# ruolin/strawberry

Measured on NVIDIA B200. Metric: fragments*EM-iters/sec, higher is better.
Workload: dtype f64

## Files before the change

### strawberry_b200/csrc/sbq.cu

```cuda
#include <algorithm>
#include <chrono>
#include <cstdarg>
#include <cstdio>
#include <cstdlib>
#include <cstring>
#include <dlfcn.h>
#include <mutex>
#include <string>
#include <thread>
#include <vector>

#include <nccl.h>

#include "../../include/sbq.h"
#include "../../include/sbq_builder.h"
#include "sbq_kernels.cuh"
#include "sbq_grid.cuh"
#include "sbq_grid_tma.cuh"
#include "sbq_grid_dual.cuh"
#include "sbq_bias.cuh"
#include "sbq_weights.cuh"
#include "sbq_synth.cuh"
#include "sbq_rawbuild.cuh"

// ... 226 lines not shown
   if (cudaPointerGetAttributes(&a, p) != cudaSuccess) {
      cudaGetLastError();
      return false;
   }
   return a.type == cudaMemoryTypeHost;
}

int materialise(sbq_ctx* c) {
   if (!c->borrowed) return SBQ_SUCCESS;
   if (c->host_released) return fail(c, SBQ_ERR_STATE, "the borrowed batch was released by sbq_upload: sbq_clear and submit again");
   bool ok = true;
   c->h_loc_row_off.clear(); c->h_loc_iso_off.clear(); c->h_row_ptr.clear();
   c->h_col.clear(); c->h_count.clear(); c->h_iso_len.clear(); c->h_alpha.clear();
   ok &= c->h_loc_row_off.append(c->b_loc_row_off, c->n_loci + 1);
   ok &= c->h_loc_iso_off.append(c->b_loc_iso_off, c->n_loci + 1);
   ok &= c->h_row_ptr.append(c->b_row_ptr, c->n_row + 1);
   ok &= c->h_col.append(c->b_col, c->nnz);
   ok &= c->h_alpha.append(c->b_alpha, c->nnz);
   ok &= c->h_count.append(c->b_count, c->n_row);
   ok &= c->h_iso_len.append(c->b_iso_len, c->n_iso);
   c->borrowed = false;
   return ok ? SBQ_SUCCESS : fail(c, SBQ_ERR_NOMEM, "pinned staging allocation failed");
}

void reset_batch(sbq_ctx* c) {
   c->borrowed = false;
   c->host_released = false;
   c->meta.clear();
   c->h_loc_row_off.clear(); c->h_loc_iso_off.clear(); c->h_row_ptr.clear();
   c->h_col.clear(); c->h_count.clear(); c->h_iso_len.clear(); c->h_alpha.clear();
   c->n_loci = c->n_row = c->n_iso = c->nnz = 0;
   c->have_cov = false;
   c->h_cov.clear();
   c->deferred = 0;
   c->raw.clear();
   c->raw_mode = false;
   c->h_wseg.clear(); c->h_wn.clear(); c->h_wmask.clear(); c->h_wpool.clear(); c->h_wlen.clear(); c->h_wpool_off.clear();
   c->resident = c->solved = c->downloaded = false;
}

int ensure_origin(sbq_ctx* c) {
   if (c->h_loc_row_off.n == 0) {
      int64_t z = 0;
      if (!c->h_loc_row_off.append(&z, 1) || !c->h_loc_iso_off.append(&z, 1) || !c->h_row_ptr.append(&z, 1))
         return fail(c, SBQ_ERR_NOMEM, "pinned staging allocation failed");
   }
   return SBQ_SUCCESS;
}

constexpr int N_BUCKETS = 5;
const int BUCKET_NT[N_BUCKETS] = {64, 128, 512, 512, 512};
int smem_bucket(size_t bytes) { return bytes <= 12 * 1024 ? 0 : bytes <= 24 * 1024 ? 1 : bytes <= 56 * 1024 ? 2 : bytes <= 112 * 1024 ? 3 : 4; }

constexpr int64_t SGRID_MAX_NNZ = 1000 * 1000;
constexpr int SGRID_CTAS_DEFAULT = 32;
inline int sgrid_ctas() {
   static const int v = getenv("SBQ_SGRID_CTAS") ? std::max(1, atoi(getenv("SBQ_SGRID_CTAS"))) : SGRID_CTAS_DEFAULT;
   return v;
}
#define SGRID_CTAS sgrid_ctas()

int cluster_size_for(int64_t nnz) {
   static int64_t th[4] = {16 * 1024, 32 * 1024, 64 * 1024, 150 * 1024};
   static bool init = false;
   if (!init) {
      init = true;
      if (const char* e = std::getenv("SBQ_CS_THRESH")) {
         long long a, b, c2, d;
         if (std::sscanf(e, "%lld,%lld,%lld,%lld", &a, &b, &c2, &d) == 4) { th[0] = a * 1024; th[1] = b * 1024; th[2] = c2 * 1024; th[3] = d * 1024; }
      }
   }
   if (nnz <= th[0]) return 1;
   if (nnz <= th[1]) return 2;
   if (nnz <= th[2]) return 4;
   if (nnz <= th[3]) return 8;
   return 16;
}

void capture_meta_host(sbq_ctx* c) {
   const int64_t *lro = loc_row_off(c), *lio = loc_iso_off(c), *rp = row_ptr(c);
   c->meta.resize((size_t)c->n_loci);
   for (int64_t l = 0; l < c->n_loci; ++l)
      c->meta[l] = {rp[lro[l + 1]] - rp[lro[l]], 0, (int32_t)(lro[l + 1] - lro[l]), (int32_t)(lio[l + 1] - lio[l])};
}

int plan(sbq_ctx* c) {
   c->warp_list.clear();
   c->grid_list.clear();
   c->sgrid_list.clear();
   c->sgrid_max_iso = c->sgrid_max_iso_dual = 1;
   c->sgrid_tma_ok = true;
   c->classes.clear();
   c->warp_max_iso = 1;
   c->max_iso_all = 1;
   c->grid_max_iso = 1;
   c->grid_max_iso_dual = 1;
   c->grid_tma_ok = true;
   c->grid_dual_ok = !getenv("SBQ_GRID_NO_DUAL");
   const bool force_dual = getenv("SBQ_GRID_DUAL") != nullptr;
   static const bool sgrid_enabled = !getenv("SBQ_NO_SGRID");
   std::vector<char> dual_locus(c->n_loci, 0);
   std::vector<int64_t> nnz_of(c->n_loci);
   LaunchClass* slot[5][N_BUCKETS] = {};
   std::vector<LaunchClass> tmp;
   tmp.reserve(20);
   static const int64_t grid_min_nnz = getenv("SBQ_GRID_MIN_NNZ") ? atoll(getenv("SBQ_GRID_MIN_NNZ")) : 300 * 1000;
   for (int64_t l = 0; l < c->n_loci; ++l) {
      const int64_t R = c->meta[l].R, T = c->meta[l].T, nnz = c->meta[l].nnz;
      nnz_of[l] = nnz;
      c->max_iso_all = std::max(c->max_iso_all, (int)T);
      if (T > SBQ_MAX_ISO) return fail(c, SBQ_ERR_UNSUPPORTED, "locus %lld has %lld isoforms (> SBQ_MAX_ISO)", (long long)l, (long long)T);
      int tier;
      if (c->force_tier) tier = c->force_tier;
      else if (T <= WT_MAX_ISO && R <= WT_MAX_ROWS && nnz <= WT_MAX_NNZ) tier = 1;
      else if (nnz >= grid_min_nnz) tier = 3;
      else tier = 2;
      if (tier == 1 && T > WT_MAX_ISO) tier = 2;
      if (tier == 3 && !grid_tier_supports((int)T)) tier = 2;
      if (tier == 2 && cluster_stream_groups((int)T, SMEM_CAP, CL_NT, 1, 0) <= 0) {
         if (!grid_tier_supports((int)T)) return fail(c, SBQ_ERR_UNSUPPORTED, "locus %lld: %lld isoforms fit no tier", (long long)l, (long long)T);
         tier = 3;
      }
      if (tier == 1) {
         c->warp_list.push_back((int32_t)l);
         c->warp_max_iso = std::max(c->warp_max_iso, (int)T);
      } else if (tier == 3) {
         const bool small = !c->force_tier && sgrid_enabled && nnz < SGRID_MAX_NNZ;
         (small ? c->sgrid_list : c->grid_list).push_back((int32_t)l);
         const bool dual = c->grid_dual_ok && (grid_dual_supports_iso((int)T) || (force_dual && grid_dual_possible((int)T))) &&
                           nnz < (1LL << 32) && nnz <= 56 * R;
         dual_locus[l] = dual;
         int& mx_dual = small ? c->sgrid_max_iso_dual : c->grid_max_iso_dual;
         int& mx_rest = small ? c->sgrid_max_iso : c->grid_max_iso;
         bool& tma_ok = small ? c->sgrid_tma_ok : c->grid_tma_ok;
         if (dual) {
            mx_dual = std::max(mx_dual, (int)T);
         } else {
            mx_rest = std::max(mx_rest, (int)T);
            if (!grid_tma_supports((int)T, (long long)R, small ? SGRID_CTAS : c->prop.multiProcessorCount)) tma_ok = false;
         }
      } else {
         int cs = c->force_cluster ? c->force_cluster : cluster_size_for(nnz);
         int csi = cs == 1 ? 0 : cs == 2 ? 1 : cs == 4 ? 2 : cs == 8 ? 3 : 4;
         const size_t slice = cluster_slice_estimate(nnz, R, (int)T, cs);
         const int bucket = cs == 1 ? smem_bucket(cluster_fixed_doubles((int)T, 1, slice) * sizeof(double) + slice + 256) : N_BUCKETS - 1;
         if (!slot[csi][bucket]) {
            tmp.push_back(LaunchClass{cs, BUCKET_NT[bucket], {}, 0, 0, 0, 0});
            slot[csi][bucket] = &tmp.back();
         }
         LaunchClass* lc = slot[csi][bucket];
         lc->loci.push_back((int32_t)l);
         lc->max_iso = std::max(lc->max_iso, (int)T);
         lc->max_slice = std::max(lc->max_slice, slice);
         lc->smem = std::max(lc->smem, cluster_class_smem((int)T, slice, lc->lpr, cs));
      }
   }
   auto by_size = [&](int32_t a, int32_t b) { return nnz_of[a] != nnz_of[b] ? nnz_of[a] > nnz_of[b] : a < b; };
   {
      bool small_keys = true;
      for (int32_t l : c->warp_list) small_keys &= nnz_of[l] <= WT_MAX_NNZ;
      if (small_keys) {
         std::vector<int32_t> first(WT_MAX_NNZ + 2, 0), sorted(c->warp_list.size());
         for (int32_t l : c->warp_list) ++first[WT_MAX_NNZ - (int)nnz_of[l] + 1];
         for (int k = 1; k <= WT_MAX_NNZ + 1; ++k) first[k] += first[k - 1];
         for (int32_t l : c->warp_list) sorted[first[WT_MAX_NNZ - (int)nnz_of[l]]++] = l;
         c->warp_list.swap(sorted);
      } else {
         std::sort(c->warp_list.begin(), c->warp_list.end(), by_size);
      }
   }
   auto order_grid = [&](std::vector<int32_t>& list, size_t& n_dual, std::vector<int64_t>& rec_off) {
      std::sort(list.begin(), list.end(), [&](int32_t a, int32_t b) {
         if (dual_locus[a] != dual_locus[b]) return dual_locus[a] > dual_locus[b];
         if (dual_locus[a]) {
            const int na = grid_dual_nc(c->meta[a].T), nb_ = grid_dual_nc(c->meta[b].T);
            if (na != nb_) return na > nb_;
         }
         return by_size(a, b);
      });
      n_dual = 0;
      for (int32_t l : list) n_dual += dual_locus[l];
      rec_off.assign(n_dual + 1, 0);
      for (size_t i = 0; i < n_dual; ++i) rec_off[i + 1] = rec_off[i] + c->meta[list[i]].R + 1;
   };
   order_grid(c->grid_list, c->grid_n_dual, c->grid_rec_off);
   order_grid(c->sgrid_list, c->sgrid_n_dual, c->sgrid_rec_off);
   for (auto& lc : tmp) {
      std::sort(lc.loci.begin(), lc.loci.end(), by_size);
      if (cluster_stream_groups(lc.max_iso, SMEM_CAP, lc.lpr, 1, 0) <= 0)
         return fail(c, SBQ_ERR_UNSUPPORTED, "locus with %d isoforms does not fit the cluster tier", lc.max_iso);
      c->classes.push_back(std::move(lc));
   }
   std::sort(c->classes.begin(), c->classes.end(), [](const LaunchClass& a, const LaunchClass& b) { return a.cs != b.cs ? a.cs > b.cs : a.max_slice > b.max_slice; });

   c->h_lists.clear();
   c->warp_list_off = 0;
   if (!c->h_lists.append(c->warp_list.data(), c->warp_list.size())) return fail(c, SBQ_ERR_NOMEM, "list staging");
   c->grid_list_off = c->h_lists.n;
   if (!c->h_lists.append(c->grid_list.data(), c->grid_list.size())) return fail(c, SBQ_ERR_NOMEM, "list staging");
   c->sgrid_list_off = c->h_lists.n;
   if (!c->h_lists.append(c->sgrid_list.data(), c->sgrid_list.size())) return fail(c, SBQ_ERR_NOMEM, "list staging");
   for (auto& lc : c->classes) {
      lc.list_off = c->h_lists.n;
      if (!c->h_lists.append(lc.loci.data(), lc.loci.size())) return fail(c, SBQ_ERR_NOMEM, "list staging");
   }
   c->stats.loci_warp = (int64_t)c->warp_list.size();
   c->stats.loci_grid = (int64_t)(c->grid_list.size() + c->sgrid_list.size());
   c->stats.loci_cta = c->n_loci - c->stats.loci_warp - c->stats.loci_grid;
   return SBQ_SUCCESS;
}

size_t align_up(size_t x, size_t a = 256) { return (x + a - 1) / a * a; }

int alloc_device(sbq_ctx* c) {
   const size_t sz_lro = align_up((c->n_loci + 1) * sizeof(int64_t)), sz_rp = align_up((c->n_row + 1) * sizeof(int64_t) + 64);
   const size_t sz_col = align_up(c->nnz * sizeof(int32_t) + 64), sz_al = align_up(c->nnz * sizeof(double) + 64);
   const size_t sz_cnt = align_up(c->n_row * sizeof(int32_t) + 64), sz_il = align_up(c->n_iso * sizeof(int32_t));
   const size_t in_bytes = 2 * sz_lro + sz_rp + sz_col + sz_al + 2 * sz_cnt + sz_il;
   const size_t sz_iso_d = align_up(c->n_iso * sizeof(double)), sz_iso_i = align_up(c->n_iso * sizeof(int32_t));
   const size_t sz_loc_i = align_up(c->n_loci * sizeof(int32_t)), sz_loc_d = align_up(c->n_loci * sizeof(double));
   const size_t out_bytes = 4 * sz_iso_d + sz_iso_i + 2 * sz_loc_i + sz_loc_d + 256;
   if (!c->d_in.reserve(in_bytes) || !c->d_out.reserve(out_bytes) || !c->d_lists.reserve(align_up((size_t)c->n_loci * sizeof(int32_t)) + 256))
      return fail(c, SBQ_ERR_NOMEM, "device allocation failed (%zu MB)", (in_bytes + out_bytes) >> 20);

   char* p = (char*)c->d_in.p;
   DevParams& dp = c->dp;
   auto carve = [&](size_t bytes) { char* q = p; p += bytes; return q; };
   int64_t* d_lro = (int64_t*)carve(sz_lro);
   int64_t* d_lio = (int64_t*)carve(sz_lro);
   int64_t* d_rp = (int64_t*)carve(sz_rp);
   int32_t* d_col = (int32_t*)carve(sz_col);
   double* d_al = (double*)carve(sz_al);
   int32_t* d_cnt = (int32_t*)carve(sz_cnt);
   dp.neff = (int32_t*)carve(sz_cnt);
   int32_t* d_il = (int32_t*)carve(sz_il);
   dp.csc = nullptr;
   dp.loc_row_off = d_lro; dp.loc_iso_off = d_lio; dp.row_ptr = d_rp; dp.col = d_col; dp.alpha = d_al;
   dp.count = d_cnt; dp.iso_len = d_il;
   p = (char*)c->d_out.p;
   dp.theta = (double*)carve(sz_iso_d);
   dp.fpkm = (double*)carve(sz_iso_d);
   dp.frac = (double*)carve(sz_iso_d);
   c->d_tpm = (double*)carve(sz_iso_d);
   dp.keep = (int32_t*)carve(sz_iso_i);
   dp.iters = (int32_t*)carve(sz_loc_i);
   dp.status = (int32_t*)carve(sz_loc_i);
   dp.locus_fpkm = (double*)carve(sz_loc_d);
   c->d_fpkm_sum = (double*)carve(256);
   c->d_lists_p = (int32_t*)c->d_lists.p;
   return SBQ_SUCCESS;
}

template <typename K>
int set_kernel_attrs(sbq_ctx* c, K kernel, size_t smem, bool nonportable) {
   CU(cudaFuncSetAttribute(kernel, cudaFuncAttributeMaxDynamicSharedMemorySize, (int)smem));
   if (nonportable) CU(cudaFuncSetAttribute(kernel, cudaFuncAttributeNonPortableClusterSizeAllowed, 1));
   return SBQ_SUCCESS;
}

template <int NT, int NCACHE, int MINB>
int launch_cluster_class_nt(sbq_ctx* c, const LaunchClass& lc, cudaStream_t st) {
   auto kernel = em_cluster_kernel<NT, NCACHE, MINB>;
   int rc = set_kernel_attrs(c, kernel, lc.smem, lc.cs > 8);
   if (rc) return rc;
   cudaLaunchConfig_t cfg{};
   cfg.gridDim = dim3((unsigned)(lc.loci.size() * lc.cs));
   cfg.blockDim = dim3(NT);
   cfg.dynamicSmemBytes = lc.smem;
   cfg.stream = st;
   cudaLaunchAttribute attr[1];
   attr[0].id = cudaLaunchAttributeClusterDimension;
   attr[0].val.clusterDim.x = (unsigned)lc.cs;
   attr[0].val.clusterDim.y = 1;
   attr[0].val.clusterDim.z = 1;
   cfg.attrs = attr;
   cfg.numAttrs = 1;
   const int32_t* list = c->d_lists_p + lc.list_off;
   CU(cudaLaunchKernelEx(&cfg, kernel, c->dp, list, (int)lc.loci.size(), (unsigned)lc.smem));
   return SBQ_SUCCESS;
}

struct StagingMark {
   size_t lro, lio, rp, col, al, cnt, il, wseg, wn, wmask, wlen, wpool, wpoff;
   int64_t n_loci, n_row, n_iso, nnz;
   explicit StagingMark(const sbq_ctx* c)
       : lro(c->h_loc_row_off.n), lio(c->h_loc_iso_off.n), rp(c->h_row_ptr.n), col(c->h_col.n), al(c->h_alpha.n), cnt(c->h_count.n), il(c->h_iso_len.n),
         wseg(c->h_wseg.n), wn(c->h_wn.n), wmask(c->h_wmask.n), wlen(c->h_wlen.n), wpool(c->h_wpool.n), wpoff(c->h_wpool_off.n),
         n_loci(c->n_loci), n_row(c->n_row), n_iso(c->n_iso), nnz(c->nnz) {}
   void restore(sbq_ctx* c) const {
      c->h_loc_row_off.n = lro; c->h_loc_iso_off.n = lio; c->h_row_ptr.n = rp; c->h_col.n = col; c->h_alpha.n = al; c->h_count.n = cnt; c->h_iso_len.n = il;
      c->h_wseg.n = wseg; c->h_wn.n = wn; c->h_wmask.n = wmask; c->h_wlen.n = wlen; c->h_wpool.n = wpool; c->h_wpool_off.n = wpoff;
      c->n_loci = n_loci; c->n_row = n_row; c->n_iso = n_iso; c->nnz = nnz;
   }
};

int submit_locked(sbq_ctx* c, const sbq_locus* loci, int64_t n_loci) {
   if (c->host_released) return fail(c, SBQ_ERR_STATE, "the borrowed batch was released by sbq_upload: sbq_clear and submit again");
   for (int64_t l = 0; l < n_loci; ++l) {
      const sbq_locus& L = loci[l];
      if (L.n_iso < 1 || L.n_row < 0 || !L.row_ptr || !L.iso_len || (L.n_row > 0 && !L.count))
         return fail(c, SBQ_ERR_INVALID, "locus %lld: bad shape or null pointer", (long long)l);
      if (L.n_iso > SBQ_MAX_ISO) return fail(c, SBQ_ERR_UNSUPPORTED, "locus %lld: %d isoforms > SBQ_MAX_ISO", (long long)l, L.n_iso);
      for (int32_t i = 1; i <= L.n_row; ++i)
         if (L.row_ptr[i] < L.row_ptr[i - 1]) return fail(c, SBQ_ERR_INVALID, "locus %lld: row_ptr not monotone", (long long)l);
      if (L.row_ptr[L.n_row] > L.row_ptr[0] && (!L.col || !L.alpha)) return fail(c, SBQ_ERR_INVALID, "locus %lld: null col / alpha", (long long)l);
   }
   cudaSetDevice(c->device);
   int rc = materialise(c);
   if (rc) return rc;
   if ((rc = ensure_origin(c))) return rc;
   const StagingMark mark(c);
   for (int64_t l = 0; l < n_loci; ++l) {
      const sbq_locus& L = loci[l];
      const int64_t k0 = L.row_ptr[0], k1 = L.row_ptr[L.n_row];
      const int64_t base = c->nnz - k0;
      bool ok = c->h_row_ptr.reserve(c->h_row_ptr.n + L.n_row);
      if (ok) {
         for (int32_t i = 1; i <= L.n_row; ++i) c->h_row_ptr.p[c->h_row_ptr.n++] = L.row_ptr[i] + base;
         ok = c->h_col.append(L.col + k0, k1 - k0) && c->h_alpha.append(L.alpha + k0, k1 - k0) &&
              c->h_count.append(L.count, L.n_row) && c->h_iso_len.append(L.iso_len, L.n_iso);
      }
      c->nnz += k1 - k0;
      c->n_row += L.n_row;
      c->n_iso += L.n_iso;
      c->n_loci += 1;
      ok = ok && c->h_loc_row_off.append(&c->n_row, 1) && c->h_loc_iso_off.append(&c->n_iso, 1);
      if (!ok) {
         mark.restore(c);
         return fail(c, SBQ_ERR_NOMEM, "pinned staging");
      }
   }
   c->resident = c->solved = c->downloaded = false;
   return SBQ_SUCCESS;
}

}

#include "sbq_multi.cuh"

extern "C" {

int sbq_abi_version(void) { return SBQ_ABI_VERSION; }

const char* sbq_error_string(int err) {
   switch (err) {
      case SBQ_SUCCESS: return "success";
      case SBQ_ERR_INVALID: return "invalid argument";
      case SBQ_ERR_NO_DEVICE: return "no CUDA device (libsbq has no CPU path)";
      case SBQ_ERR_CUDA: return "CUDA runtime error";
      case SBQ_ERR_NOMEM: return "out of memory";
      case SBQ_ERR_STATE: return "invalid call sequence";
      case SBQ_ERR_UNSUPPORTED: return "shape outside supported limits";
      default: return "unknown error";
   }
}

const char* sbq_last_error(const sbq_ctx* c) { return c ? c->err.c_str() : ""; }

void sbq_config_default(sbq_config* cfg) {
   if (!cfg) return;
   memset(cfg, 0, sizeof *cfg);
   cfg->device = -1;
   cfg->max_iter = 1000;
   cfg->theta_tol = 1e-2;
   cfg->row_eps = 1e-5;
   cfg->min_iso_frac = 0.0;
   cfg->effective_len_norm = 0;
   cfg->insert_mean = 0.0;
   cfg->bias_mode = 0;
   cfg->max_out_it = 100;
   cfg->max_theta_it = 5000;
   cfg->max_bias_it = 10;
   cfg->bias_tol = 1e-2;
   cfg->n_gpus = 1;
}

int sbq_create(const sbq_config* cfg, sbq_ctx** out) {
   if (!cfg || !out) return SBQ_ERR_INVALID;
   *out = nullptr;
   if (cfg->max_iter < 1 || !(cfg->theta_tol >= 0) || cfg->bias_mode < 0 || cfg->bias_mode > 1) return SBQ_ERR_INVALID;
   if (cfg->bias_mode == 1 && (cfg->max_out_it < 1 || cfg->max_theta_it < 1 || cfg->max_bias_it < 1 || !(cfg->bias_tol >= 0))) return SBQ_ERR_INVALID;
   if (cfg->n_gpus < 0 || cfg->n_gpus > 64) return SBQ_ERR_INVALID;
   setenv("CUDA_DEVICE_MAX_CONNECTIONS", "32", 0);
   int ndev = 0;
   if (cudaGetDeviceCount(&ndev) != cudaSuccess || ndev == 0) {
      cudaGetLastError();
      return SBQ_ERR_NO_DEVICE;
   }
   int dev = cfg->device;
   if (dev < 0) {
      if (cfg->n_gpus > 1) dev = 0;
      else if (cudaGetDevice(&dev) != cudaSuccess) return SBQ_ERR_NO_DEVICE;
   }
   if (dev >= ndev) return SBQ_ERR_INVALID;
   if (cfg->n_gpus > 1 && dev + cfg->n_gpus > ndev) return SBQ_ERR_NO_DEVICE;
   sbq_ctx* c = new sbq_ctx();
   c->cfg = *cfg;
   c->device = dev;
   auto bail = [&](int code) { sbq_destroy(c); return code; };
   if (cudaSetDevice(dev) != cudaSuccess) return bail(SBQ_ERR_CUDA);
   if (cudaGetDeviceProperties(&c->prop, dev) != cudaSuccess) return bail(SBQ_ERR_CUDA);
   if (c->prop.major < 10) return bail(SBQ_ERR_NO_DEVICE);
   if (cudaStreamCreateWithFlags(&c->stream, cudaStreamNonBlocking) != cudaSuccess) return bail(SBQ_ERR_CUDA);
   if (cudaStreamCreateWithFlags(&c->copy_st, cudaStreamNonBlocking) != cudaSuccess) return bail(SBQ_ERR_CUDA);
   if (cudaEventCreateWithFlags(&c->ev_grid_ready, cudaEventDisableTiming) != cudaSuccess) return bail(SBQ_ERR_CUDA);
   for (auto& e : c->ev_class_ready)
      if (cudaEventCreateWithFlags(&e, cudaEventDisableTiming) != cudaSuccess) return bail(SBQ_ERR_CUDA);
   for (auto& s : c->side)
      if (cudaStreamCreateWithFlags(&s, cudaStreamNonBlocking) != cudaSuccess) return bail(SBQ_ERR_CUDA);
   for (auto& e : c->ev)
      if (cudaEventCreate(&e) != cudaSuccess) return bail(SBQ_ERR_CUDA);
   if (cudaEventCreateWithFlags(&c->ev_fork, cudaEventDisableTiming) != cudaSuccess) return bail(SBQ_ERR_CUDA);
   for (auto& e : c->ev_join)
      if (cudaEventCreateWithFlags(&e, cudaEventDisableTiming) != cudaSuccess) return bail(SBQ_ERR_CUDA);
   for (auto& t : c->lt)
// ... 89 lines not shown
   if (rows < 0 || isos < n_loci) return fail(c, SBQ_ERR_INVALID, "bad locus offsets");
   const int64_t k0 = rp[lro[0]], k1 = rp[lro[n_loci]];
   if (k1 < k0 || (k1 > k0 && (!col || !alpha)) || (rows > 0 && !count)) return fail(c, SBQ_ERR_INVALID, "bad CSR arrays");
   for (int64_t l = 0; l < n_loci; ++l) {
      const int64_t T = lio[l + 1] - lio[l];
      if (lro[l + 1] < lro[l] || T < 1) return fail(c, SBQ_ERR_INVALID, "locus %lld: bad shape", (long long)l);
      if (T > SBQ_MAX_ISO) return fail(c, SBQ_ERR_UNSUPPORTED, "locus %lld: %lld isoforms > SBQ_MAX_ISO", (long long)l, (long long)T);
   }
   if (c->n_loci == 0 && lro[0] == 0 && lio[0] == 0 && k0 == 0 && is_pinned(lro) && is_pinned(lio) && is_pinned(rp) &&
       is_pinned(iso_len) && (rows == 0 || is_pinned(count)) && (k1 == 0 || (is_pinned(col) && is_pinned(alpha)))) {
      c->borrowed = true;
      c->b_loc_row_off = lro; c->b_loc_iso_off = lio; c->b_row_ptr = rp;
      c->b_col = col; c->b_alpha = alpha; c->b_count = count; c->b_iso_len = iso_len;
      c->n_loci = n_loci; c->n_row = rows; c->n_iso = isos; c->nnz = k1;
      c->deferred = 2;
      c->resident = c->solved = c->downloaded = false;
      return SBQ_SUCCESS;
   }
   if (c->host_released) return fail(c, SBQ_ERR_STATE, "the borrowed batch was released by sbq_upload: sbq_clear and submit again");
   for (int64_t i = lro[0]; i < lro[n_loci]; ++i)
      if (rp[i + 1] < rp[i]) return fail(c, SBQ_ERR_INVALID, "row %lld: row_ptr not monotone", (long long)i);
   int rc = materialise(c);
   if (rc) return rc;
   if ((rc = ensure_origin(c))) return rc;
   const bool ok = c->h_loc_row_off.reserve(c->h_loc_row_off.n + n_loci) && c->h_loc_iso_off.reserve(c->h_loc_iso_off.n + n_loci) &&
                   c->h_row_ptr.reserve(c->h_row_ptr.n + rows) && c->h_col.reserve(c->h_col.n + (k1 - k0)) && c->h_alpha.reserve(c->h_alpha.n + (k1 - k0)) &&
                   c->h_count.reserve(c->h_count.n + rows) && c->h_iso_len.reserve(c->h_iso_len.n + isos);
   if (!ok) return fail(c, SBQ_ERR_NOMEM, "pinned staging");
   for (int64_t l = 1; l <= n_loci; ++l) {
      c->h_loc_row_off.p[c->h_loc_row_off.n++] = c->n_row + (lro[l] - lro[0]);
      c->h_loc_iso_off.p[c->h_loc_iso_off.n++] = c->n_iso + (lio[l] - lio[0]);
   }
   const int64_t base = c->nnz - k0;
   for (int64_t i = 1; i <= rows; ++i) c->h_row_ptr.p[c->h_row_ptr.n++] = rp[lro[0] + i] + base;
   c->h_col.append(col + k0, k1 - k0);
   c->h_alpha.append(alpha + k0, k1 - k0);
   c->h_count.append(count + lro[0], rows);
   c->h_iso_len.append(iso_len + lio[0], isos);
   c->n_loci += n_loci; c->n_row += rows; c->n_iso += isos; c->nnz += k1 - k0;
   c->deferred = 2;
   c->resident = c->solved = c->downloaded = false;
   return SBQ_SUCCESS;
}

int sbq_validate(sbq_ctx* c) {
   if (!c) return SBQ_ERR_INVALID;
   std::lock_guard<std::mutex> lk(c->mu);
   if (c->host_released) return fail(c, SBQ_ERR_STATE, "the borrowed batch was released by sbq_upload");
   const int64_t *lro = loc_row_off(c), *lio = loc_iso_off(c), *rp = row_ptr(c);
   const int32_t* col = colp(c);
   for (int64_t l = 0; l < c->n_loci; ++l) {
      const int64_t T = lio[l + 1] - lio[l];
      for (int64_t i = lro[l]; i < lro[l + 1]; ++i) {
         if (rp[i + 1] < rp[i]) return fail(c, SBQ_ERR_INVALID, "locus %lld row %lld: row_ptr not monotone", (long long)l, (long long)(i - lro[l]));
         for (int64_t k = rp[i]; k < rp[i + 1]; ++k) {
            if (col[k] < 0 || col[k] >= T) return fail(c, SBQ_ERR_INVALID, "locus %lld: column %d out of range", (long long)l, col[k]);
            if (k > rp[i] && col[k] <= col[k - 1]) return fail(c, SBQ_ERR_INVALID, "locus %lld row %lld: columns not strictly ascending", (long long)l, (long long)(i - lro[l]));
         }
      }
   }
   return SBQ_SUCCESS;
}

}

static int raw_upload(sbq_ctx* c);

static int upload_begin(sbq_ctx* c) {
   CU(cudaSetDevice(c->device));
   if (c->upload_pending) {
      CU(cudaStreamSynchronize(c->copy_st));
      c->upload_pending = false;
   }
   if (c->n_loci == 0) return fail(c, SBQ_ERR_STATE, "nothing submitted");
   if (c->host_released) return fail(c, SBQ_ERR_STATE, "the borrowed batch was released by the previous sbq_upload: sbq_clear and submit again");
   {
      const int rc = alloc_device(c);
      if (rc) return rc;
   }
   DevParams& dp = c->dp;
   int64_t *d_lro = const_cast<int64_t*>(dp.loc_row_off), *d_lio = const_cast<int64_t*>(dp.loc_iso_off), *d_rp = const_cast<int64_t*>(dp.row_ptr);
   int32_t *d_col = const_cast<int32_t*>(dp.col), *d_cnt = const_cast<int32_t*>(dp.count), *d_il = const_cast<int32_t*>(dp.iso_len);
   double* d_al = const_cast<double*>(dp.alpha);

   cudaStream_t st = c->copy_st;
   c->upload_pending = true;
   c->resident = c->solved = c->downloaded = false;
   CU(cudaEventRecord(c->ev[0], st));
   CU(cudaMemcpyAsync(d_lro, loc_row_off(c), (c->n_loci + 1) * sizeof(int64_t), cudaMemcpyHostToDevice, st));
   CU(cudaMemcpyAsync(d_lio, loc_iso_off(c), (c->n_loci + 1) * sizeof(int64_t), cudaMemcpyHostToDevice, st));
   CU(cudaMemcpyAsync(d_rp, row_ptr(c), (c->n_row + 1) * sizeof(int64_t), cudaMemcpyHostToDevice, st));
   if (c->n_row) CU(cudaMemcpyAsync(d_cnt, countp(c), c->n_row * sizeof(int32_t), cudaMemcpyHostToDevice, st));
   CU(cudaMemcpyAsync(d_il, iso_lenp(c), c->n_iso * sizeof(int32_t), cudaMemcpyHostToDevice, st));
   if (!c->r_frags.reserve((size_t)c->n_loci) || !c->d_frags.reserve(align_up((size_t)c->n_loci * 8))) return fail(c, SBQ_ERR_NOMEM, "fragment-total buffers");
   locus_frags_kernel<<<std::max(1, std::min<int>((int)((c->n_loci + 7) / 8), c->prop.multiProcessorCount * 8)), 256, 0, st>>>(d_lro, d_cnt, c->n_loci, (long long*)c->d_frags.p);
   CU(cudaGetLastError());
   CU(cudaMemcpyAsync(c->r_frags.p, c->d_frags.p, (size_t)c->n_loci * 8, cudaMemcpyDeviceToHost, st));
   if (c->nnz) CU(cudaMemcpyAsync(d_col, colp(c), c->nnz * sizeof(int32_t), cudaMemcpyHostToDevice, st));
   const bool timing = getenv("SBQ_TIMING") != nullptr;
   const auto t_plan0 = std::chrono::steady_clock::now();
   {
      capture_meta_host(c);
      const int rc = plan(c);
      if (rc) {
         cudaStreamSynchronize(st);
         c->upload_pending = false;
         return rc;
      }
   }
   if (timing) fprintf(stderr, "SBQ_TIMING plan_ms %.3f\n", std::chrono::duration<double, std::milli>(std::chrono::steady_clock::now() - t_plan0).count());
   if (c->h_lists.n) CU(cudaMemcpyAsync(c->d_lists_p, c->h_lists.p, c->h_lists.n * sizeof(int32_t), cudaMemcpyHostToDevice, st));
   const int64_t* lro = loc_row_off(c);
   const int64_t* rp = row_ptr(c);
   const double* al = alphap(c);
   std::vector<std::pair<int64_t, int64_t>> done;
   auto copy_loci = [&](const std::vector<int32_t>& loci) -> int {
      for (int32_t l : loci) {
         const int64_t k0 = rp[lro[l]], k1 = rp[lro[l + 1]];
         if (k1 > k0) {
            CU(cudaMemcpyAsync(d_al + k0, al + k0, (size_t)(k1 - k0) * sizeof(double), cudaMemcpyHostToDevice, st));
            done.emplace_back(k0, k1);
         }
      }
      return SBQ_SUCCESS;
   };
   for (auto& r : c->class_ready) r = false;
   c->grid_ready = false;
   if (!(c->grid_list.empty() && c->sgrid_list.empty()) && c->grid_list.size() + c->sgrid_list.size() <= 16) {
      int rc = copy_loci(c->grid_list);
      if (rc) return rc;
      rc = copy_loci(c->sgrid_list);
      if (rc) return rc;
      CU(cudaEventRecord(c->ev_grid_ready, st));
      c->grid_ready = true;
   }
   size_t n_prio = 0;
   for (size_t i = 0; i < c->classes.size() && i < (size_t)N_SIDE_STREAMS; ++i) {
      if (c->classes[i].cs < 8 || n_prio + c->classes[i].loci.size() > 48) continue;
      n_prio += c->classes[i].loci.size();
      const int rc = copy_loci(c->classes[i].loci);
      if (rc) return rc;
      CU(cudaEventRecord(c->ev_class_ready[i], st));
      c->class_ready[i] = true;
   }
   std::sort(done.begin(), done.end());
   int64_t pos = 0;
   for (size_t i = 0; i <= done.size(); ++i) {
      const int64_t end = i < done.size() ? done[i].first : c->nnz;
      if (end > pos) CU(cudaMemcpyAsync(d_al + pos, al + pos, (size_t)(end - pos) * sizeof(double), cudaMemcpyHostToDevice, st));
      if (i < done.size()) pos = std::max(pos, done[i].second);
   }
   CU(cudaEventRecord(c->ev[1], st));
   if (!c->classes.empty()) {
      if (!c->d_csc.reserve(align_up(c->nnz * 4 + 16))) return fail(c, SBQ_ERR_NOMEM, "device allocation failed (transposed-index scratch)");
      dp.csc = (unsigned*)c->d_csc.p;
   }
   c->stats.h2d_bytes = 2 * (c->n_loci + 1) * 8 + (c->n_row + 1) * 8 + c->nnz * 12 + c->n_row * 4 + c->n_iso * 4 + (int64_t)c->h_lists.n * 4;
   c->stats.n_loci = c->n_loci; c->stats.n_row = c->n_row; c->stats.n_iso = c->n_iso; c->stats.nnz = c->nnz;
   c->stats.weights_ms = 0.0;
   c->col16_ready = false;
   c->resident = true;
   return SBQ_SUCCESS;
}

static int upload_wait(sbq_ctx* c) {
   if (!c->upload_pending) return SBQ_SUCCESS;
   CU(cudaSetDevice(c->device));
   CU(cudaStreamSynchronize(c->copy_st));
   c->upload_pending = false;
   if (c->borrowed) c->host_released = true;
   for (size_t l = 0; l < c->meta.size(); ++l) c->meta[l].frags = c->r_frags.p[l];
   float ms = 0;
   CU(cudaEventElapsedTime(&ms, c->ev[0], c->ev[1]));
   c->stats.upload_ms = ms;
   return SBQ_SUCCESS;
}

extern "C" {

int sbq_upload_begin(sbq_ctx* c) {
   if (!c) return SBQ_ERR_INVALID;
   if (c->multi || c->deferred == 1 || c->raw_mode || c->cfg.bias_mode == 1) return sbq_upload(c);
   std::lock_guard<std::mutex> lk(c->mu);
   return upload_begin(c);
}

int sbq_upload(sbq_ctx* c) {
   if (!c) return SBQ_ERR_INVALID;
   if (c->multi) return multi_upload(c);
   std::lock_guard<std::mutex> lk(c->mu);
   if (c->raw_mode) {
      if (c->n_loci == 0) return fail(c, SBQ_ERR_STATE, "nothing submitted");
      return raw_upload(c);
   }
   {
      int rc = upload_begin(c);
      if (!rc) rc = upload_wait(c);
      if (rc) return rc;
   }
   if (c->deferred == 1) {
      if (!c->have_model) return fail(c, SBQ_ERR_STATE, "deferred weights need sbq_set_insert_model()");
      if ((int64_t)c->h_wseg.n != c->nnz) return fail(c, SBQ_ERR_STATE, "deferred-weight descriptors do not cover the batch");
      const size_t b_seg = align_up(c->nnz * 8 + 8), b_n = align_up(c->nnz + 8), b_m = align_up(c->nnz * 4 + 8), b_l = align_up(c->nnz * 4 + 8);
      const size_t b_pool = align_up(c->h_wpool.n * 4 + 8), b_emp = align_up(c->model_emp.size() * 8 + 8);
      if (!c->d_weights.reserve(b_seg + b_n + b_m + b_l + b_pool + b_emp)) return fail(c, SBQ_ERR_NOMEM, "device allocation failed (weight descriptors)");
      char* q = (char*)c->d_weights.p;
      int64_t* d_seg = (int64_t*)q; q += b_seg;
      uint8_t* d_n = (uint8_t*)q; q += b_n;
      uint32_t* d_m = (uint32_t*)q; q += b_m;
      int32_t* d_l = (int32_t*)q; q += b_l;
      uint32_t* d_pool = (uint32_t*)q; q += b_pool;
      double* d_emp = (double*)q;
      cudaStream_t st = c->stream;
      CU(cudaEventRecord(c->ev[5], st));
      CU(cudaMemcpyAsync(d_seg, c->h_wseg.p, c->nnz * 8, cudaMemcpyHostToDevice, st));
      CU(cudaMemcpyAsync(d_n, c->h_wn.p, c->nnz, cudaMemcpyHostToDevice, st));
      CU(cudaMemcpyAsync(d_m, c->h_wmask.p, c->nnz * 4, cudaMemcpyHostToDevice, st));
      CU(cudaMemcpyAsync(d_l, c->h_wlen.p, c->nnz * 4, cudaMemcpyHostToDevice, st));
      if (c->h_wpool.n) CU(cudaMemcpyAsync(d_pool, c->h_wpool.p, c->h_wpool.n * 4, cudaMemcpyHostToDevice, st));
      if (!c->model_emp.empty()) CU(cudaMemcpyAsync(d_emp, c->model_emp.data(), c->model_emp.size() * 8, cudaMemcpyHostToDevice, st));
      WeightModel wm{c->model.use_emp, c->model.start_offset, c->model.end_offset, c->model.total_reads, d_emp, c->model.mean, c->model.sd, c->model_read_len};
      const int blocks = std::max(1, std::min<int>((int)((c->nnz + 7) / 8), c->prop.multiProcessorCount * 16));
      weights_kernel<<<blocks, 256, 0, st>>>(c->nnz, d_seg, d_n, d_m, d_l, d_pool, wm, const_cast<double*>(c->dp.alpha));
      CU(cudaGetLastError());
      CU(cudaEventRecord(c->ev[6], st));
      CU(cudaStreamSynchronize(st));
      float wms = 0;
      CU(cudaEventElapsedTime(&wms, c->ev[5], c->ev[6]));
      c->weights_ms = wms;
      c->stats.weights_ms = wms;
      c->stats.h2d_bytes += (int64_t)(c->nnz * 17 + c->h_wpool.n * 4 + c->model_emp.size() * 8);
   }
   if (c->cfg.bias_mode == 1) {
      if (!c->have_cov) return fail(c, SBQ_ERR_STATE, "bias_mode = 1 needs sbq_set_covariates() after the last submit");
      const size_t K = (size_t)c->n_cov;
      const size_t bx = align_up(c->n_row * K * 8 + 8), bw = align_up(c->n_row * 8 + 8), bb = align_up(c->n_loci * K * 8 + 8), bo = align_up(c->n_loci * 4 + 8);
      if (!c->d_bias.reserve(bx + 2 * bw + bb + 2 * bo + 64)) return fail(c, SBQ_ERR_NOMEM, "device allocation failed (bias scratch)");
      char* q = (char*)c->d_bias.p;
      c->bpar.x = (const double*)q; q += bx;
      c->bpar.w = (double*)q; q += bw;
      c->bpar.d = (double*)q; q += bw;
      c->bpar.beta = (double*)q; q += bb;
      c->bpar.outer = (int32_t*)q; q += bo;
      c->d_bias_list = (int32_t*)q; q += bo;
      c->d_bias_queue = (int*)q;
      c->bpar.n_cov = c->n_cov;
      {
         c->bias_list.clear();
         std::vector<int32_t> cls[6];
         for (int k = 0; k < 6; ++k) c->bias_cls[k] = BiasClass{};
         for (int64_t l = 0; l < c->n_loci; ++l) {
            const int cs = bias_cluster_size(c->meta[l].nnz);
            const int k = bias_warp_tier(c->meta[l].nnz, c->meta[l].R, c->meta[l].T) ? 5 : cs == 16 ? 0 : cs == 8 ? 1 : cs == 4 ? 2 : cs == 2 ? 3 : 4;
            cls[k].push_back((int32_t)l);
            c->bias_cls[k].cs = cs;
            c->bias_cls[k].max_iso = std::max(c->bias_cls[k].max_iso, (int)c->meta[l].T);
         }
         for (int k = 0; k < 6; ++k) {
            std::sort(cls[k].begin(), cls[k].end(), [&](int32_t a, int32_t b) { return c->meta[a].nnz != c->meta[b].nnz ? c->meta[a].nnz > c->meta[b].nnz : a < b; });
            c->bias_cls[k].off = c->bias_list.size();
            c->bias_cls[k].n = cls[k].size();
            c->bias_list.insert(c->bias_list.end(), cls[k].begin(), cls[k].end());
         }
         if (c->n_loci) CU(cudaMemcpyAsync(c->d_bias_list, c->bias_list.data(), c->n_loci * 4, cudaMemcpyHostToDevice, c->stream));
      }
      if (K) CU(cudaMemcpyAsync((void*)c->bpar.x, c->h_cov.p, c->n_row * K * 8, cudaMemcpyHostToDevice, c->stream));
      CU(cudaStreamSynchronize(c->stream));
      c->stats.h2d_bytes += (int64_t)(c->n_row * K * 8);
   }
   c->resident = true;
   c->col16_ready = false;
   c->solved = c->downloaded = false;
   return SBQ_SUCCESS;
}

int sbq_solve(sbq_ctx* c, int64_t total_mapped_reads) {
   if (!c) return SBQ_ERR_INVALID;
   if (c->multi) return multi_solve(c, total_mapped_reads);
   std::lock_guard<std::mutex> lk(c->mu);
   CU(cudaSetDevice(c->device));
   if (!c->resident) return fail(c, SBQ_ERR_STATE, "sbq_solve before sbq_upload");

   DevParams& dp = c->dp;
   dp.max_iter = c->cfg.max_iter;
   dp.tol = c->cfg.theta_tol;
   dp.row_eps = c->cfg.row_eps;
   dp.min_frac = c->cfg.min_iso_frac;
   dp.eff_len_norm = c->cfg.effective_len_norm;
   dp.insert_mean = c->cfg.insert_mean;
   dp.rpm = 1e6 / (double)(int)total_mapped_reads;

   cudaStream_t st = c->stream;
   int64_t launches = 0;
   if (c->cfg.bias_mode == 1) {
      const size_t smem = bias_smem_bytes(c->max_iso_all);
      if (smem > SMEM_CAP) return fail(c, SBQ_ERR_UNSUPPORTED, "bias mode supports up to %d isoforms per locus", (int)((SMEM_CAP / 8 - 8) / (5 + BI_W)));
      c->bpar.max_out_it = c->cfg.max_out_it;
      c->bpar.max_theta_it = c->cfg.max_theta_it;
      c->bpar.max_bias_it = c->cfg.max_bias_it;
      c->bpar.bias_tol = c->cfg.bias_tol;
      int rc_attr = set_kernel_attrs(c, em_bias_kernel, smem, c->bias_cls[0].n > 0);
      if (rc_attr) return rc_attr;
      CU(cudaEventRecord(c->ev[2], st));
      CU(cudaEventRecord(c->ev_fork, st));
      int n_side = 0;
      if (c->bias_cls[5].n) {
         const BiasClass& bc = c->bias_cls[5];
         cudaStream_t ss = c->side[n_side];
         CU(cudaStreamWaitEvent(ss, c->ev_fork, 0));
         ++n_side;
         const size_t wsmem = bias_warp_smem_bytes();
         CU(cudaFuncSetAttribute(em_bias_warp_kernel, cudaFuncAttributeMaxDynamicSharedMemorySize, (int)wsmem));
         int occ = 1;
         CU(cudaOccupancyMaxActiveBlocksPerMultiprocessor(&occ, em_bias_warp_kernel, BW_WARPS * 32, wsmem));
         const long long want = ((long long)bc.n + BW_WARPS - 1) / BW_WARPS;
         const unsigned grid = (unsigned)std::max(1LL, std::min(want, (long long)c->prop.multiProcessorCount * std::max(1, occ)));
         CU(cudaMemsetAsync(c->d_bias_queue, 0, sizeof(int), ss));
         em_bias_warp_kernel<<<grid, BW_WARPS * 32, wsmem, ss>>>(c->dp, c->bpar, (const int32_t*)(c->d_bias_list + bc.off), (int)bc.n, c->d_bias_queue);
         CU(cudaGetLastError());
         ++launches;
      }
      for (int k = 0; k < 5; ++k) {
         const BiasClass& bc = c->bias_cls[k];
         if (!bc.n) continue;
         cudaStream_t ss = c->side[n_side % N_SIDE_STREAMS];
         if (n_side < N_SIDE_STREAMS) CU(cudaStreamWaitEvent(ss, c->ev_fork, 0));
         ++n_side;
         cudaLaunchConfig_t cfg{};
         cfg.gridDim = dim3((unsigned)(bc.n * bc.cs));
         cfg.blockDim = dim3(BI_NT);
         cfg.dynamicSmemBytes = bias_smem_bytes(bc.max_iso);
         cfg.stream = ss;
         cudaLaunchAttribute attr[1];
         attr[0].id = cudaLaunchAttributeClusterDimension;
         attr[0].val.clusterDim.x = (unsigned)bc.cs;
         attr[0].val.clusterDim.y = 1;
         attr[0].val.clusterDim.z = 1;
         cfg.attrs = attr;
         cfg.numAttrs = 1;
         CU(cudaLaunchKernelEx(&cfg, em_bias_kernel, c->dp, c->bpar, (const int32_t*)(c->d_bias_list + bc.off), (int)bc.n));
         ++launches;
      }
      for (int i = 0; i < std::min(n_side, N_SIDE_STREAMS); ++i) {
         CU(cudaEventRecord(c->ev_join[i], c->side[i]));
         CU(cudaStreamWaitEvent(st, c->ev_join[i], 0));
      }
      CU(cudaEventRecord(c->ev[3], st));
      fpkm_sum_kernel<<<1, 1024, 0, st>>>(dp.locus_fpkm, c->n_loci, c->d_fpkm_sum);
      CU(cudaGetLastError());
      CU(cudaEventRecord(c->ev[4], st));
      CU(cudaStreamSynchronize(st));
      float ms_ = 0;
      CU(cudaEventElapsedTime(&ms_, c->ev[2], c->ev[4]));
      c->stats.solve_ms = ms_;
      CU(cudaEventElapsedTime(&ms_, c->ev[2], c->ev[3]));
      c->stats.em_ms = ms_;
      c->stats.grid_em_ms = 0;
      c->stats.kernel_launches = launches + 1;
      c->launch_stats.clear();
      c->locus_launch.assign(c->n_loci, -1);
      c->solved = true;
      c->downloaded = false;
      return SBQ_SUCCESS;
   }
   CU(cudaEventRecord(c->ev[2], st));
   CU(cudaEventRecord(c->ev_fork, st));
   int used_side = 0;
   c->stats.grid_em_ms = 0;
   for (auto& t : c->lt) t.used = false;
   const bool pending = c->upload_pending;
   auto launch_grid_part = [&](const std::vector<int32_t>& list, size_t list_off, size_t n_dual_, const std::vector<int64_t>& rec_off, int max_iso_rest,
                               bool tma_ok, const cudaDeviceProp& prop_, DevBuf& scratch, DevBuf& rowrec, DevBuf& pkbuf, cudaStream_t gs_, int& variant,
                               int& n_launch) -> int {
      int rc = 0;
      variant = 0;
      const int32_t* d_grid = c->d_lists_p + list_off;
      const int n_dual = (int)n_dual_, n_rest = (int)list.size() - n_dual;
      if (n_dual) {
         GridDualBufs bf{&scratch.p, &scratch.cap, &c->d_col16.p, &c->d_col16.cap, &rowrec.p, &rowrec.cap, &pkbuf.p, &pkbuf.cap};
         int nl = 0;
         std::vector<int> h_iso((size_t)n_dual);
         for (int i = 0; i < n_dual; ++i) h_iso[i] = c->meta[list[i]].T;
         rc = grid_dual_launch(c->dp, c->nnz, d_grid, n_dual, h_iso.data(), rec_off.data(), prop_, bf, c->col16_ready, gs_, &nl);
         n_launch += nl;
         variant = 3;
      }
      if (rc == 0 && n_rest) {
         int nl = 0;
         if (tma_ok && !getenv("SBQ_GRID_NO_TMA")) {
            if (!variant) variant = 2;
            rc = grid_tma_launch(c->dp, c->nnz, d_grid + n_dual, n_rest, max_iso_rest, prop_, &scratch.p, &scratch.cap,
                                 &c->d_col16.p, &c->d_col16.cap, c->col16_ready, gs_, &nl);
         } else {
            if (!variant) variant = 1;
            rc = grid_tier_launch(c->dp, d_grid + n_dual, n_rest, prop_, &scratch.p, &scratch.cap, gs_, &nl);
         }
         n_launch += nl;
      }
      return rc;
   };
   auto grid_failed = [&](int rc) -> int {
      c->resident = false;
      c->col16_ready = false;
      return fail(c, rc < -6 ? SBQ_ERR_CUDA : rc, "grid tier launch failed: %s", cudaGetErrorString(cudaGetLastError()));
   };
   if (!(c->grid_list.empty() && c->sgrid_list.empty())) {
      const size_t need16 = (size_t)c->nnz * 2 + 256;
      if (need16 > c->d_col16.cap) {
         if (!c->d_col16.reserve(need16)) return fail(c, SBQ_ERR_NOMEM, "device allocation failed (16-bit slots)");
         c->col16_ready = false;
      }
   }
   if (!c->grid_list.empty()) {
      if (pending) CU(cudaStreamWaitEvent(st, c->grid_ready ? c->ev_grid_ready : c->ev[1], 0));
      CU(cudaEventRecord(c->ev[6], st));
      int n_launch = 0;
      const int rc = launch_grid_part(c->grid_list, c->grid_list_off, c->grid_n_dual, c->grid_rec_off, c->grid_max_iso, c->grid_tma_ok, c->prop,
                                      c->d_grid_scratch, c->d_rowrec, c->d_pk, st, c->grid_variant, n_launch);
      if (rc != 0) return grid_failed(rc);
      launches += n_launch;
      CU(cudaEventRecord(c->ev[7], st));
   }
   c->lt_sgrid.used = false;
   if (!c->sgrid_list.empty()) {
      cudaDeviceProp prop_sg = c->prop;
      prop_sg.multiProcessorCount = std::min(SGRID_CTAS, c->prop.multiProcessorCount);
      cudaStream_t gs_ = c->sgrid_st;
      CU(cudaStreamWaitEvent(gs_, c->ev_fork, 0));
      if (pending) CU(cudaStreamWaitEvent(gs_, c->grid_ready ? c->ev_grid_ready : c->ev[1], 0));
      if (!c->grid_list.empty()) {
         CU(cudaStreamWaitEvent(gs_, c->ev[7], 0));
      }
      CU(cudaEventRecord(c->lt_sgrid.e0, gs_));
      int n_launch = 0;
      const int rc = launch_grid_part(c->sgrid_list, c->sgrid_list_off, c->sgrid_n_dual, c->sgrid_rec_off, c->sgrid_max_iso, c->sgrid_tma_ok, prop_sg,
                                      c->d_sgrid_scratch, c->d_srowrec, c->d_spk, gs_, c->sgrid_variant, n_launch);
      if (rc != 0) return grid_failed(rc);
      launches += n_launch;
      CU(cudaEventRecord(c->lt_sgrid.e1, gs_));
      CU(cudaEventRecord(c->ev_sgrid_join, gs_));
      c->lt_sgrid.used = true;
   }
   if (!(c->grid_list.empty() && c->sgrid_list.empty())) c->col16_ready = true;
   const bool serialize = getenv("SBQ_SERIALIZE") != nullptr;
   static const int order_mode = getenv("SBQ_ORDER") ? atoi(getenv("SBQ_ORDER")) : SBQ_DEFAULT_ORDER;
   const int ncls = (int)c->classes.size();
   std::vector<int> ord;
   int warp_pos = ncls;
   {
      std::vector<int> big, small, rest;
      for (int i = 0; i < ncls; ++i) {
         const LaunchClass& lc = c->classes[i];
         if (lc.lpr < CL_NT) small.push_back(i);
         else if (lc.cs >= (order_mode == 3 ? 16 : 8)) big.push_back(i);
         else rest.push_back(i);
      }
      if (order_mode == 1) { ord = small; ord.insert(ord.end(), big.begin(), big.end()); ord.insert(ord.end(), rest.begin(), rest.end()); warp_pos = 0; }
      else if (order_mode == 2 || order_mode == 3) { ord = big; warp_pos = (int)ord.size(); ord.insert(ord.end(), small.begin(), small.end()); ord.insert(ord.end(), rest.begin(), rest.end()); }
      else { for (int i = 0; i < ncls; ++i) ord.push_back(i); }
   }
   auto launch_warp = [&]() -> int {
      if (c->warp_list.empty()) return SBQ_SUCCESS;
      const size_t smem = warp_tier_smem_bytes(c->warp_max_iso);
      CU(cudaFuncSetAttribute(em_warp_kernel, cudaFuncAttributeMaxDynamicSharedMemorySize, (int)smem));
      const int n = (int)c->warp_list.size();
      int per_sm = 1;
      CU(cudaOccupancyMaxActiveBlocksPerMultiprocessor(&per_sm, em_warp_kernel, WT_WARPS * 32, smem));
      int grid = std::max(1, std::min((n + WT_WARPS - 1) / WT_WARPS, per_sm * c->prop.multiProcessorCount));
      static const int warp_cta_cap = getenv("SBQ_WARP_CTAS") ? atoi(getenv("SBQ_WARP_CTAS")) : SBQ_DEFAULT_WARP_CTAS;
      if (warp_cta_cap > 0) grid = std::min(grid, warp_cta_cap);
      int* queue = (int*)((char*)c->d_fpkm_sum + 64);
      if (pending) CU(cudaStreamWaitEvent(st, c->ev[1], 0));
      CU(cudaMemsetAsync(queue, 0, sizeof(int), st));
      CU(cudaEventRecord(c->lt[0].e0, st));
      em_warp_kernel<<<grid, WT_WARPS * 32, smem, st>>>(c->dp, c->d_lists_p + c->warp_list_off, n, c->warp_max_iso, queue);
      CU(cudaGetLastError());
      CU(cudaEventRecord(c->lt[0].e1, st));
      c->lt[0].used = true;
      ++launches;
      return SBQ_SUCCESS;
   };
   for (int pos = 0; pos <= ncls; ++pos) {
      if (pos == warp_pos) {
         const int rcw = launch_warp();
         if (rcw) return rcw;
      }
      if (pos == ncls) break;
      const int i = ord[pos];
      const LaunchClass& lc = c->classes[i];
      cudaStream_t ss = serialize ? st : c->side[i % N_SIDE_STREAMS];
      if (!serialize && i < N_SIDE_STREAMS) CU(cudaStreamWaitEvent(ss, c->ev_fork, 0));
      if (pending) CU(cudaStreamWaitEvent(ss, (i < N_SIDE_STREAMS && c->class_ready[i]) ? c->ev_class_ready[i] : c->ev[1], 0));
      LaunchTimer& t = c->lt[2 + i % N_SIDE_STREAMS];
      CU(cudaEventRecord(t.e0, ss));
      int rc = lc.lpr == 64 ? launch_cluster_class_nt<64, 0, 8>(c, lc, ss) : lc.lpr == 128 ? launch_cluster_class_nt<128, 0, 4>(c, lc, ss) :
               lc.lpr == 256 ? launch_cluster_class_nt<256, 0, 2>(c, lc, ss) : launch_cluster_class_nt<CL_NT, 0, 1>(c, lc, ss);
      if (rc) return rc;
      CU(cudaEventRecord(t.e1, ss));
      t.used = true;
      ++launches;
   }
   used_side = ncls;
   for (int i = 0; i < std::min(used_side, N_SIDE_STREAMS) && !serialize; ++i) {
      CU(cudaEventRecord(c->ev_join[i], c->side[i]));
      CU(cudaStreamWaitEvent(st, c->ev_join[i], 0));
   }
   if (c->lt_sgrid.used) CU(cudaStreamWaitEvent(st, c->ev_sgrid_join, 0));
   CU(cudaEventRecord(c->ev[3], st));
   fpkm_sum_kernel<<<1, 1024, 0, st>>>(dp.locus_fpkm, c->n_loci, c->d_fpkm_sum);
   CU(cudaGetLastError());
   ++launches;
   CU(cudaEventRecord(c->ev[4], st));
   CU(cudaStreamSynchronize(st));
   if (pending) {
      const int rcw = upload_wait(c);
      if (rcw) return rcw;
   }
   float ms = 0;
   CU(cudaEventElapsedTime(&ms, c->ev[2], c->ev[4]));
   c->stats.solve_ms = ms;
   CU(cudaEventElapsedTime(&ms, c->ev[2], c->ev[3]));
   c->stats.em_ms = ms;
   if (!c->grid_list.empty()) {
      CU(cudaEventElapsedTime(&ms, c->ev[6], c->ev[7]));
      c->stats.grid_em_ms = ms;
   }
   c->launch_stats.clear();
   c->locus_launch.assign(c->n_loci, -1);
   auto add_stat = [&](int kind, int cs, int lpr, const std::vector<int32_t>& loci, double ms_, cudaEvent_t e0 = nullptr) {
      sbq_launch_stat ls{};
      ls.kind = kind; ls.cluster_size = cs; ls.lanes_per_row = lpr; ls.n_loci = (int64_t)loci.size(); ls.ms = ms_;
      float st_ms = 0;
      if (e0 && cudaEventElapsedTime(&st_ms, c->ev[2], e0) == cudaSuccess) ls.start_ms = st_ms;
      for (int32_t l : loci) c->locus_launch[l] = (int32_t)c->launch_stats.size();
      c->launch_stats.push_back(ls);
   };
   if (c->lt[0].used) { CU(cudaEventElapsedTime(&ms, c->lt[0].e0, c->lt[0].e1)); add_stat(1, 1, 1, c->warp_list, ms, c->lt[0].e0); }
   if (!c->grid_list.empty()) { add_stat(3, 0, 32, c->grid_list, c->stats.grid_em_ms, c->ev[6]); c->launch_stats.back().variant = c->grid_variant; }
   if (c->lt_sgrid.used) {
      CU(cudaEventElapsedTime(&ms, c->lt_sgrid.e0, c->lt_sgrid.e1));
      add_stat(3, std::min(SGRID_CTAS, c->prop.multiProcessorCount), 32, c->sgrid_list, ms, c->lt_sgrid.e0);
      c->launch_stats.back().variant = c->sgrid_variant;
   }
   for (size_t i = 0; i < c->classes.size(); ++i) {
      LaunchTimer& t = c->lt[2 + i % N_SIDE_STREAMS];
      CU(cudaEventElapsedTime(&ms, t.e0, t.e1));
      add_stat(2, c->classes[i].cs, c->classes[i].lpr, c->classes[i].loci, ms, t.e0);
   }
   c->stats.kernel_launches = launches;
   c->solved = true;
   c->downloaded = false;
   return SBQ_SUCCESS;
}

int sbq_fpkm_sum(sbq_ctx* c, double* local_sum) {
   if (!c || !local_sum) return SBQ_ERR_INVALID;
   if (c->multi) {
      std::lock_guard<std::mutex> lk(c->mu);
      if (!c->solved) return fail(c, SBQ_ERR_STATE, "sbq_fpkm_sum before sbq_solve");
      const int rc = multi_allreduce_locked(c);
      if (!rc) *local_sum = c->multi->global_sum;
      return rc;
   }
   std::lock_guard<std::mutex> lk(c->mu);
   CU(cudaSetDevice(c->device));
   if (!c->solved) return fail(c, SBQ_ERR_STATE, "sbq_fpkm_sum before sbq_solve");
   CU(cudaMemcpyAsync(local_sum, c->d_fpkm_sum, sizeof(double), cudaMemcpyDeviceToHost, c->stream));
   CU(cudaStreamSynchronize(c->stream));
   return SBQ_SUCCESS;
}

int sbq_fpkm_sum_to_device(sbq_ctx* c, void* dev_double) {
   if (!c || !dev_double) return SBQ_ERR_INVALID;
   if (c->multi) {
      std::lock_guard<std::mutex> lk(c->mu);
      if (!c->solved) return fail(c, SBQ_ERR_STATE, "sbq_fpkm_sum_to_device before sbq_solve");
      const int rc = multi_allreduce_locked(c);
      if (rc) return rc;
      CU(cudaMemcpy(dev_double, c->multi->d_sum[0] + 1, sizeof(double), cudaMemcpyDefault));
      return SBQ_SUCCESS;
   }
   std::lock_guard<std::mutex> lk(c->mu);
   CU(cudaSetDevice(c->device));
   if (!c->solved) return fail(c, SBQ_ERR_STATE, "sbq_fpkm_sum_to_device before sbq_solve");
   CU(cudaMemcpyAsync(dev_double, c->d_fpkm_sum, sizeof(double), cudaMemcpyDeviceToDevice, c->stream));
   CU(cudaStreamSynchronize(c->stream));
   return SBQ_SUCCESS;
}

int sbq_finalize_tpm(sbq_ctx* c, double global_fpkm_sum) {
   if (!c) return SBQ_ERR_INVALID;
   if (c->multi) return multi_finalize_tpm(c, global_fpkm_sum);
   std::lock_guard<std::mutex> lk(c->mu);
   CU(cudaSetDevice(c->device));
   if (!c->solved) return fail(c, SBQ_ERR_STATE, "sbq_finalize_tpm before sbq_solve");
   const int64_t n = c->n_iso;
   tpm_kernel<<<(unsigned)((n + 255) / 256), 256, 0, c->stream>>>(c->dp.fpkm, c->d_tpm, n, global_fpkm_sum);
   CU(cudaGetLastError());
   c->stats.kernel_launches += 1;
   c->downloaded = false;
   return SBQ_SUCCESS;
}

int sbq_download(sbq_ctx* c) {
   if (!c) return SBQ_ERR_INVALID;
   if (c->multi) return multi_download(c);
   std::lock_guard<std::mutex> lk(c->mu);
   CU(cudaSetDevice(c->device));
   if (!c->solved) return fail(c, SBQ_ERR_STATE, "sbq_download before sbq_solve");
   const size_t ni = c->n_iso, nl = c->n_loci;
   bool ok = c->r_theta.reserve(ni) && c->r_fpkm.reserve(ni) && c->r_frac.reserve(ni) && c->r_tpm.reserve(ni) &&
             c->r_keep.reserve(ni) && c->r_iters.reserve(nl) && c->r_status.reserve(nl) && c->r_locus_fpkm.reserve(nl);
   if (!ok) return fail(c, SBQ_ERR_NOMEM, "pinned result buffers");
   cudaStream_t st = c->stream;
   CU(cudaEventRecord(c->ev[8], st));
   CU(cudaMemcpyAsync(c->r_theta.p, c->dp.theta, ni * 8, cudaMemcpyDeviceToHost, st));
   CU(cudaMemcpyAsync(c->r_fpkm.p, c->dp.fpkm, ni * 8, cudaMemcpyDeviceToHost, st));
   CU(cudaMemcpyAsync(c->r_frac.p, c->dp.frac, ni * 8, cudaMemcpyDeviceToHost, st));
   CU(cudaMemcpyAsync(c->r_tpm.p, c->d_tpm, ni * 8, cudaMemcpyDeviceToHost, st));
   CU(cudaMemcpyAsync(c->r_keep.p, c->dp.keep, ni * 4, cudaMemcpyDeviceToHost, st));
   CU(cudaMemcpyAsync(c->r_iters.p, c->dp.iters, nl * 4, cudaMemcpyDeviceToHost, st));
   CU(cudaMemcpyAsync(c->r_status.p, c->dp.status, nl * 4, cudaMemcpyDeviceToHost, st));
   CU(cudaMemcpyAsync(&c->r_fpkm_sum, c->d_fpkm_sum, 8, cudaMemcpyDeviceToHost, st));
   CU(cudaEventRecord(c->ev[9], st));
   CU(cudaStreamSynchronize(st));
   float ms = 0;
   CU(cudaEventElapsedTime(&ms, c->ev[8], c->ev[9]));
   c->stats.download_ms = ms;
   c->stats.d2h_bytes = (int64_t)ni * 36 + (int64_t)nl * 8 + 8;

   c->stats_stale = true;
   c->downloaded = true;
   return SBQ_SUCCESS;
}

int sbq_run(sbq_ctx* c, int64_t total_mapped_reads) {
   int rc = sbq_upload_begin(c);
   if (rc) return rc;
   if ((rc = sbq_solve(c, total_mapped_reads))) return rc;
   if (c->multi) {
      if ((rc = multi_tpm(c))) return rc;
      return sbq_download(c);
   }
   double s = 0.0;
   if ((rc = sbq_fpkm_sum(c, &s))) return rc;
   if ((rc = sbq_finalize_tpm(c, s))) return rc;
   return sbq_download(c);
}

// ... 201 lines not shown
      while (cap < 2 * Hl) cap <<= 1;
      tab_off[l + 1] = tab_off[l] + cap;
   }
   const int64_t CM = cm_off[L], TAB = tab_off[L];
   const int n_scan = (int)((std::max<int64_t>(H, 1) + RB_SCAN_BLOCK - 1) / RB_SCAN_BLOCK);
   size_t need = 0;
   auto sz = [&](size_t bytes) { const size_t o = need; need += align_up(bytes + 16); return o; };
   const size_t o_hl = sz(H * 4), o_hfp = sz((H + 1) * 8), o_hfo = sz(r.hf_off.size() * 4), o_hfl = sz(r.hf_len.size() * 4), o_hfc = sz(r.hf_code.size());
   const size_t o_hm = sz(H * 4), o_hr = sz(H * 4), o_lho = sz((L + 1) * 8), o_lio = sz((L + 1) * 8), o_lso = sz((L + 1) * 8);
   const size_t o_ifp = sz((T + 1) * 8), o_ifo = sz(r.if_off.size() * 4), o_ifl = sz(r.if_len.size() * 4), o_ifc = sz(r.if_code.size());
   const size_t o_sl = sz(S * 4), o_sr = sz(S * 4), o_isp = sz((T + 1) * 8), o_isg = sz(r.iso_seg.size() * 4), o_il = sz(T * 4);
   const size_t o_co = sz(H * RB_MAXC * 2), o_nc = sz(H), o_va = sz(H), o_ch = sz(H * 8), o_fh = sz(H * 8), o_cmo = sz((L + 1) * 8), o_cm = sz(CM * 4);
   const size_t o_to = sz((L + 1) * 8), o_k1 = sz(TAB * 8), o_m1 = sz(TAB * 4), o_s1 = sz(H * 4), o_k2 = sz(TAB * 8), o_m2 = sz(TAB * 4), o_s2 = sz(H * 4);
   const size_t o_ir = sz(H * 4), o_cp = sz((H + 1) * 8), o_hc = sz(H * 4), o_fl = sz(64), o_bs = sz((size_t)n_scan * 8 + 8), o_g = sz((L + 1) * 8);
   if (!c->d_raw.reserve(need)) return fail(c, SBQ_ERR_NOMEM, "device allocation failed (raw batch, %zu MB)", need >> 20);
   char* base = (char*)c->d_raw.p;
   cudaStream_t st = c->stream;
   CU(cudaEventRecord(c->ev[0], st));
   auto up = [&](size_t off, const void* src, size_t bytes) -> int {
      if (bytes) CU(cudaMemcpyAsync(base + off, src, bytes, cudaMemcpyHostToDevice, st));
      return 0;
   };
   int rc = 0;
   rc |= up(o_hl, r.hit_locus.data(), H * 4); rc |= up(o_hfp, r.hit_feat_ptr.data(), (H + 1) * 8); rc |= up(o_hfo, r.hf_off.data(), r.hf_off.size() * 4);
   rc |= up(o_hfl, r.hf_len.data(), r.hf_len.size() * 4); rc |= up(o_hfc, r.hf_code.data(), r.hf_code.size()); rc |= up(o_hm, r.hit_mass.data(), H * 4);
   rc |= up(o_hr, r.hit_ref.data(), H * 4); rc |= up(o_lho, r.loc_hit_off.data(), (L + 1) * 8); rc |= up(o_lio, lio, (L + 1) * 8);
   rc |= up(o_lso, r.loc_seg_off.data(), (L + 1) * 8); rc |= up(o_ifp, r.iso_feat_ptr.data(), (T + 1) * 8); rc |= up(o_ifo, r.if_off.data(), r.if_off.size() * 4);
   rc |= up(o_ifl, r.if_len.data(), r.if_len.size() * 4); rc |= up(o_ifc, r.if_code.data(), r.if_code.size()); rc |= up(o_sl, r.seg_left.data(), S * 4);
   rc |= up(o_sr, r.seg_right.data(), S * 4); rc |= up(o_isp, r.iso_seg_ptr.data(), (T + 1) * 8); rc |= up(o_isg, r.iso_seg.data(), r.iso_seg.size() * 4);
   rc |= up(o_il, c->h_iso_len.p, T * 4); rc |= up(o_cmo, cm_off.data(), (L + 1) * 8); rc |= up(o_to, tab_off.data(), (L + 1) * 8);
   if (rc) return SBQ_ERR_CUDA;
   RawBatch& b = c->rb;
   b = RawBatch{};
   b.n_hit = H; b.n_loci = (int32_t)L; b.long_read = r.long_read;
   b.hit_locus = (const int32_t*)(base + o_hl); b.hit_feat_ptr = (const int64_t*)(base + o_hfp); b.hf_off = (const uint32_t*)(base + o_hfo);
   b.hf_len = (const uint32_t*)(base + o_hfl); b.hf_code = (const uint8_t*)(base + o_hfc); b.hit_mass = (const float*)(base + o_hm);
   b.hit_ref = (const int32_t*)(base + o_hr); b.loc_hit_off = (const int64_t*)(base + o_lho); b.loc_iso_off = (const int64_t*)(base + o_lio);
   b.loc_seg_off = (const int64_t*)(base + o_lso); b.iso_feat_ptr = (const int64_t*)(base + o_ifp); b.if_off = (const uint32_t*)(base + o_ifo);
   b.if_len = (const uint32_t*)(base + o_ifl); b.if_code = (const uint8_t*)(base + o_ifc); b.seg_left = (const uint32_t*)(base + o_sl);
   b.seg_right = (const uint32_t*)(base + o_sr); b.iso_seg_ptr = (const int64_t*)(base + o_isp); b.iso_seg = (const int32_t*)(base + o_isg);
   b.iso_len = (const int32_t*)(base + o_il);
   b.coords = (uint16_t*)(base + o_co); b.ncoord = (uint8_t*)(base + o_nc); b.valid = (uint8_t*)(base + o_va); b.chash = (unsigned long long*)(base + o_ch);
   b.fhash = (unsigned long long*)(base + o_fh); b.loc_cm_off = (const int64_t*)(base + o_cmo); b.cm = (uint32_t*)(base + o_cm);
   b.loc_tab_off = (const int64_t*)(base + o_to); b.keys1 = (unsigned long long*)(base + o_k1); b.min1 = (uint32_t*)(base + o_m1); b.slot1 = (uint32_t*)(base + o_s1);
   b.keys2 = (unsigned long long*)(base + o_k2); b.min2 = (uint32_t*)(base + o_m2); b.slot2 = (uint32_t*)(base + o_s2);
   b.is_rep = (int32_t*)(base + o_ir); b.cls_prefix = (int64_t*)(base + o_cp); b.hit_class = (int32_t*)(base + o_hc); b.flags = (int*)(base + o_fl);
   long long* d_bs = (long long*)(base + o_bs);
   int64_t* d_gather = (int64_t*)(base + o_g);
   CU(cudaMemsetAsync(base + o_k1, 0xff, TAB * 8, st));
   CU(cudaMemsetAsync(base + o_m1, 0xff, TAB * 4, st));
   CU(cudaMemsetAsync(base + o_k2, 0xff, TAB * 8, st));
   CU(cudaMemsetAsync(base + o_m2, 0xff, TAB * 4, st));
   CU(cudaMemsetAsync(b.flags, 0, 64, st));
   const int nbk = std::max(1, std::min<int>((int)((H + 127) / 128), c->prop.multiProcessorCount * 16));
   auto check_flags = [&](const char* where) -> int {
      int f = 0;
      CU(cudaMemcpyAsync(&f, b.flags, sizeof f, cudaMemcpyDeviceToHost, st));
      CU(cudaStreamSynchronize(st));
      if (f) return fail(c, SBQ_ERR_UNSUPPORTED, "device class assignment refused the batch (%s):%s%s%s%s - use the host builder (sbq_build_locus) for it", where,
                         f & RB_FLAG_COORDS ? " a hit touches more than 16 exon segments;" : "", f & RB_FLAG_COLLISION ? " 64-bit hash collision;" : "",
                         f & RB_FLAG_MASS ? " fragment masses are not multiples of 1/2 (or a class holds >= 2^23): the float sum would depend on the set order;" : "",
                         f & RB_FLAG_NSEG ? " a class spans more than 32 segments of an isoform;" : "");
      return 0;
   };
   if (H) {
      raw_hit_kernel<<<nbk, 128, 0, st>>>(b);
      raw_class_insert_kernel<<<nbk, 256, 0, st>>>(b);
      raw_class_rep_kernel<<<nbk, 256, 0, st>>>(b);
      CU(cudaGetLastError());
   }
   if (rb_scan(st, b.is_rep, H, d_bs, b.cls_prefix)) return fail(c, SBQ_ERR_CUDA, "scan failed");
   rb_gather_kernel<<<(unsigned)((L + 1 + 255) / 256), 256, 0, st>>>(b.cls_prefix, b.loc_hit_off, L + 1, d_gather);
   std::vector<int64_t> cls_off(L + 1);
   CU(cudaMemcpyAsync(cls_off.data(), d_gather, (L + 1) * 8, cudaMemcpyDeviceToHost, st));
   if ((rc = check_flags("hits"))) return rc;
   const int64_t R = cls_off[L];
   std::vector<int64_t> cmask_off(L + 1, 0);
   std::vector<int32_t> class_locus((size_t)R);
   for (int64_t l = 0; l < L; ++l) {
      const int64_t W = (lio[l + 1] - lio[l] + 31) / 32;
      cmask_off[l + 1] = cmask_off[l] + (cls_off[l + 1] - cls_off[l]) * W;
      for (int64_t x = cls_off[l]; x < cls_off[l + 1]; ++x) class_locus[x] = (int32_t)l;
   }
   size_t need2 = 0;
   auto sz2 = [&](size_t bytes) { const size_t o = need2; need2 += align_up(bytes + 16); return o; };
   const int n_scan2 = (int)((std::max<int64_t>(R, 1) + RB_SCAN_BLOCK - 1) / RB_SCAN_BLOCK);
   const size_t p_co = sz2((L + 1) * 8), p_mo = sz2((L + 1) * 8), p_cl = sz2(R * 4), p_rep = sz2(R * 8), p_ms = sz2(R * 4), p_nf = sz2(R * 4), p_cmk = sz2(cmask_off[L] * 4),
                p_nz = sz2(R * 4), p_rp = sz2((R + 1) * 8), p_bs = sz2((size_t)n_scan2 * 8 + 8), p_g = sz2((L + 1) * 8);
   if (!c->d_raw2.reserve(need2)) return fail(c, SBQ_ERR_NOMEM, "device allocation failed (class arrays)");
   char* base2 = (char*)c->d_raw2.p;
   CU(cudaMemcpyAsync(base2 + p_co, cls_off.data(), (L + 1) * 8, cudaMemcpyHostToDevice, st));
   CU(cudaMemcpyAsync(base2 + p_mo, cmask_off.data(), (L + 1) * 8, cudaMemcpyHostToDevice, st));
   if (R) CU(cudaMemcpyAsync(base2 + p_cl, class_locus.data(), R * 4, cudaMemcpyHostToDevice, st));
   CU(cudaMemsetAsync(base2 + p_ms, 0, align_up(R * 4 + 16), st));
   CU(cudaMemsetAsync(base2 + p_nf, 0, align_up(R * 4 + 16), st));
   CU(cudaMemsetAsync(base2 + p_cmk, 0, align_up(cmask_off[L] * 4 + 16), st));
   b.loc_cls_off = (const int64_t*)(base2 + p_co); b.loc_cmask_off = (const int64_t*)(base2 + p_mo); b.class_rep = (int64_t*)(base2 + p_rep);
   b.class_mass = (float*)(base2 + p_ms); b.class_nfrag = (int32_t*)(base2 + p_nf); b.cmask = (uint32_t*)(base2 + p_cmk); b.class_nnz = (int32_t*)(base2 + p_nz);
   const int32_t* d_class_locus = (const int32_t*)(base2 + p_cl);
   int64_t* d_rp_tmp = (int64_t*)(base2 + p_rp);
   const int nbc = std::max(1, std::min<int>((int)((R + 127) / 128), c->prop.multiProcessorCount * 16));
   if (H) {
      raw_member_kernel<<<nbk, 256, 0, st>>>(b);
      raw_mass_kernel<<<nbk, 256, 0, st>>>(b);
   }
   if (R) raw_nnz_kernel<<<nbc, 256, 0, st>>>(b, R, d_class_locus);
   CU(cudaGetLastError());
   if (rb_scan(st, b.class_nnz, R, (long long*)(base2 + p_bs), d_rp_tmp)) return fail(c, SBQ_ERR_CUDA, "scan failed");
   rb_gather_kernel<<<(unsigned)((L + 1 + 255) / 256), 256, 0, st>>>(d_rp_tmp, b.loc_cls_off, L + 1, (int64_t*)(base2 + p_g));
   std::vector<int64_t> nz_off(L + 1);
   CU(cudaMemcpyAsync(nz_off.data(), base2 + p_g, (L + 1) * 8, cudaMemcpyDeviceToHost, st));
   if ((rc = check_flags("classes"))) return rc;
   c->n_row = R;
   c->nnz = nz_off[L];
   if ((rc = alloc_device(c))) return rc;
   DevParams& dp = c->dp;
   CU(cudaMemcpyAsync(const_cast<int64_t*>(dp.loc_row_off), cls_off.data(), (L + 1) * 8, cudaMemcpyHostToDevice, st));
   CU(cudaMemcpyAsync(const_cast<int64_t*>(dp.loc_iso_off), lio, (L + 1) * 8, cudaMemcpyHostToDevice, st));
   CU(cudaMemcpyAsync(const_cast<int64_t*>(dp.row_ptr), d_rp_tmp, (R + 1) * 8, cudaMemcpyDeviceToDevice, st));
   CU(cudaMemcpyAsync(const_cast<int32_t*>(dp.iso_len), c->h_iso_len.p, T * 4, cudaMemcpyHostToDevice, st));
   const int64_t nnz = c->nnz;
   const size_t b_seg = align_up(nnz * 8 + 8), b_n = align_up(nnz + 8), b_m = align_up(nnz * 4 + 8), b_l = align_up(nnz * 4 + 8), b_pool = align_up((size_t)nnz * RB_POOL * 4 + 8),
                b_emp = align_up(c->model_emp.size() * 8 + 8);
   if (!c->d_weights.reserve(b_seg + b_n + b_m + b_l + b_pool + b_emp)) return fail(c, SBQ_ERR_NOMEM, "device allocation failed (weight descriptors)");
   char* q = (char*)c->d_weights.p;
   int64_t* d_seg = (int64_t*)q; q += b_seg;
   uint8_t* d_n = (uint8_t*)q; q += b_n;
   uint32_t* d_m = (uint32_t*)q; q += b_m;
   int32_t* d_l = (int32_t*)q; q += b_l;
   uint32_t* d_pool = (uint32_t*)q; q += b_pool;
   double* d_emp = (double*)q;
   if (R) raw_fill_kernel<<<nbc, 128, 0, st>>>(b, R, d_class_locus, dp.row_ptr, const_cast<int32_t*>(dp.col), const_cast<double*>(dp.alpha), const_cast<int32_t*>(dp.count),
                                               d_seg, d_n, d_m, d_l, d_pool);
   CU(cudaGetLastError());
   if ((rc = check_flags("weights"))) return rc;
   CU(cudaEventRecord(c->ev[5], st));
   if (!r.long_read && nnz) {
      if (!c->model_emp.empty()) CU(cudaMemcpyAsync(d_emp, c->model_emp.data(), c->model_emp.size() * 8, cudaMemcpyHostToDevice, st));
      WeightModel wm{c->model.use_emp, c->model.start_offset, c->model.end_offset, c->model.total_reads, d_emp, c->model.mean, c->model.sd, c->model_read_len};
      const int blocks = std::max(1, std::min<int>((int)((nnz + 7) / 8), c->prop.multiProcessorCount * 16));
      weights_kernel<<<blocks, 256, 0, st>>>(nnz, d_seg, d_n, d_m, d_l, d_pool, wm, const_cast<double*>(dp.alpha));
      CU(cudaGetLastError());
   }
   CU(cudaEventRecord(c->ev[6], st));
   if (!c->r_frags.reserve((size_t)L) || !c->d_frags.reserve(align_up((size_t)L * 8))) return fail(c, SBQ_ERR_NOMEM, "fragment-total buffers");
   locus_frags_kernel<<<std::max(1, std::min<int>((int)((L + 7) / 8), c->prop.multiProcessorCount * 8)), 256, 0, st>>>(dp.loc_row_off, dp.count, L, (long long*)c->d_frags.p);
   CU(cudaMemcpyAsync(c->r_frags.p, c->d_frags.p, (size_t)L * 8, cudaMemcpyDeviceToHost, st));
   CU(cudaStreamSynchronize(st));
   c->meta.resize((size_t)L);
   for (int64_t l = 0; l < L; ++l) c->meta[l] = {nz_off[l + 1] - nz_off[l], c->r_frags.p[l], (int32_t)(cls_off[l + 1] - cls_off[l]), (int32_t)(lio[l + 1] - lio[l])};
   if ((rc = plan(c))) return rc;
   if (c->h_lists.n) CU(cudaMemcpyAsync(c->d_lists_p, c->h_lists.p, c->h_lists.n * sizeof(int32_t), cudaMemcpyHostToDevice, st));
   if (!c->classes.empty()) {
      if (!c->d_csc.reserve(align_up(c->nnz * 4 + 16))) return fail(c, SBQ_ERR_NOMEM, "device allocation failed (transposed-index scratch)");
      dp.csc = (unsigned*)c->d_csc.p;
   }
   CU(cudaEventRecord(c->ev[1], st));
   CU(cudaStreamSynchronize(st));
   float ms = 0;
   CU(cudaEventElapsedTime(&ms, c->ev[0], c->ev[1]));
   c->stats.upload_ms = ms;
   CU(cudaEventElapsedTime(&ms, c->ev[5], c->ev[6]));
   c->stats.weights_ms = ms;
   c->weights_ms = ms;
   c->stats.h2d_bytes = (int64_t)(H * 20 + r.hf_off.size() * 9 + r.if_off.size() * 9 + S * 8 + r.iso_seg.size() * 4 + T * 20 + L * 40);
   c->stats.n_loci = c->n_loci; c->stats.n_row = c->n_row; c->stats.n_iso = c->n_iso; c->stats.nnz = c->nnz;
   c->resident = true;
   c->col16_ready = false;
   c->solved = c->downloaded = false;
   return SBQ_SUCCESS;
}

extern "C" {

int sbq_fetch_raw_classes(sbq_ctx* c, int32_t* hit_class, uint8_t* hit_ncoord, uint16_t* hit_coords, int64_t* class_rep, float* class_mass, int32_t* class_nfrag) {
   if (!c) return SBQ_ERR_INVALID;
   std::lock_guard<std::mutex> lk(c->mu);
   if (c->multi) return fail(c, SBQ_ERR_UNSUPPORTED, "sbq_fetch_raw_classes is single-device (a test aid)");
   CU(cudaSetDevice(c->device));
   if (!c->resident || !c->raw_mode) return fail(c, SBQ_ERR_STATE, "sbq_fetch_raw_classes needs an uploaded raw batch");
   const RawBatch& b = c->rb;
   cudaStream_t st = c->stream;
   if (hit_class && b.n_hit) CU(cudaMemcpyAsync(hit_class, b.hit_class, b.n_hit * 4, cudaMemcpyDeviceToHost, st));
   if (hit_ncoord && b.n_hit) CU(cudaMemcpyAsync(hit_ncoord, b.ncoord, b.n_hit, cudaMemcpyDeviceToHost, st));
   if (hit_coords && b.n_hit) CU(cudaMemcpyAsync(hit_coords, b.coords, b.n_hit * RB_MAXC * 2, cudaMemcpyDeviceToHost, st));
   if (class_rep && c->n_row) CU(cudaMemcpyAsync(class_rep, b.class_rep, c->n_row * 8, cudaMemcpyDeviceToHost, st));
   if (class_mass && c->n_row) CU(cudaMemcpyAsync(class_mass, b.class_mass, c->n_row * 4, cudaMemcpyDeviceToHost, st));
   if (class_nfrag && c->n_row) CU(cudaMemcpyAsync(class_nfrag, b.class_nfrag, c->n_row * 4, cudaMemcpyDeviceToHost, st));
   CU(cudaStreamSynchronize(st));
   return SBQ_SUCCESS;
}

int sbq_synth_giant(sbq_ctx* c, const sbq_synth_giant_spec* sp) {
   if (!c || !sp || sp->n_loci < 1 || sp->rows_per_locus < 1 || sp->iso_lo < 1 || sp->iso_hi < sp->iso_lo || sp->iso_hi > SBQ_MAX_ISO ||
       !(sp->mean_extra >= 0) || sp->mean_extra > 200.0)
      return SBQ_ERR_INVALID;
   if (c->multi) return fail(c, SBQ_ERR_UNSUPPORTED, "sbq_synth_giant is per device: give every device of a partition its own locus ids");
   if (c->cfg.bias_mode) return fail(c, SBQ_ERR_UNSUPPORTED, "sbq_synth_giant generates no covariates");
   std::lock_guard<std::mutex> lk(c->mu);
   CU(cudaSetDevice(c->device));
   reset_batch(c);
   const int L = sp->n_loci;
   const int64_t rows = sp->rows_per_locus, n_row = (int64_t)L * rows;
   std::vector<SynthLocus> hl((size_t)L);
   std::vector<int64_t> h_lro((size_t)L + 1), h_lio((size_t)L + 1, 0);
   for (int l = 0; l < L; ++l) {
      const uint64_t id = sp->locus_ids ? (uint64_t)(uint32_t)sp->locus_ids[l] : (uint64_t)l;
      hl[l].key_deg = synth_key(sp->seed, id, 1);
      hl[l].key_ent = synth_key(sp->seed, id, 2);
      hl[l].key_len = synth_key(sp->seed, id, 3);
      hl[l].T = sp->iso_lo + (int32_t)(sm64(synth_key(sp->seed, id, 0)) % (uint64_t)(sp->iso_hi - sp->iso_lo + 1));
      hl[l].pad = 0;
      h_lro[l] = (int64_t)l * rows;
      h_lio[l + 1] = h_lio[l] + hl[l].T;
   }
   h_lro[L] = n_row;
   double cdf[SYN_CDF];
   {
      double pk = std::exp(-sp->mean_extra);
      cdf[0] = pk;
      for (int k = 1; k < SYN_CDF; ++k) {
         pk = pk * (sp->mean_extra / (double)k);
         cdf[k] = cdf[k - 1] + pk;
      }
   }
   const int n_scan = (int)((n_row + SYN_SCAN_BLOCK - 1) / SYN_SCAN_BLOCK);
   const size_t b_loci = align_up(L * sizeof(SynthLocus)), b_cdf = align_up(sizeof cdf), b_deg = align_up((size_t)n_row), b_sum = align_up((size_t)n_scan * 8 + 8);
   if (!c->d_synth.reserve(b_loci + b_cdf + b_deg + b_sum + 256)) return fail(c, SBQ_ERR_NOMEM, "device allocation failed (generator scratch)");
   char* q = (char*)c->d_synth.p;
   SynthLocus* d_loci = (SynthLocus*)q; q += b_loci;
   double* d_cdf = (double*)q; q += b_cdf;
   unsigned char* d_deg = (unsigned char*)q; q += b_deg;
   long long* d_bsum = (long long*)q; q += b_sum;
   unsigned long long* d_total = (unsigned long long*)q;
   cudaStream_t st = c->stream;
   CU(cudaEventRecord(c->ev[0], st));
   CU(cudaMemcpyAsync(d_loci, hl.data(), L * sizeof(SynthLocus), cudaMemcpyHostToDevice, st));
   CU(cudaMemcpyAsync(d_cdf, cdf, sizeof cdf, cudaMemcpyHostToDevice, st));
   CU(cudaMemsetAsync(d_total, 0, 8, st));
   const int nb = c->prop.multiProcessorCount * 8;
   synth_degree_kernel<<<nb, 256, 0, st>>>(d_loci, L, rows, d_cdf, d_deg, d_total);
   CU(cudaGetLastError());
   unsigned long long total = 0;
   CU(cudaMemcpyAsync(&total, d_total, 8, cudaMemcpyDeviceToHost, st));
   CU(cudaStreamSynchronize(st));
   c->n_loci = L; c->n_row = n_row; c->n_iso = h_lio[L]; c->nnz = (int64_t)total;
   {
      const int rc = alloc_device(c);
      if (rc) { reset_batch(c); return rc; }
   }
   DevParams& dp = c->dp;
   CU(cudaMemcpyAsync(const_cast<int64_t*>(dp.loc_row_off), h_lro.data(), (L + 1) * 8, cudaMemcpyHostToDevice, st));
   CU(cudaMemcpyAsync(const_cast<int64_t*>(dp.loc_iso_off), h_lio.data(), (L + 1) * 8, cudaMemcpyHostToDevice, st));
   synth_scan_sums_kernel<<<n_scan, 1024, 0, st>>>(d_deg, n_row, d_bsum);
   synth_scan_blocks_kernel<<<1, 1024, 0, st>>>(d_bsum, n_scan);
   synth_scan_fill_kernel<<<n_scan, 1024, 0, st>>>(d_deg, n_row, d_bsum, const_cast<int64_t*>(dp.row_ptr), const_cast<int32_t*>(dp.count));
   synth_fill_kernel<<<nb, 256, 0, st>>>(d_loci, L, rows, dp.row_ptr, const_cast<int32_t*>(dp.col), const_cast<double*>(dp.alpha));
   synth_len_kernel<<<std::min(L, 1024), 256, 0, st>>>(d_loci, L, dp.loc_iso_off, const_cast<int32_t*>(dp.iso_len));
   CU(cudaGetLastError());
   std::vector<int64_t> bound((size_t)L + 1);
   CU(cudaMemcpy2DAsync(bound.data(), 8, dp.row_ptr, (size_t)rows * 8, 8, (size_t)L + 1, cudaMemcpyDeviceToHost, st));
   CU(cudaStreamSynchronize(st));
   c->meta.resize((size_t)L);
   for (int l = 0; l < L; ++l) c->meta[l] = {bound[l + 1] - bound[l], rows, (int32_t)rows, hl[l].T};
   if (rows > INT32_MAX) return fail(c, SBQ_ERR_INVALID, "rows_per_locus too large");
   {
      const int rc = plan(c);
      if (rc) { reset_batch(c); return rc; }
   }
   if (c->h_lists.n) CU(cudaMemcpyAsync(c->d_lists_p, c->h_lists.p, c->h_lists.n * sizeof(int32_t), cudaMemcpyHostToDevice, st));
   if (!c->classes.empty()) {
      if (!c->d_csc.reserve(align_up(c->nnz * 4 + 16))) return fail(c, SBQ_ERR_NOMEM, "device allocation failed (transposed-index scratch)");
      dp.csc = (unsigned*)c->d_csc.p;
   }
   CU(cudaEventRecord(c->ev[1], st));
   CU(cudaStreamSynchronize(st));
   float ms = 0;
   CU(cudaEventElapsedTime(&ms, c->ev[0], c->ev[1]));
   c->stats.upload_ms = ms;
   c->stats.h2d_bytes = 0;
   c->stats.n_loci = c->n_loci; c->stats.n_row = c->n_row; c->stats.n_iso = c->n_iso; c->stats.nnz = c->nnz;
   c->stats.weights_ms = 0.0;
   c->deferred = 2;
   c->host_released = true;
   c->resident = true;
   c->col16_ready = false;
   c->solved = c->downloaded = false;
   return SBQ_SUCCESS;
}

int sbq_fetch_batch(sbq_ctx* c, int64_t* loc_row_off_, int64_t* loc_iso_off_, int64_t* row_ptr_, int32_t* col, double* alpha, int32_t* count, int32_t* iso_len) {
   if (!c) return SBQ_ERR_INVALID;
   if (c->multi) return fail(c, SBQ_ERR_UNSUPPORTED, "sbq_fetch_batch is single-device");
   std::lock_guard<std::mutex> lk(c->mu);
   CU(cudaSetDevice(c->device));
   if (!c->resident) return fail(c, SBQ_ERR_STATE, "sbq_fetch_batch before sbq_upload / sbq_synth_giant");
   { const int rcw = upload_wait(c); if (rcw) return rcw; }
   cudaStream_t st = c->stream;
   if (loc_row_off_) CU(cudaMemcpyAsync(loc_row_off_, c->dp.loc_row_off, (c->n_loci + 1) * 8, cudaMemcpyDeviceToHost, st));
   if (loc_iso_off_) CU(cudaMemcpyAsync(loc_iso_off_, c->dp.loc_iso_off, (c->n_loci + 1) * 8, cudaMemcpyDeviceToHost, st));
   if (row_ptr_) CU(cudaMemcpyAsync(row_ptr_, c->dp.row_ptr, (c->n_row + 1) * 8, cudaMemcpyDeviceToHost, st));
   if (col) CU(cudaMemcpyAsync(col, c->dp.col, c->nnz * 4, cudaMemcpyDeviceToHost, st));
   if (alpha) CU(cudaMemcpyAsync(alpha, c->dp.alpha, c->nnz * 8, cudaMemcpyDeviceToHost, st));
   if (count) CU(cudaMemcpyAsync(count, c->dp.count, c->n_row * 4, cudaMemcpyDeviceToHost, st));
   if (iso_len) CU(cudaMemcpyAsync(iso_len, c->dp.iso_len, c->n_iso * 4, cudaMemcpyDeviceToHost, st));
   CU(cudaStreamSynchronize(st));
   return SBQ_SUCCESS;
}

int sbq_fetch_alpha(sbq_ctx* c, double* alpha) {
   if (!c || !alpha) return SBQ_ERR_INVALID;
   if (c->multi) return fail(c, SBQ_ERR_UNSUPPORTED, "sbq_fetch_alpha is single-device");
   std::lock_guard<std::mutex> lk(c->mu);
   CU(cudaSetDevice(c->device));
   if (!c->resident) return fail(c, SBQ_ERR_STATE, "sbq_fetch_alpha before sbq_upload");
   { const int rcw = upload_wait(c); if (rcw) return rcw; }
   CU(cudaMemcpyAsync(alpha, c->dp.alpha, c->nnz * 8, cudaMemcpyDeviceToHost, c->stream));
   CU(cudaStreamSynchronize(c->stream));
   return SBQ_SUCCESS;
}

int sbq_set_covariates(sbq_ctx* c, const double* x, int64_t n_row, int32_t n_cov) {
   if (!c || n_cov < 0 || n_cov > BI_MAX_COV || (n_cov > 0 && !x)) return SBQ_ERR_INVALID;
   std::lock_guard<std::mutex> lk(c->mu);
   if (n_row != c->n_row) return fail(c, SBQ_ERR_INVALID, "covariates for %lld rows, %lld rows queued", (long long)n_row, (long long)c->n_row);
   cudaSetDevice(c->device);
   c->h_cov.clear();
   if (!c->h_cov.append(x, (size_t)n_row * n_cov)) return fail(c, SBQ_ERR_NOMEM, "pinned staging");
   c->n_cov = n_cov;
   c->have_cov = true;
   c->resident = c->solved = c->downloaded = false;
   return SBQ_SUCCESS;
}

int sbq_bias_results(sbq_ctx* c, double* beta, int32_t* outer_iters) {
   if (!c) return SBQ_ERR_INVALID;
   std::lock_guard<std::mutex> lk(c->mu);
   CU(cudaSetDevice(c->device));
   if (c->cfg.bias_mode != 1 || !c->solved) return fail(c, SBQ_ERR_STATE, "sbq_bias_results needs a solved bias-mode batch");
   if (c->multi) {
      MultiState& m = *c->multi;
      const size_t K = (size_t)c->n_cov;
      for (size_t i = 0; i < m.child.size(); ++i) {
         const size_t n = m.loci_of[i].size();
         if (!n) continue;
         std::vector<double> b(n * K + 1);
         std::vector<int32_t> o(n);
         const int rc = sbq_bias_results(m.child[i], b.data(), o.data());
         if (rc) return fail(c, rc, "device %d: %s", m.devices[i], m.child[i]->err.c_str());
         for (size_t x = 0; x < n; ++x) {
            const int32_t l = m.loci_of[i][x];
            if (beta && K) memcpy(beta + (size_t)l * K, b.data() + x * K, K * 8);
            if (outer_iters) outer_iters[l] = o[x];
         }
      }
      return SBQ_SUCCESS;
   }
   const size_t K = (size_t)c->n_cov, nl = (size_t)c->n_loci;
   if (!c->r_beta.reserve(nl * K + 1) || !c->r_outer.reserve(nl)) return fail(c, SBQ_ERR_NOMEM, "pinned result buffers");
   if (K) CU(cudaMemcpyAsync(c->r_beta.p, c->bpar.beta, nl * K * 8, cudaMemcpyDeviceToHost, c->stream));
   CU(cudaMemcpyAsync(c->r_outer.p, c->bpar.outer, nl * 4, cudaMemcpyDeviceToHost, c->stream));
   CU(cudaStreamSynchronize(c->stream));
   if (beta && K) memcpy(beta, c->r_beta.p, nl * K * 8);
   if (outer_iters) memcpy(outer_iters, c->r_outer.p, nl * 4);
   return SBQ_SUCCESS;
}

int sbq_get_launch_stats(const sbq_ctx* cc, sbq_launch_stat* out, int cap) {
   if (!cc || (!out && cap > 0)) return SBQ_ERR_INVALID;
   sbq_ctx* c = const_cast<sbq_ctx*>(cc);
   std::lock_guard<std::mutex> lk(c->mu);
   if (c->multi) {
      int n = 0;
      for (sbq_ctx* ch : c->multi->child) {
         const int k = sbq_get_launch_stats(ch, out && n < cap ? out + n : nullptr, n < cap ? cap - n : 0);
         if (k > 0) n += k;
      }
      return n;
   }
   account(c);
   const int n = (int)c->launch_stats.size();
   for (int i = 0; i < n && i < cap; ++i) out[i] = c->launch_stats[i];
   return n;
}

int sbq_partition_lpt(const int64_t* cost, int64_t n, int32_t n_parts, int32_t* owner) {
   if (n < 0 || n_parts < 1 || (n > 0 && (!cost || !owner))) return SBQ_ERR_INVALID;
   std::vector<int64_t> order((size_t)n);
   for (int64_t i = 0; i < n; ++i) order[i] = i;
   std::sort(order.begin(), order.end(), [&](int64_t a, int64_t b) { return cost[a] != cost[b] ? cost[a] > cost[b] : a < b; });
   std::vector<int64_t> load((size_t)n_parts, 0);
   for (int64_t l : order) {
      int32_t best = 0;
      for (int32_t q = 1; q < n_parts; ++q)
         if (load[q] < load[best]) best = q;
      owner[l] = best;
      load[best] += cost[l];
   }
   return SBQ_SUCCESS;
}

int sbq_locus_devices(sbq_ctx* c, int32_t* device_of_locus) {
   if (!c || !device_of_locus) return SBQ_ERR_INVALID;
   std::lock_guard<std::mutex> lk(c->mu);
   if (!c->resident) return fail(c, SBQ_ERR_STATE, "sbq_locus_devices before sbq_upload");
   for (int64_t l = 0; l < c->n_loci; ++l) device_of_locus[l] = c->multi ? c->multi->devices[c->multi->owner[l]] : c->device;
   return SBQ_SUCCESS;
}

int sbq_em_solve(sbq_ctx* c, const sbq_locus* locus, double* theta, int32_t* iters) {
   if (!c || !locus || !theta) return SBQ_ERR_INVALID;
   int rc = sbq_clear(c);
   if (rc) return rc;
   if ((rc = sbq_submit(c, locus, 1))) return rc;
   if ((rc = sbq_run(c, 1000000))) return rc;
   int32_t it = 0, st = 0;
   if ((rc = sbq_results(c, theta, nullptr, nullptr, nullptr, nullptr, &it, &st))) return rc;
   if (iters) *iters = it;
   return st;
}

#ifdef SBQ_TRACE
int sbq_debug_trace(unsigned long long* out, int cap) {
   unsigned n = 0;
   cudaDeviceSynchronize();
// ... 24 lines not shown
```

### strawberry_b200/csrc/sbq_kernels.cuh

```cuda
#pragma once
#include <cooperative_groups.h>
#include <cuda_runtime.h>
#include <stdint.h>

namespace sbq {
namespace cg = cooperative_groups;

enum : int { LOCUS_OK = 0, LOCUS_ITER_CAP = 1, LOCUS_ZERO_DENOM = 2, LOCUS_NO_ROWS = 3 };

struct DevParams {
   const int64_t* loc_row_off;
   const int64_t* loc_iso_off;
   const int64_t* row_ptr;
   const int32_t* col;
   const double* alpha;
   const int32_t* count;
   const int32_t* iso_len;
   int32_t* neff;
   unsigned* csc;
   double* theta;
   double* fpkm;
   double* frac;
   int32_t* keep;
   int32_t* iters;
   int32_t* status;
   double* locus_fpkm;
   int max_iter;
   double tol;
   double row_eps;
   double min_frac;
   int eff_len_norm;
   double insert_mean;
   double rpm;
};

__device__ __forceinline__ double warp_sum(double v) {
#pragma unroll
   for (int o = 16; o > 0; o >>= 1) v += __shfl_xor_sync(0xffffffffu, v, o);
   return v;
}
__device__ __forceinline__ long long warp_sum_ll(long long v) {
#pragma unroll
   for (int o = 16; o > 0; o >>= 1) v += __shfl_xor_sync(0xffffffffu, v, o);
   return v;
}
template <int W>
__device__ __forceinline__ double group_sum(double v) {
#pragma unroll
   for (int o = W / 2; o > 0; o >>= 1) v += __shfl_xor_sync(0xffffffffu, v, o);
   return v;
}

__device__ __forceinline__ double iso_fpkm(const DevParams& p, double theta, int len, bool& na) {
   double kb;
   na = false;
   if (p.eff_len_norm) {
      kb = (double)len - p.insert_mean;
      if (kb < 0) { na = true; return 0.0; }
      kb = 1e3 / kb;
   } else {
      kb = 1e3 / (double)len;
   }
   return theta * p.rpm * kb;
}

#ifdef SBQ_TRACE
constexpr unsigned TRACE_CAP = 1u << 18;
__device__ unsigned long long g_trace[TRACE_CAP * 4];
__device__ unsigned g_trace_n;
__device__ __forceinline__ unsigned long long trace_now() { unsigned long long t; asm volatile("mov.u64 %0, %%globaltimer;" : "=l"(t)); return t; }
__device__ __forceinline__ unsigned trace_smid() { unsigned s; asm volatile("mov.u32 %0, %%smid;" : "=r"(s)); return s; }
__device__ __forceinline__ void trace_emit(unsigned cs, unsigned nt, int locus, unsigned rank, unsigned long long t0, int iters) {
   const unsigned i = atomicAdd(&g_trace_n, 1u);
   if (i < TRACE_CAP) {
      g_trace[4 * i] = ((unsigned long long)cs << 48) | ((unsigned long long)nt << 32) | (unsigned)locus;
      g_trace[4 * i + 1] = ((unsigned long long)rank << 48) | ((unsigned long long)trace_smid() << 32) | (unsigned)iters;
      g_trace[4 * i + 2] = t0;
      g_trace[4 * i + 3] = trace_now();
   }
}
#endif
constexpr int WT_WARPS = 8;
constexpr int WT_MAX_ISO = 32;
constexpr int WT_MAX_ROWS = 64;
constexpr int WT_MAX_NNZ = 256;
constexpr int WT_STRIDE = 33;

__host__ __device__ inline size_t warp_tier_smem_bytes(int max_iso) {
   return (size_t)WT_WARPS * ((size_t)max_iso * WT_STRIDE + WT_MAX_ISO) * sizeof(double);
}

constexpr int WT_REG = 4;

__global__ void __launch_bounds__(WT_WARPS * 32)
em_warp_kernel(DevParams p, const int32_t* __restrict__ list, int n_list, int max_iso, int* queue) {
   extern __shared__ double smem[];
   const int warp = threadIdx.x >> 5, lane = threadIdx.x & 31;
   double* acc = smem + (size_t)warp * ((size_t)max_iso * WT_STRIDE + WT_MAX_ISO);
   double* th = acc + (size_t)max_iso * WT_STRIDE;
   const int32_t* __restrict__ col = p.col;
   const double* __restrict__ al = p.alpha;
   const double tol2 = p.tol * p.tol;
#ifdef SBQ_TRACE
   const unsigned long long trace_t0 = trace_now();
#endif

   for (;;) {
      int w = 0;
      if (lane == 0) w = atomicAdd(queue, 1);
      w = __shfl_sync(0xffffffffu, w, 0);
      if (w >= n_list) {
#ifdef SBQ_TRACE
         if (threadIdx.x == 0) trace_emit(0, WT_WARPS * 32, -1, 0, trace_t0, 0);
#endif
         break;
      }
      const int l = list[w];
      const int64_t r0 = p.loc_row_off[l];
      const int R = (int)(p.loc_row_off[l + 1] - r0);
      const int64_t t0 = p.loc_iso_off[l];
      const int T = (int)(p.loc_iso_off[l + 1] - t0);
      const int64_t* __restrict__ rp = p.row_ptr + r0;
      int32_t* neff = p.neff + r0;

      for (int x = lane; x < T * WT_STRIDE; x += 32) acc[x] = 0.0;
      __syncwarp();

      long long tot = 0;
      int kept = 0;
      int64_t my_k0 = 0;
      int my_cnt = 0, my_ne = -1;
      for (int i = lane; i < R; i += 32) {
         const int64_t k0 = rp[i], k1 = rp[i + 1];
         const int n = p.count[r0 + i];
         tot += n;
         bool keep = false;
         for (int64_t k = k0; k < k1; ++k) keep |= al[k] > p.row_eps;
         neff[i] = keep ? n : -1;
         if (keep) {
            ++kept;
            for (int64_t k = k0; k < k1; ++k) acc[col[k] * WT_STRIDE + lane] += al[k];
         }
         if (i == lane) { my_k0 = k0; my_cnt = (int)(k1 - k0); my_ne = keep ? n : -1; }
      }
      tot = warp_sum_ll(tot);
      kept = (int)warp_sum_ll(kept);
      __syncwarp();
      const int nl = R < 32 ? R : 32;
      double s = 0.0;
      if (lane < T) {
         for (int x = 0; x < nl; ++x) { s += acc[lane * WT_STRIDE + x]; acc[lane * WT_STRIDE + x] = 0.0; }
      }
      const bool fast = R <= 32 && __all_sync(0xffffffffu, my_cnt <= WT_REG);
      double ra[WT_REG];
      int rc[WT_REG];
#pragma unroll
      for (int e = 0; e < WT_REG; ++e) {
         const bool v = fast && my_ne >= 0 && e < my_cnt;
         ra[e] = v ? al[my_k0 + e] : 0.0;
         rc[e] = v ? col[my_k0 + e] : 0;
      }
      const double theta0 = (double)tot / (double)T;
      double cur = theta0;
      int status = LOCUS_ITER_CAP, iters = 0;
      if (kept == 0) {
         status = LOCUS_NO_ROWS;
      } else {
         if (lane < T) th[lane] = cur;
         __syncwarp();
         for (int it = 0; it < p.max_iter; ++it) {
            iters = it + 1;
            bool zero = false;
            if (fast) {
               double t[WT_REG], d = 0.0;
#pragma unroll
               for (int e = 0; e < WT_REG; ++e) { t[e] = th[rc[e]]; d += ra[e] * t[e]; }
               if (my_ne >= 0) {
                  if (d == 0) {
                     zero = true;
                  } else {
                     const double r = (double)my_ne / d;
#pragma unroll
                     for (int e = 0; e < WT_REG; ++e)
                        if (ra[e] != 0.0) acc[rc[e] * WT_STRIDE + lane] += ra[e] * t[e] * r;
                  }
               }
            } else {
               for (int i = lane; i < R; i += 32) {
                  const int ne = neff[i];
                  if (ne < 0) continue;
                  const int64_t k0 = rp[i], k1 = rp[i + 1];
                  double d = 0.0;
                  for (int64_t k = k0; k < k1; ++k) d += al[k] * th[col[k]];
                  if (d == 0) {
                     zero = true;
                  } else {
                     const double r = (double)ne / d;
                     for (int64_t k = k0; k < k1; ++k) {
                        const int c = col[k];
                        acc[c * WT_STRIDE + lane] += al[k] * th[c] * r;
                     }
                  }
               }
            }
            if (__any_sync(0xffffffffu, zero)) { status = LOCUS_ZERO_DENOM; break; }
            __syncwarp();
            double nw = 0.0;
            if (lane < T) {
               double n0 = 0.0, n1 = 0.0;
               int x = 0;
               for (; x + 1 < nl; x += 2) {
                  n0 += acc[lane * WT_STRIDE + x];
                  n1 += acc[lane * WT_STRIDE + x + 1];
                  acc[lane * WT_STRIDE + x] = 0.0;
                  acc[lane * WT_STRIDE + x + 1] = 0.0;
               }
               if (x < nl) { n0 += acc[lane * WT_STRIDE + x]; acc[lane * WT_STRIDE + x] = 0.0; }
               nw = n0 + n1;
            }
            const double diff = lane < T ? nw - cur : 0.0;
            const double d2 = warp_sum(diff * diff);
            if (d2 < tol2) { status = LOCUS_OK; break; }
            cur = nw;
            __syncwarp();
            if (lane < T) th[lane] = (s != 0) ? cur / s : 0.0;
            __syncwarp();
         }
      }

      const double theta_out = (status == LOCUS_ZERO_DENOM || status == LOCUS_NO_ROWS) ? theta0 : cur;
      bool na = false;
      double f = 0.0;
      if (lane < T && status != LOCUS_NO_ROWS) f = iso_fpkm(p, theta_out, p.iso_len[t0 + lane], na);
      const double sum = warp_sum(f);
      double fr = 0.0;
      int kp = 0;
      if (lane < T && status != LOCUS_NO_ROWS) {
         if (!na) fr = f / sum;
         kp = !(fr < p.min_frac) ? (na ? -1 : 1) : 0;
      }
      const double kept_sum = warp_sum(kp != 0 ? f : 0.0);
      if (lane < T) {
         p.theta[t0 + lane] = theta_out;
         p.fpkm[t0 + lane] = f;
         p.frac[t0 + lane] = fr;
         p.keep[t0 + lane] = kp;
      }
      if (lane == 0) {
         p.iters[l] = iters;
         p.status[l] = status;
         p.locus_fpkm[l] = kept_sum;
      }
      __syncwarp();
   }
}

constexpr int CL_NT = 512;
constexpr int CL_NT_SMALL = 128;
constexpr int CL_LPR_STREAM = 32;

constexpr int CL_A2A_MAX = 4096;
constexpr size_t CL_SMEM_CAP = 220 * 1024;
__host__ __device__ inline int cluster_a2a_stride(int T) { return (T + 1) & ~1; }
__host__ __device__ inline bool cluster_a2a(int T, int cs, size_t slice_bytes) {
   if (cs <= 1 || (long long)cs * cluster_a2a_stride(T) > CL_A2A_MAX) return false;
   return ((size_t)4 * T + (size_t)cs * cluster_a2a_stride(T) + 64) * sizeof(double) + slice_bytes + 256 <= CL_SMEM_CAP;
}
__host__ __device__ inline size_t cluster_fixed_doubles(int T, int cs, size_t slice_bytes) {
   return (size_t)4 * T + (cluster_a2a(T, cs, slice_bytes) ? (size_t)cs * cluster_a2a_stride(T) + 64 : (size_t)2 * T + 64);
}

__host__ __device__ inline int cluster_stream_groups(int T, size_t smem_bytes, int nt, int cs, size_t slice_bytes) {
   const long long budget = (long long)(smem_bytes / sizeof(double)) - (long long)cluster_fixed_doubles(T, cs, slice_bytes);
   long long G = budget / (T > 0 ? T : 1);
   if (G > nt / CL_LPR_STREAM) G = nt / CL_LPR_STREAM;
   return (int)G;
}
__host__ __device__ inline int cluster_diag_slots(int T) { return (T + 7) & ~3; }
__host__ __device__ inline size_t cluster_resident_csr_bytes(size_t nnz_c, size_t nrows, int T) {
   const size_t npos = nnz_c + (size_t)T;
   return (npos + 1) * 8 + (nrows + 2) * 8 + (size_t)cluster_diag_slots(T) * 4 + nrows * 4 + ((size_t)T + 1) * 4 + nrows * 2 + npos * 2 + 64;
}
__host__ __device__ inline size_t cluster_resident_bytes(size_t nnz_c, size_t nrows, int T) {
   return cluster_resident_csr_bytes(nnz_c, nrows, T) + nnz_c * 4 + 4;
}

__host__ __device__ inline size_t cluster_class_smem(int max_iso, size_t slice_bytes, int nt, int cs) {
   const size_t fixed = cluster_fixed_doubles(max_iso, cs, slice_bytes) * sizeof(double);
   const size_t stream = (size_t)(nt / CL_LPR_STREAM) * max_iso * sizeof(double);
   const size_t want = fixed + (slice_bytes > stream ? slice_bytes : stream) + 256;
   return want < CL_SMEM_CAP ? want : CL_SMEM_CAP;
}
__host__ __device__ inline size_t cluster_slice_estimate(long long nnz, long long R, int T, int cs) {
   return (size_t)(1.12 * (double)cluster_resident_bytes((size_t)(nnz / cs + 1), (size_t)(R / cs + 1), T)) + 512;
}

template <int NT>
__device__ __forceinline__ double block_sum(double v, double* red) {
   v = warp_sum(v);
   if ((threadIdx.x & 31) == 0) red[threadIdx.x >> 5] = v;
   __syncthreads();
   double t = 0.0;
#pragma unroll
   for (int w = 0; w < NT / 32; ++w) t += red[w];
   __syncthreads();
   return t;
}

struct GlobalRows {
   const int64_t* rp;
   const double* al;
   const int32_t* col;
   int32_t* ne;
   int64_t k_a;
   __device__ __forceinline__ unsigned start(int i) const { return (unsigned)(rp[i] - k_a); }
   __device__ __forceinline__ double a(unsigned k) const { return al[k]; }
   __device__ __forceinline__ int c(unsigned k) const { return col[k]; }
   __device__ __forceinline__ int get_ne(int i) const { return ne[i]; }
   __device__ __forceinline__ void set_ne(int i, int v) const { ne[i] = v; }
};

template <int LPR, typename Rows>
__device__ __forceinline__ void cluster_setup_pass(const Rows& rows, const int32_t* __restrict__ cnt, int nrows, int G, int g, int lg,
                                                   double row_eps, double* my_acc, long long& tot, int& kept) {
   for (int base = 0; base < nrows; base += G) {
      const int i = base + g;
      const bool valid = i < nrows;
      unsigned k0 = 0, k1 = 0;
      int n = 0;
      if (valid) { k0 = rows.start(i); k1 = rows.start(i + 1); n = cnt[i]; }
      bool keep = false;
      for (unsigned k = k0 + lg; k < k1; k += LPR) keep |= rows.a(k) > row_eps;
#pragma unroll
      for (int o = LPR / 2; o > 0; o >>= 1) keep |= (bool)__shfl_xor_sync(0xffffffffu, (int)keep, o);
      if (valid && lg == 0) { rows.set_ne(i, keep ? n : -1); tot += n; kept += keep; }
      if (keep)
         for (unsigned k = k0 + lg; k < k1; k += LPR) my_acc[rows.c(k)] += rows.a(k);
      __syncwarp();
   }
}

template <int LPR, typename Rows>
__device__ __forceinline__ void cluster_em_pass(const Rows& rows, int nrows, int G, int g, int lg, const double* th, double* my_acc, int& zero) {
   for (int base = 0; base < nrows; base += 2 * G) {
      const int i0 = base + g, i1 = base + G + g;
      int ne0 = -1, ne1 = -1;
      unsigned a0 = 0, b0 = 0, a1 = 0, b1 = 0;
      if (i0 < nrows) { ne0 = rows.get_ne(i0); if (ne0 >= 0) { a0 = rows.start(i0); b0 = rows.start(i0 + 1); } }
      if (i1 < nrows) { ne1 = rows.get_ne(i1); if (ne1 >= 0) { a1 = rows.start(i1); b1 = rows.start(i1 + 1); } }
      double d0 = 0.0, d1 = 0.0;
      for (unsigned k = a0 + lg; k < b0; k += LPR) d0 += rows.a(k) * th[rows.c(k)];
      for (unsigned k = a1 + lg; k < b1; k += LPR) d1 += rows.a(k) * th[rows.c(k)];
#pragma unroll
      for (int o = LPR / 2; o > 0; o >>= 1) {
         d0 += __shfl_xor_sync(0xffffffffu, d0, o);
         d1 += __shfl_xor_sync(0xffffffffu, d1, o);
      }
      if (ne0 >= 0) {
         if (d0 == 0) zero = 1;
         else {
            const double r = (double)ne0 / d0;
            for (unsigned k = a0 + lg; k < b0; k += LPR) { const int c = rows.c(k); my_acc[c] += rows.a(k) * th[c] * r; }
         }
      }
      __syncwarp();
      if (ne1 >= 0) {
         if (d1 == 0) zero = 1;
         else {
            const double r = (double)ne1 / d1;
            for (unsigned k = a1 + lg; k < b1; k += LPR) { const int c = rows.c(k); my_acc[c] += rows.a(k) * th[c] * r; }
         }
      }
      __syncwarp();
   }
}

struct ResidentSlice {
   double* al;
   double* r;
   unsigned* jd;
   int* ne;
   unsigned* cp;
   unsigned short* rlen;
   unsigned short* col;
   unsigned* ent;
   unsigned* ent_g;
   unsigned n_ent_s;
   __device__ __forceinline__ unsigned get_ent(unsigned x) const { return x < n_ent_s ? ent[x] : ent_g[x]; }
   __device__ __forceinline__ void put_ent(unsigned x, unsigned v) const { if (x < n_ent_s) ent[x] = v; else ent_g[x] = v; }
   int nrows, T;
   unsigned nnz, npos;
};

#ifndef SBQ_MIN_LANES
#define SBQ_MIN_LANES 1
#endif
__device__ __forceinline__ int lanes_for(int items, int nt) {
   int l = 32;
   while (l > SBQ_MIN_LANES && (long long)items * l > nt) l >>= 1;
   return l;
}

template <int NT>
__device__ __forceinline__ void resident_e_pass_rows4(const ResidentSlice& S, const double* th, int& zero) {
   const int tid = threadIdx.x;
   for (int base = 0; base < S.nrows; base += 4 * NT) {
      int sv[4], ne[4], len[4];
      double d[4];
#pragma unroll
      for (int u = 0; u < 4; ++u) {
         sv[u] = base + u * NT + tid;
         ne[u] = -1; len[u] = 0; d[u] = 0.0;
         if (sv[u] < S.nrows) {
            ne[u] = S.ne[sv[u]];
            if (ne[u] >= 0) len[u] = S.rlen[sv[u]];
         }
      }
      const int maxlen = max(max(len[0], len[1]), max(len[2], len[3]));
      for (int k = 0; k < maxlen; k += 4) {
         const uint4 o = *reinterpret_cast<const uint4*>(S.jd + k);
         const unsigned ov[4] = {o.x, o.y, o.z, o.w};
         double a[4][4];
         int c[4][4];
#pragma unroll
         for (int u = 0; u < 4; ++u)
#pragma unroll
            for (int e = 0; e < 4; ++e) {
               const unsigned pos = k + e < len[u] ? ov[e] + (unsigned)sv[u] : S.npos;
               a[u][e] = S.al[pos];
               c[u][e] = (int)S.col[pos];
            }
#pragma unroll
         for (int u = 0; u < 4; ++u)
#pragma unroll
            for (int e = 0; e < 4; ++e) {
               const double t = a[u][e] * th[c[u][e]];
               d[u] += k + e < len[u] ? t : 0.0;
            }
      }
#pragma unroll
      for (int u = 0; u < 4; ++u) {
         if (sv[u] < S.nrows) {
            double r = 0.0;
            if (ne[u] >= 0) {
               if (d[u] == 0) zero = 1; else r = (double)ne[u] / d[u];
            }
            S.r[sv[u]] = r;
         }
      }
   }
}

template <int NT>
__device__ __forceinline__ void resident_e_pass(const ResidentSlice& S, const double* th, int lpr, int& zero) {
   const int tid = threadIdx.x, g = tid / lpr, lg = tid % lpr, par = NT / lpr;
   for (int base = 0; base < S.nrows; base += par) {
      const int s = base + g;
      int ne = -1, len = 0;
      if (s < S.nrows) {
         ne = S.ne[s];
         if (ne >= 0) len = S.rlen[s];
      }
      double d0 = 0.0, d1 = 0.0;
      int k = 4 * lg;
      for (; k + 4 * lpr + 4 <= len; k += 8 * lpr) {
         const uint4 o = *reinterpret_cast<const uint4*>(S.jd + k);
         const uint4 q = *reinterpret_cast<const uint4*>(S.jd + k + 4 * lpr);
         const unsigned p0 = o.x + s, p1 = o.y + s, p2 = o.z + s, p3 = o.w + s;
         const unsigned p4 = q.x + s, p5 = q.y + s, p6 = q.z + s, p7 = q.w + s;
         const int c0 = S.col[p0], c1 = S.col[p1], c2 = S.col[p2], c3 = S.col[p3];
         const int c4 = S.col[p4], c5 = S.col[p5], c6 = S.col[p6], c7 = S.col[p7];
         const double a0 = S.al[p0], a1 = S.al[p1], a2 = S.al[p2], a3 = S.al[p3];
         const double a4 = S.al[p4], a5 = S.al[p5], a6 = S.al[p6], a7 = S.al[p7];
         const double t0 = th[c0], t1 = th[c1], t2 = th[c2], t3 = th[c3];
         const double t4 = th[c4], t5 = th[c5], t6 = th[c6], t7 = th[c7];
         d0 += a0 * t0;
         d1 += a1 * t1;
         d0 += a2 * t2;
         d1 += a3 * t3;
         d0 += a4 * t4;
         d1 += a5 * t5;
         d0 += a6 * t6;
         d1 += a7 * t7;
      }
      for (; k < len; k += 4 * lpr) {
         const uint4 o = *reinterpret_cast<const uint4*>(S.jd + k);
         const bool v1 = k + 1 < len, v2 = k + 2 < len, v3 = k + 3 < len;
         const unsigned p0 = o.x + s, p1 = v1 ? o.y + s : S.npos, p2 = v2 ? o.z + s : S.npos, p3 = v3 ? o.w + s : S.npos;
         const double a0 = S.al[p0], a1 = S.al[p1], a2 = S.al[p2], a3 = S.al[p3];
         const int c0 = S.col[p0], c1 = S.col[p1], c2 = S.col[p2], c3 = S.col[p3];
         const double t0 = a0 * th[c0], t1 = a1 * th[c1], t2 = a2 * th[c2], t3 = a3 * th[c3];
         d0 += t0;
         d1 += v1 ? t1 : 0.0;
         d0 += v2 ? t2 : 0.0;
         d1 += v3 ? t3 : 0.0;
      }
      double d = d0 + d1;
      for (int o = lpr >> 1; o > 0; o >>= 1) d += __shfl_xor_sync(0xffffffffu, d, o);
      if (s < S.nrows && lg == 0) {
         double r = 0.0;
         if (ne >= 0) {
            if (d == 0) zero = 1; else r = (double)ne / d;
         }
         S.r[s] = r;
      }
   }
}

template <int NT, typename Emit>
__device__ __forceinline__ void resident_col_pass(const ResidentSlice& S, const double* scale, const Emit& emit, int lpc) {
   const int tid = threadIdx.x, g = tid / lpc, lg = tid % lpc, par = NT / lpc;
   const unsigned pad = ((unsigned)S.nrows << 16) | S.npos;
   for (int base = 0; base < S.T; base += par) {
      const int j = base + g;
      double sum = 0.0;
      if (j < S.T) {
         const unsigned x1 = S.cp[j + 1];
         for (unsigned x = S.cp[j] + lg; x < x1; x += 8 * lpc) {
            unsigned e[8];
#pragma unroll
            for (int u = 0; u < 8; ++u) e[u] = (x + u * lpc < x1) ? S.get_ent(x + u * lpc) : pad;
#pragma unroll
            for (int u = 0; u < 8; ++u) sum += S.al[e[u] & 0xffffu] * S.r[e[u] >> 16];
         }
      }
      for (int o = lpc >> 1; o > 0; o >>= 1) sum += __shfl_xor_sync(0xffffffffu, sum, o);
      if (j < S.T && lg == 0) *emit.ptr(j) = scale ? scale[j] * sum : sum;
   }
}

template <int NCACHE>
struct ColSlot {
   int j;
   int q, lanes, wl;
   unsigned x_tail, x1;
   int ncache;
   double* out;
   unsigned e[NCACHE > 0 ? NCACHE : 1];
};
struct RowSlot {
   int s;
   int q, lanes, n;
   int len;
   int ne;
};

template <int NT>
__device__ __forceinline__ unsigned assign_slots(int n_items, int my_len, unsigned total_work, unsigned* s_slot, int* s_lanes, int* s_total) {
   const int tid = threadIdx.x;
   const int budget = max(NT / 4, NT - n_items / 2 - 16);
   int E = max(8, (int)((total_work + budget - 1) / budget));
   for (;;) {
      if (tid < n_items) s_lanes[tid] = min(32, max(1, (my_len + E - 1) / E));
      __syncthreads();
      if (tid == 0) {
         int off = 0;
         for (int i0 = 0; i0 < n_items; i0 += 8) {
            int L[8];
#pragma unroll
            for (int u = 0; u < 8; ++u) L[u] = i0 + u < n_items ? s_lanes[i0 + u] : 0;
#pragma unroll
            for (int u = 0; u < 8; ++u) {
               if ((off & 31) + L[u] > 32) off = (off + 31) & ~31;
               const int o = off;
               off += L[u];
               L[u] = o | (L[u] << 16);
            }
#pragma unroll
            for (int u = 0; u < 8; ++u)
               if (i0 + u < n_items) s_lanes[i0 + u] = L[u];
         }
         *s_total = off;
      }
      __syncthreads();
      const int total = *s_total;
      if (total <= NT) break;
      __syncthreads();
      E += max(1, E >> 3);
   }
   s_slot[tid] = 0xffffffffu;
   __syncthreads();
   if (tid < n_items) {
      const int off = s_lanes[tid] & 0xffff, L = s_lanes[tid] >> 16;
      for (int q = 0; q < L; ++q) s_slot[off + q] = (unsigned)tid | ((unsigned)q << 16) | ((unsigned)L << 24);
   }
   __syncthreads();
   const unsigned sl = s_slot[tid];
   __syncthreads();
   return sl;
}

template <int NT>
__device__ __forceinline__ unsigned assign_row_slots(const unsigned short* rlen, int nrows, unsigned total_work, unsigned* s_winfo) {
   const int tid = threadIdx.x;
   if (tid < 32) {
      const int E0 = max(8, (int)((total_work + NT - 1) / NT));
      const int longest = nrows > 0 ? (int)rlen[0] : 1;
      int E = E0 + (E0 * tid + 7) / 8;
      if (tid == 31) E = max(E, longest);
      int first = 0;
      for (int w = 0; w < NT / 32 && first < nrows; ++w) first += 32 / min(32, max(1, ((int)rlen[first] + E - 1) / E));
      const unsigned fits = __ballot_sync(0xffffffffu, first >= nrows);
      if (tid == __ffs(fits) - 1) {
         int f = 0, w = 0;
         for (; w < NT / 32 && f < nrows; ++w) {
            const int L = min(32, max(1, ((int)rlen[f] + E - 1) / E));
            const int n = 32 / L;
            s_winfo[w] = (unsigned)f | ((unsigned)n << 16) | ((unsigned)L << 24);
            f += n;
         }
         for (; w < NT / 32; ++w) s_winfo[w] = 0xffffffffu;
      }
   }
   __syncthreads();
   const unsigned info = s_winfo[tid >> 5];
   __syncthreads();
   return info;
}

__device__ __forceinline__ double row_sum(double v, int q, int lanes, int n) {
   for (int o = 1; o < lanes; o <<= 1) {
      const double u = __shfl_down_sync(0xffffffffu, v, o * n);
      if (q + o < lanes) v += u;
   }
   return v;
}

__device__ __forceinline__ double group_sum(double v, int q, int lanes, int wl) {
   for (int o = 1; o < wl; o <<= 1) {
      const double u = __shfl_down_sync(0xffffffffu, v, o);
      if (q + o < lanes) v += u;
   }
   return v;
}

__device__ __forceinline__ void slot_e_pass(const ResidentSlice& S, const RowSlot& rs, const double* th, int& zero) {
   const unsigned s = (unsigned)max(rs.s, 0);
   const int len = rs.len, step = 4 * rs.lanes;
   double d0 = 0.0, d1 = 0.0;
   int k = 4 * rs.q;
   for (; k + step + 4 <= len; k += 2 * step) {
      const uint4 o = *reinterpret_cast<const uint4*>(S.jd + k);
      const uint4 q = *reinterpret_cast<const uint4*>(S.jd + k + step);
      const unsigned p0 = o.x + s, p1 = o.y + s, p2 = o.z + s, p3 = o.w + s;
      const unsigned p4 = q.x + s, p5 = q.y + s, p6 = q.z + s, p7 = q.w + s;
      const int c0 = S.col[p0], c1 = S.col[p1], c2 = S.col[p2], c3 = S.col[p3];
      const int c4 = S.col[p4], c5 = S.col[p5], c6 = S.col[p6], c7 = S.col[p7];
      const double a0 = S.al[p0], a1 = S.al[p1], a2 = S.al[p2], a3 = S.al[p3];
      const double a4 = S.al[p4], a5 = S.al[p5], a6 = S.al[p6], a7 = S.al[p7];
      const double t0 = th[c0], t1 = th[c1], t2 = th[c2], t3 = th[c3];
      const double t4 = th[c4], t5 = th[c5], t6 = th[c6], t7 = th[c7];
      d0 += a0 * t0;
      d1 += a1 * t1;
      d0 += a2 * t2;
      d1 += a3 * t3;
      d0 += a4 * t4;
      d1 += a5 * t5;
      d0 += a6 * t6;
      d1 += a7 * t7;
   }
   for (; k < len; k += step) {
      const uint4 o = *reinterpret_cast<const uint4*>(S.jd + k);
      const bool v1 = k + 1 < len, v2 = k + 2 < len, v3 = k + 3 < len;
      const unsigned p0 = o.x + s, p1 = v1 ? o.y + s : S.npos, p2 = v2 ? o.z + s : S.npos, p3 = v3 ? o.w + s : S.npos;
      const double a0 = S.al[p0], a1 = S.al[p1], a2 = S.al[p2], a3 = S.al[p3];
      const int c0 = S.col[p0], c1 = S.col[p1], c2 = S.col[p2], c3 = S.col[p3];
      const double t0 = a0 * th[c0], t1 = a1 * th[c1], t2 = a2 * th[c2], t3 = a3 * th[c3];
      d0 += t0;
      d1 += v1 ? t1 : 0.0;
      d0 += v2 ? t2 : 0.0;
      d1 += v3 ? t3 : 0.0;
   }
   const double d = row_sum(d0 + d1, rs.q, rs.lanes, rs.n);
   if (rs.s >= 0 && rs.q == 0) {
      double r = 0.0;
      if (rs.ne >= 0) {
         if (d == 0) zero = 1; else r = (double)rs.ne / d;
      }
      S.r[s] = r;
   }
}

template <int NCACHE>
__device__ __forceinline__ void slot_col_pass(const ResidentSlice& S, const ColSlot<NCACHE>& cs, const double* scale) {
   double s0 = 0.0, s1 = 0.0;
   if (NCACHE > 0) {
#pragma unroll
      for (int u0 = 0; u0 < NCACHE; u0 += 8) {
         if (u0 < cs.ncache) {
#pragma unroll
            for (int u = u0; u < u0 + 8; u += 2) {
               s0 += S.al[cs.e[u] & 0xffffu] * S.r[cs.e[u] >> 16];
               s1 += S.al[cs.e[u + 1] & 0xffffu] * S.r[cs.e[u + 1] >> 16];
            }
         }
      }
   }
   if (cs.x_tail < cs.x1) {
      const unsigned pad = ((unsigned)S.nrows << 16) | S.npos;
      for (unsigned x = cs.x_tail; x < cs.x1; x += 8 * cs.lanes) {
         unsigned e[8];
#pragma unroll
         for (int u = 0; u < 8; ++u) e[u] = (x + u * cs.lanes < cs.x1) ? S.get_ent(x + u * cs.lanes) : pad;
         double a[8], r[8];
#pragma unroll
         for (int u = 0; u < 8; ++u) { a[u] = S.al[e[u] & 0xffffu]; r[u] = S.r[e[u] >> 16]; }
#pragma unroll
         for (int u = 0; u < 8; u += 2) {
            s0 += a[u] * r[u];
            s1 += a[u + 1] * r[u + 1];
         }
      }
   }
   const double sum = group_sum(s0 + s1, cs.q, cs.lanes, cs.wl);
   if (cs.j >= 0 && cs.q == 0) *cs.out = scale ? scale[cs.j] * sum : sum;
}

__device__ __forceinline__ void cluster_arrive_release() { asm volatile("barrier.cluster.arrive.release.aligned;" ::: "memory"); }
__device__ __forceinline__ void cluster_arrive_relaxed() { asm volatile("barrier.cluster.arrive.relaxed.aligned;" ::: "memory"); }
__device__ __forceinline__ void cluster_wait() { asm volatile("barrier.cluster.wait.acquire.aligned;" ::: "memory"); }

struct OwnerMap {
   cg::cluster_group* cluster;
   double* stage;
   int B;
   unsigned rank, CS;
   __device__ __forceinline__ double* ptr(int j) const {
      const int o = j / B;
      double* base = CS > 1 ? cluster->map_shared_rank(stage, (unsigned)o) : stage;
      return base + (size_t)rank * B + (j - o * B);
   }
};
struct LocalOut {
   double* out;
   __device__ __forceinline__ double* ptr(int j) const { return out + j; }
};

template <int NT, int NCACHE, int MINB>
__global__ void __launch_bounds__(NT, MINB)
em_cluster_kernel(DevParams p, const int32_t* __restrict__ list, int n_list, unsigned smem_launch) {
   cg::cluster_group cluster = cg::this_cluster();
   const unsigned CS = cluster.num_blocks();
   const unsigned rank = cluster.block_rank();
   const int item = blockIdx.x / CS;
   const int l = list[item];
   const int tid = threadIdx.x, lane = tid & 31;
#ifdef SBQ_TRACE
   const unsigned long long trace_t0 = trace_now();
#endif

   const int64_t r0 = p.loc_row_off[l];
   const int R = (int)(p.loc_row_off[l + 1] - r0);
   const int64_t t0 = p.loc_iso_off[l];
   const int T = (int)(p.loc_iso_off[l + 1] - t0);

   extern __shared__ double smem[];
   double* th = smem;
   double* bufA = th + T;
   double* bufB = bufA + T;
   double* sdiv = bufB + T;
   double* part = sdiv + T;
   const int64_t* __restrict__ rp = p.row_ptr + r0;
   const size_t slice_est = cluster_slice_estimate((long long)(rp[R] - rp[0]), R, T, (int)CS);
   double* dyn = smem + cluster_fixed_doubles(T, (int)CS, slice_est);
   __shared__ double red[NT / 32];
   __shared__ int s_rows[2];
   double* cur = bufA;
   double* nxt = bufB;

   const unsigned smem_bytes = min(smem_launch, (unsigned)cluster_class_smem(T, slice_est, NT, (int)CS));

   if (tid < 2) {
      const int64_t base = rp[0], nnz = rp[R] - base;
      const int64_t target = base + (nnz * (int64_t)(rank + tid)) / CS;
      int lo = 0, hi = R;
      if (rank + tid >= CS) lo = R;
      else if (rank + tid == 0) hi = 0;
      while (lo < hi) {
         const int mid = (lo + hi) >> 1;
         if (rp[mid] < target) lo = mid + 1; else hi = mid;
      }
      s_rows[tid] = lo;
   }
   __syncthreads();
   const int ra = s_rows[0], rb = s_rows[1], nrows = rb - ra;
   const int64_t k_a = rp[ra];
   const unsigned nnz_c = (unsigned)(rp[rb] - k_a);

   const size_t used = (size_t)((char*)dyn - (char*)smem);
   const int lpr = lanes_for(nrows, NT), lpc = lanes_for(T, NT);
   int too_long = 0;
   for (int i = tid; i < nrows; i += NT) too_long |= (rp[ra + i + 1] - rp[ra + i]) > (int64_t)T;
   too_long = __syncthreads_or(too_long);
   const bool small_idx = (uint64_t)nnz_c + (uint64_t)T <= 65535u && nrows <= 65535 && !too_long;
   const unsigned npos = nnz_c + (unsigned)T;
   const bool csc_in_smem = small_idx && used + cluster_resident_bytes(nnz_c, (size_t)nrows, T) <= smem_bytes;
   const bool resident = small_idx && used + cluster_resident_csr_bytes(nnz_c, (size_t)nrows, T) <= smem_bytes;
   const int jdn = cluster_diag_slots(T);
   ResidentSlice S;
   S.al = dyn;
   S.r = S.al + npos + 1;
   S.jd = (unsigned*)(S.r + nrows + 1 + ((npos + nrows) & 1u));
   S.ne = (int*)(S.jd + jdn);
   S.cp = (unsigned*)(S.ne + nrows);
   S.rlen = (unsigned short*)(S.cp + T + 1);
   S.col = S.rlen + nrows;
   S.ent = (unsigned*)(S.col + npos + 1 + ((npos + 1 + nrows) & 1u));
   S.ent_g = p.csc + (size_t)k_a;
   S.n_ent_s = 0;
   if (csc_in_smem) S.n_ent_s = nnz_c;
   else if (resident) S.n_ent_s = (unsigned)min((size_t)nnz_c, (smem_bytes - used - cluster_resident_csr_bytes(nnz_c, (size_t)nrows, T)) / 4);
   S.nrows = nrows; S.T = T; S.nnz = nnz_c; S.npos = npos;
   GlobalRows grows{rp + ra, p.alpha + k_a, p.col + k_a, p.neff + r0 + ra, k_a};
   const int G = resident ? 0 : cluster_stream_groups(T, smem_bytes, NT, (int)CS, slice_est);
   double* acc = dyn;
   const int g32 = tid / CL_LPR_STREAM, lg32 = tid % CL_LPR_STREAM;
   double* my_acc = acc + (size_t)(g32 < G ? g32 : 0) * T;
   const bool use_slots = resident && T <= NT;
   const bool use_row_slots = resident && nrows <= NT;
   ColSlot<NCACHE> slot;
   slot.j = -1; slot.q = 0; slot.lanes = 1; slot.wl = 1; slot.x_tail = slot.x1 = 0; slot.ncache = 0; slot.out = part;
   RowSlot rslot;
   rslot.s = -1; rslot.q = 0; rslot.lanes = 1; rslot.n = 1; rslot.len = 0; rslot.ne = -1;

#ifdef SBQ_PHASE_TIMING
   long long ph[8] = {0, 0, 0, 0, 0, 0, 0, 0};
#define SBQ_TICK(k) { const long long t_ = clock64(); ph[k] += t_ - t_prev; t_prev = t_; }
#define SBQ_STICK(k) { const long long t_ = clock64(); st[k] += t_ - t_prev; t_prev = t_; }
   long long st[8] = {0, 0, 0, 0, 0, 0, 0, 0};
   long long t_prev = clock64();
   const long long t_start = t_prev;
#else
#define SBQ_TICK(k)
#define SBQ_STICK(k)
#endif
   long long tot = 0;
   int kept = 0;
   if (resident) {
      unsigned* keys = (unsigned*)S.al;
      int P = 1;
      while (P < nrows) P <<= 1;
      for (int i = tid; i < P; i += NT)
         keys[i] = i < nrows ? ((65535u - (unsigned)(rp[ra + i + 1] - rp[ra + i])) << 16) | (unsigned)i : 0xffffffffu;
      __syncthreads();
      for (int kk = 2; kk <= P; kk <<= 1) {
         for (int jj = kk >> 1; jj > 0; jj >>= 1) {
            for (int i = tid; i < P; i += NT) {
               const int x = i ^ jj;
               if (x > i) {
                  const unsigned a = keys[i], b = keys[x];
                  if (((i & kk) == 0) ? (a > b) : (a < b)) { keys[i] = b; keys[x] = a; }
               }
            }
            __syncthreads();
         }
      }
      SBQ_STICK(0)
      for (int i = tid; i < nrows; i += NT) {
         const unsigned key = keys[i];
         S.rlen[i] = (unsigned short)(65535u - (key >> 16));
         S.ne[i] = (int)(key & 0xffffu);
      }
      for (int j = tid; j <= T; j += NT) S.cp[j] = 0;
      __syncthreads();
      for (int k = tid; k < jdn; k += NT) {
         unsigned v = 0;
         if (k > 0) {
            int lo = 0, hi = nrows;
            while (lo < hi) {
               const int mid = (lo + hi) >> 1;
               if ((int)S.rlen[mid] > k - 1) lo = mid + 1; else hi = mid;
            }
            v = (unsigned)lo | (lo > 0 ? 1u : 0u);
         }
         S.jd[k] = v;
      }
      __syncthreads();
      if (tid < 32) {
         const int chunk = (jdn + 31) / 32, k0 = lane * chunk, k1 = min(jdn, k0 + chunk);
         unsigned sum = 0;
         for (int k = k0; k < k1; ++k) sum += S.jd[k];
         unsigned incl = sum;
         for (int o = 1; o < 32; o <<= 1) {
            const unsigned v = __shfl_up_sync(0xffffffffu, incl, o);
            if (lane >= o) incl += v;
         }
         unsigned run = incl - sum;
         for (int k = k0; k < k1; ++k) { run += S.jd[k]; S.jd[k] = run; }
      }
      __syncthreads();
      SBQ_STICK(1)
      {
         const int32_t* __restrict__ cnt = p.count + r0 + ra;
         int lf = 1;
         while (lf < 32 && (long long)lf * nrows < (long long)nnz_c) lf <<= 1;
         const int g = tid / lf, lg = tid % lf, par = NT / lf;
         for (int base = 0; base < nrows; base += 2 * par) {
            int sv[2], iv[2], lenv[2], keepv[2];
            unsigned g0v[2];
            double a[2][4];
            int c[2][4];
#pragma unroll
            for (int r = 0; r < 2; ++r) {
               sv[r] = base + r * par + g;
               iv[r] = 0; lenv[r] = 0; g0v[r] = 0; keepv[r] = 0;
               if (sv[r] < nrows) {
                  iv[r] = S.ne[sv[r]];
                  lenv[r] = S.rlen[sv[r]];
               }
            }
#pragma unroll
            for (int r = 0; r < 2; ++r)
               if (sv[r] < nrows) g0v[r] = (unsigned)(rp[ra + iv[r]] - k_a);
#pragma unroll
            for (int r = 0; r < 2; ++r)
#pragma unroll
               for (int u = 0; u < 4; ++u) {
                  const int k = lg + u * lf;
                  a[r][u] = 0.0; c[r][u] = 0;
                  if (k < lenv[r]) { a[r][u] = grows.al[g0v[r] + k]; c[r][u] = grows.col[g0v[r] + k]; }
               }
#pragma unroll
            for (int r = 0; r < 2; ++r) {
#pragma unroll
               for (int u = 0; u < 4; ++u) {
                  const int k = lg + u * lf;
                  if (k < lenv[r]) {
                     const unsigned pos = S.jd[k] + sv[r];
                     S.al[pos] = a[r][u];
                     S.col[pos] = (unsigned short)c[r][u];
                     keepv[r] |= a[r][u] > p.row_eps;
                     atomicAdd(&S.cp[c[r][u] + 1], 1u);
                  }
               }
               for (int k = lg + 4 * lf; k < lenv[r]; k += lf) {
                  const double av = grows.al[g0v[r] + k];
                  const int cv = grows.col[g0v[r] + k];
                  const unsigned pos = S.jd[k] + sv[r];
                  S.al[pos] = av;
                  S.col[pos] = (unsigned short)cv;
                  keepv[r] |= av > p.row_eps;
                  atomicAdd(&S.cp[cv + 1], 1u);
               }
            }
            __syncwarp();
#pragma unroll
            for (int r = 0; r < 2; ++r) {
               int keep = keepv[r];
               for (int o = lf >> 1; o > 0; o >>= 1) keep |= __shfl_xor_sync(0xffffffffu, keep, o);
               if (sv[r] < nrows && lg == 0) {
                  const int n = cnt[iv[r]];
                  S.ne[sv[r]] = keep ? n : -1;
                  S.r[sv[r]] = keep ? 1.0 : 0.0;
                  tot += n;
                  kept += keep;
               }
            }
         }
         if (tid == 0) { S.al[npos] = 0.0; S.col[npos] = 0; S.r[nrows] = 0.0; }
      }
      __syncthreads();
      if (tid < 32) {
         const int chunk = (T + 31) / 32, j0 = lane * chunk, j1 = min(T, j0 + chunk);
         unsigned sum = 0;
         for (int j = j0; j < j1; ++j) sum += S.cp[j + 1];
         unsigned incl = sum;
         for (int o = 1; o < 32; o <<= 1) {
            const unsigned v = __shfl_up_sync(0xffffffffu, incl, o);
            if (lane >= o) incl += v;
         }
         unsigned run = incl - sum;
         for (int j = j0; j < j1; ++j) { const unsigned c = S.cp[j + 1]; S.cp[j + 1] = run + c; run += c; }
      }
      __syncthreads();
      SBQ_STICK(2)
      {
         const int nw = NT / 32, w = tid >> 5;
         const int C = min(32, (T + nw - 1) / nw);
         const int nchunks = (T + C - 1) / C;
         const unsigned lt = (1u << lane) - 1u;
         for (int ch = w; ch < nchunks; ch += nw) {
            const int jlo = ch * C, jn = min(C, T - jlo);
            unsigned wp = lane < jn ? S.cp[jlo + lane] : 0u;
            for (int base = 0; base < nrows; base += 32) {
               const int s = base + lane;
               int len = 0, cur = 0;
               if (s < nrows) {
                  len = S.rlen[s];
                  int lo = 0, hi = len;
                  while (lo < hi) {
                     const int mid = (lo + hi) >> 1;
                     if ((int)S.col[S.jd[mid] + s] < jlo) lo = mid + 1; else hi = mid;
                  }
                  cur = lo;
               }
               unsigned pos = 0;
               int nextc = -1;
               if (cur < len) { pos = S.jd[cur] + s; nextc = S.col[pos]; }
               if (__ballot_sync(0xffffffffu, nextc >= 0 && nextc < jlo + jn) == 0u) continue;
               for (int jj = 0; jj < jn; ++jj) {
                  const bool hit = nextc == jlo + jj;
                  const unsigned m = __ballot_sync(0xffffffffu, hit);
                  const unsigned basep = __shfl_sync(0xffffffffu, wp, jj);
                  if (hit) {
                     S.put_ent(basep + __popc(m & lt), pos | ((unsigned)s << 16));
                     ++cur;
                     nextc = -1;
                     if (cur < len) { pos = S.jd[cur] + s; nextc = S.col[pos]; }
                  }
                  if (lane == jj) wp += __popc(m);
               }
            }
         }
      }
      __syncthreads();
      SBQ_STICK(3)
      __shared__ unsigned s_slot[NT];
      __shared__ int s_lanes[NT];
      __shared__ int s_total;
      if (use_row_slots) {
         const unsigned info = assign_row_slots<NT>(S.rlen, nrows, nnz_c, s_slot);
         if (info != 0xffffffffu) {
            const int first = (int)(info & 0xffffu), n = (int)((info >> 16) & 0xffu), L = (int)(info >> 24);
            rslot.lanes = L;
            rslot.n = n;
            rslot.q = lane / n;
            const int row = first + lane % n;
            if (rslot.q < L && row < nrows) {
               rslot.s = row;
               rslot.ne = S.ne[row];
               rslot.len = rslot.ne >= 0 ? (int)S.rlen[row] : 0;
            } else {
               rslot.q = L;
            }
         }
      }
      SBQ_STICK(4)
      if (use_slots) {
         const int len_j = tid < T ? (int)(S.cp[tid + 1] - S.cp[tid]) : 0;
         const unsigned sl = assign_slots<NT>(T, len_j, nnz_c, s_slot, s_lanes, &s_total);
         const unsigned pad = ((unsigned)nrows << 16) | npos;
         if (sl != 0xffffffffu) {
            slot.j = (int)(sl & 0xffffu);
            slot.lanes = (int)(sl >> 24);
            slot.q = (int)((sl >> 16) & 0xffu);
            const unsigned x0 = S.cp[slot.j] + (unsigned)slot.q;
            slot.x1 = S.cp[slot.j + 1];
            slot.x_tail = x0 + (unsigned)NCACHE * slot.lanes;
            if (NCACHE > 0) {
#pragma unroll
               for (int u = 0; u < NCACHE; ++u) {
                  const unsigned x = x0 + (unsigned)u * slot.lanes;
                  const bool v = x < slot.x1;
                  slot.e[u] = v ? S.get_ent(x) : pad;
                  slot.ncache += v;
               }
            }
            slot.out = part + slot.j;
         } else if (NCACHE > 0) {
#pragma unroll
            for (int u = 0; u < NCACHE; ++u) slot.e[u] = pad;
         }
         slot.wl = __reduce_max_sync(0xffffffffu, slot.lanes);
         SBQ_STICK(5)
         slot_col_pass(S, slot, nullptr);
      } else {
         resident_col_pass<NT>(S, nullptr, LocalOut{part}, lpc);
      }
   } else {
      for (int x = tid; x < G * T; x += NT) acc[x] = 0.0;
      __syncthreads();
      if (g32 < G) cluster_setup_pass<CL_LPR_STREAM>(grows, p.count + r0 + ra, nrows, G, g32, lg32, p.row_eps, my_acc, tot, kept);
      __syncthreads();
      for (int j = tid; j < T; j += NT) {
         double sj = 0.0;
         for (int gg = 0; gg < G; ++gg) { sj += acc[(size_t)gg * T + j]; acc[(size_t)gg * T + j] = 0.0; }
         part[j] = sj;
      }
   }
   {
      const double tot_b = block_sum<NT>((double)tot, red);
      const double kept_b = block_sum<NT>((double)kept, red);
      if (tid == 0) { part[T + 1] = tot_b; part[T + 2] = kept_b; }
   }
   cluster.sync();
   double total = 0.0, kept_all = 0.0;
   for (unsigned r = 0; r < CS; ++r) {
      const double* rp_part = CS > 1 ? cluster.map_shared_rank(part, r) : part;
      total += rp_part[T + 1];
      kept_all += rp_part[T + 2];
   }
   for (int j = tid; j < T; j += NT) {
      double sj = 0.0;
      for (unsigned r = 0; r < CS; ++r) {
         const double* rp_part = CS > 1 ? cluster.map_shared_rank(part, r) : part;
         sj += rp_part[j];
      }
      sdiv[j] = sj;
   }
   const double theta0 = total / (double)T;
   for (int j = tid; j < T; j += NT) { cur[j] = theta0; th[j] = theta0; }
   cluster.sync();

   const double tol2 = p.tol * p.tol;
   int status = LOCUS_ITER_CAP, iters = 0;
#ifdef SBQ_PHASE_TIMING
   const long long t_setup = clock64() - t_start;
   t_prev = clock64();
#endif
   const bool a2a = cluster_a2a(T, (int)CS, slice_est);
   const int Tp = cluster_a2a_stride(T);
   const int B = a2a ? Tp : (T + (int)CS - 1) / (int)CS;
   double* stage = part;
   double* dsq = a2a ? part + (size_t)CS * Tp : part + T + 16;
   double* flags = a2a ? dsq + 16 : part + 2 * T + 32;
   double* d2p = flags + 16;
   const OwnerMap own{&cluster, a2a ? stage + (size_t)rank * Tp : stage, a2a ? T : B, a2a ? 0u : rank, a2a ? 1u : CS};
   if (slot.j >= 0) slot.out = own.ptr(slot.j);
   const int nb = max(0, min(B, T - (int)rank * B));
   bool pend_b = false;
   if (kept_all == 0) {
      status = LOCUS_NO_ROWS;
   } else {
      for (int it = 0; it < p.max_iter; ++it) {
         iters = it + 1;
         int zero = 0;
         if (resident) {
            if (use_row_slots) slot_e_pass(S, rslot, th, zero);
            else if (lpr == 1) resident_e_pass_rows4<NT>(S, th, zero);
            else resident_e_pass<NT>(S, th, lpr, zero);
            SBQ_TICK(0)
            zero = __syncthreads_or(zero);
            SBQ_TICK(1)
            if (use_slots) slot_col_pass(S, slot, th);
            else resident_col_pass<NT>(S, th, own, lpc);
            SBQ_TICK(2)
         } else {
            if (g32 < G) cluster_em_pass<CL_LPR_STREAM>(grows, nrows, G, g32, lg32, th, my_acc, zero);
            zero = __syncthreads_or(zero);
            for (int j = tid; j < T; j += NT) {
               double sj = 0.0;
               for (int gg = 0; gg < G; ++gg) { sj += acc[(size_t)gg * T + j]; acc[(size_t)gg * T + j] = 0.0; }
               *own.ptr(j) = sj;
            }
         }
         double d2 = 0.0;
         if (CS == 1) {
            __syncthreads();
            SBQ_TICK(3)
            if (zero) { status = LOCUS_ZERO_DENOM; break; }
            double dd = 0.0;
            for (int j = tid; j < T; j += NT) {
               const double v = stage[j], sj = sdiv[j];
               nxt[j] = v;
               th[j] = (sj != 0) ? v / sj : 0.0;
               const double diff = v - cur[j];
               dd += diff * diff;
            }
            if ((tid & ~31) < T) dd = warp_sum(dd);
            if (lane == 0) dsq[tid >> 5] = dd;
            SBQ_TICK(4)
            __syncthreads();
            SBQ_TICK(6)
#pragma unroll
            for (int w = 0; w < NT / 32; ++w) d2 += dsq[w];
         } else if (a2a) {
            __syncthreads();
            if (pend_b) { cluster_wait(); pend_b = false; }
            {
               const int half = Tp >> 1, items = ((int)CS - 1) * half;
               const double2* mine = reinterpret_cast<const double2*>(stage + (size_t)rank * Tp);
               for (int x = tid; x < items; x += NT) {
                  const int pr = x / half, jj = x - pr * half;
                  const unsigned peer = (rank + 1u + (unsigned)pr) & (CS - 1u);
                  reinterpret_cast<double2*>(cluster.map_shared_rank(stage, peer) + (size_t)rank * Tp)[jj] = mine[jj];
               }
               if (tid < (int)CS) cluster.map_shared_rank(flags, (unsigned)tid)[rank] = (double)zero;
            }
            SBQ_TICK(3)
            cluster_arrive_release();
            cluster_wait();
            SBQ_TICK(4)
            double zf = 0.0;
            for (unsigned r = 0; r < CS; ++r) zf += flags[r];
            if (zf != 0.0) { status = LOCUS_ZERO_DENOM; break; }
            double dd = 0.0;
            for (int j = tid; j < T; j += NT) {
               double a[16];
#pragma unroll
               for (int r = 0; r < 16; ++r) a[r] = r < (int)CS ? stage[(size_t)r * Tp + j] : 0.0;
#pragma unroll
               for (int o = 8; o > 0; o >>= 1)
#pragma unroll
                  for (int r = 0; r < o; ++r) a[r] += a[r + o];
               const double v = a[0], sj = sdiv[j];
               nxt[j] = v;
               th[j] = (sj != 0) ? v / sj : 0.0;
               const double diff = v - cur[j];
               dd += diff * diff;
            }
            if ((tid & ~31) < T) dd = warp_sum(dd);
            if (lane == 0) dsq[tid >> 5] = dd;
            SBQ_TICK(5)
            __syncthreads();
            cluster_arrive_relaxed();
            pend_b = true;
            SBQ_TICK(6)
#pragma unroll
            for (int w = 0; w < NT / 32; ++w) d2 += dsq[w];
         } else {
            if (tid < (int)CS) cluster.map_shared_rank(flags, (unsigned)tid)[rank] = (double)zero;
            cluster.sync();
            SBQ_TICK(3)
            double zf = 0.0;
            for (unsigned r = 0; r < CS; ++r) zf += flags[r];
            if (zf != 0.0) { status = LOCUS_ZERO_DENOM; break; }
            {
               const int items = nb * (int)CS;
               const unsigned r = (unsigned)tid % CS;
               double* peer_nxt = cluster.map_shared_rank(nxt, r);
               double* peer_th = cluster.map_shared_rank(th, r);
               for (int base = 0; base < items; base += NT) {
                  const int x = base + tid, jj = x / (int)CS;
                  double v = x < items ? stage[(size_t)r * B + jj] : 0.0;
                  for (unsigned o = CS >> 1; o > 0; o >>= 1) v += __shfl_xor_sync(0xffffffffu, v, o);
                  if (x < items) {
                     const int j = (int)rank * B + jj;
                     const double sj = sdiv[j];
                     peer_nxt[j] = v;
                     peer_th[j] = (sj != 0) ? v / sj : 0.0;
                     if (r == 0) { const double diff = v - cur[j]; dsq[jj] = diff * diff; }
                  }
               }
            }
            SBQ_TICK(4)
            __syncthreads();
            if (tid < 32) {
               double d = 0.0;
               for (int jj = lane; jj < nb; jj += 32) d += dsq[jj];
               d = warp_sum(d);
               if (lane < (int)CS) cluster.map_shared_rank(d2p, (unsigned)lane)[rank] = d;
            }
            SBQ_TICK(5)
            cluster.sync();
            SBQ_TICK(6)
            for (unsigned r = 0; r < CS; ++r) d2 += d2p[r];
         }
         if (d2 < tol2) { status = LOCUS_OK; break; }
         { double* t_ = cur; cur = nxt; nxt = t_; }
         SBQ_TICK(7)
      }
   }
#ifdef SBQ_PHASE_TIMING
   if (rank == 0 && (tid == 0 || tid == NT - 32))
      printf("setup: sort %lld jd %lld fill %lld csc %lld rowslots %lld colslots %lld\n", st[0], st[1], st[2], st[3], st[4], st[5]);
   if (rank == 0 && (tid == 0 || tid == NT - 32))
      printf("locus %d tid %d iters %d resident %d csc_smem %d slots %d/%d lanes %d/%d ncache %d lpr %d lpc %d nrows %d nnz %u setup %lld | E %lld or %lld col %lld csync1 %lld own %lld d2 %lld csync2 %lld chk %lld (cycles/iter)\n", l, tid, iters,
             (int)resident, (int)csc_in_smem, (int)use_row_slots, (int)use_slots, rslot.lanes, slot.lanes, slot.ncache, lpr, lpc, nrows, nnz_c, t_setup, ph[0] / iters, ph[1] / iters, ph[2] / iters, ph[3] / iters, ph[4] / iters, ph[5] / iters, ph[6] / iters, ph[7] / iters);
#endif
   if (pend_b) cluster_wait();
   cluster.sync();
#ifdef SBQ_TRACE
   if (tid == 0) trace_emit(CS, NT, l, rank, trace_t0, iters);
#endif

   if (rank != 0) return;
   const bool uniform = status == LOCUS_ZERO_DENOM || status == LOCUS_NO_ROWS;
   double fsum = 0.0;
   for (int j = tid; j < T; j += NT) {
      const double tj = uniform ? theta0 : cur[j];
      bool na = false;
      double f = 0.0;
      if (status != LOCUS_NO_ROWS) f = iso_fpkm(p, tj, p.iso_len[t0 + j], na);
      p.theta[t0 + j] = tj;
      p.fpkm[t0 + j] = f;
      th[j] = na ? -1.0 : 0.0;
      fsum += f;
   }
   fsum = block_sum<NT>(fsum, red);
   double ksum = 0.0;
   for (int j = tid; j < T; j += NT) {
      const bool na = th[j] < 0;
      const double f = p.fpkm[t0 + j];
      double fr = 0.0;
      int kp = 0;
      if (status != LOCUS_NO_ROWS) {
         if (!na) fr = f / fsum;
         kp = !(fr < p.min_frac) ? (na ? -1 : 1) : 0;
      }
      p.frac[t0 + j] = fr;
      p.keep[t0 + j] = kp;
      if (kp != 0) ksum += f;
   }
   ksum = block_sum<NT>(ksum, red);
   if (tid == 0) {
      p.iters[l] = iters;
      p.status[l] = status;
      p.locus_fpkm[l] = ksum;
   }
}

__global__ void __launch_bounds__(1024) fpkm_sum_kernel(const double* __restrict__ locus_fpkm, int64_t n, double* out) {
   __shared__ double red[32];
   double v = 0.0;
   for (int64_t i = threadIdx.x; i < n; i += 1024) v += locus_fpkm[i];
   v = block_sum<1024>(v, red);
   if (threadIdx.x == 0) *out = v;
}

__global__ void tpm_kernel(const double* __restrict__ fpkm, double* __restrict__ tpm, int64_t n, double total) {
   const int64_t i = (int64_t)blockIdx.x * blockDim.x + threadIdx.x;
   if (i < n) tpm[i] = 1e6 * fpkm[i] / total;
}

__global__ void __launch_bounds__(256) locus_frags_kernel(const int64_t* __restrict__ loc_row_off, const int32_t* __restrict__ count, int64_t n_loci, long long* __restrict__ out) {
   const int lane = threadIdx.x & 31;
   const int64_t nw = ((int64_t)gridDim.x * blockDim.x) >> 5;
   for (int64_t l = ((int64_t)blockIdx.x * blockDim.x + threadIdx.x) >> 5; l < n_loci; l += nw) {
      long long v = 0;
      for (int64_t i = loc_row_off[l] + lane; i < loc_row_off[l + 1]; i += 32) v += count[i];
      v = warp_sum_ll(v);
      if (lane == 0) out[l] = v;
   }
}

__global__ void tpm_dev_kernel(const double* __restrict__ fpkm, double* __restrict__ tpm, int64_t n, const double* __restrict__ total) {
   const int64_t i = (int64_t)blockIdx.x * blockDim.x + threadIdx.x;
   const double tot = *total;
   if (i < n) tpm[i] = 1e6 * fpkm[i] / tot;
}

}
```

Baseline: 51.10 billion.

## Pack resident sparse slice into vectorized blocked layout with shared/global CSC blocks

Reorganizes the resident per-cluster sparse slice so row entries are stored in padded groups loaded as double2/uint2 with packed 16-bit column pairs, and the transposed (column) index is stored in uint4 blocks split between shared memory and a global overflow region. The column pass now walks these blocks per column instead of scalar entries with per-lane caching, removing the NCACHE template parameter and slot caching. This cuts the number of scalar shared loads in both E and column passes but adds padding overhead (extra smem allowance, larger scratch) and more complex setup.

```diff
diff --git a/strawberry_b200/csrc/sbq.cu b/strawberry_b200/csrc/sbq.cu
--- a/strawberry_b200/csrc/sbq.cu
+++ b/strawberry_b200/csrc/sbq.cu
@@ -402,7 +402,7 @@
          lc->loci.push_back((int32_t)l);
          lc->max_iso = std::max(lc->max_iso, (int)T);
          lc->max_slice = std::max(lc->max_slice, slice);
-         lc->smem = std::max(lc->smem, cluster_class_smem((int)T, slice, lc->lpr, cs));
+         lc->smem = std::max(lc->smem, cluster_class_smem((int)T, slice, cluster_pad_allowance(R, cs), lc->lpr, cs));
       }
    }
    auto by_size = [&](int32_t a, int32_t b) { return nnz_of[a] != nnz_of[b] ? nnz_of[a] > nnz_of[b] : a < b; };
@@ -508,9 +508,9 @@
    return SBQ_SUCCESS;
 }
 
-template <int NT, int NCACHE, int MINB>
+template <int NT, int MINB>
 int launch_cluster_class_nt(sbq_ctx* c, const LaunchClass& lc, cudaStream_t st) {
-   auto kernel = em_cluster_kernel<NT, NCACHE, MINB>;
+   auto kernel = em_cluster_kernel<NT, MINB>;
    int rc = set_kernel_attrs(c, kernel, lc.smem, lc.cs > 8);
    if (rc) return rc;
    cudaLaunchConfig_t cfg{};
@@ -906,7 +906,7 @@
    }
    CU(cudaEventRecord(c->ev[1], st));
    if (!c->classes.empty()) {
-      if (!c->d_csc.reserve(align_up(c->nnz * 4 + 16))) return fail(c, SBQ_ERR_NOMEM, "device allocation failed (transposed-index scratch)");
+      if (!c->d_csc.reserve(align_up(cluster_csc_scratch_entries(c->nnz, c->n_iso) * 4))) return fail(c, SBQ_ERR_NOMEM, "device allocation failed (transposed-index scratch)");
       dp.csc = (unsigned*)c->d_csc.p;
    }
    c->stats.h2d_bytes = 2 * (c->n_loci + 1) * 8 + (c->n_row + 1) * 8 + c->nnz * 12 + c->n_row * 4 + c->n_iso * 4 + (int64_t)c->h_lists.n * 4;
@@ -1043,6 +1043,7 @@
    dp.eff_len_norm = c->cfg.effective_len_norm;
    dp.insert_mean = c->cfg.insert_mean;
    dp.rpm = 1e6 / (double)(int)total_mapped_reads;
+   dp.csc_smem_cap = getenv("SBQ_CSC_SMEM_BLOCKS") ? std::max(0, atoi(getenv("SBQ_CSC_SMEM_BLOCKS"))) + 1 : 0;
 
    cudaStream_t st = c->stream;
    int64_t launches = 0;
@@ -1247,8 +1248,8 @@
       if (pending) CU(cudaStreamWaitEvent(ss, (i < N_SIDE_STREAMS && c->class_ready[i]) ? c->ev_class_ready[i] : c->ev[1], 0));
       LaunchTimer& t = c->lt[2 + i % N_SIDE_STREAMS];
       CU(cudaEventRecord(t.e0, ss));
-      int rc = lc.lpr == 64 ? launch_cluster_class_nt<64, 0, 8>(c, lc, ss) : lc.lpr == 128 ? launch_cluster_class_nt<128, 0, 4>(c, lc, ss) :
-               lc.lpr == 256 ? launch_cluster_class_nt<256, 0, 2>(c, lc, ss) : launch_cluster_class_nt<CL_NT, 0, 1>(c, lc, ss);
+      int rc = lc.lpr == 64 ? launch_cluster_class_nt<64, 8>(c, lc, ss) : lc.lpr == 128 ? launch_cluster_class_nt<128, 4>(c, lc, ss) :
+               lc.lpr == 256 ? launch_cluster_class_nt<256, 2>(c, lc, ss) : launch_cluster_class_nt<CL_NT, 1>(c, lc, ss);
       if (rc) return rc;
       CU(cudaEventRecord(t.e1, ss));
       t.used = true;
@@ -1756,7 +1757,7 @@
    if ((rc = plan(c))) return rc;
    if (c->h_lists.n) CU(cudaMemcpyAsync(c->d_lists_p, c->h_lists.p, c->h_lists.n * sizeof(int32_t), cudaMemcpyHostToDevice, st));
    if (!c->classes.empty()) {
-      if (!c->d_csc.reserve(align_up(c->nnz * 4 + 16))) return fail(c, SBQ_ERR_NOMEM, "device allocation failed (transposed-index scratch)");
+      if (!c->d_csc.reserve(align_up(cluster_csc_scratch_entries(c->nnz, c->n_iso) * 4))) return fail(c, SBQ_ERR_NOMEM, "device allocation failed (transposed-index scratch)");
       dp.csc = (unsigned*)c->d_csc.p;
    }
    CU(cudaEventRecord(c->ev[1], st));
@@ -1874,7 +1875,7 @@
    }
    if (c->h_lists.n) CU(cudaMemcpyAsync(c->d_lists_p, c->h_lists.p, c->h_lists.n * sizeof(int32_t), cudaMemcpyHostToDevice, st));
    if (!c->classes.empty()) {
-      if (!c->d_csc.reserve(align_up(c->nnz * 4 + 16))) return fail(c, SBQ_ERR_NOMEM, "device allocation failed (transposed-index scratch)");
+      if (!c->d_csc.reserve(align_up(cluster_csc_scratch_entries(c->nnz, c->n_iso) * 4))) return fail(c, SBQ_ERR_NOMEM, "device allocation failed (transposed-index scratch)");
       dp.csc = (unsigned*)c->d_csc.p;
    }
    CU(cudaEventRecord(c->ev[1], st));
diff --git a/strawberry_b200/csrc/sbq_kernels.cuh b/strawberry_b200/csrc/sbq_kernels.cuh
--- a/strawberry_b200/csrc/sbq_kernels.cuh
+++ b/strawberry_b200/csrc/sbq_kernels.cuh
@@ -18,6 +18,7 @@
    const int32_t* iso_len;
    int32_t* neff;
    unsigned* csc;
+   int csc_smem_cap;
    double* theta;
    double* fpkm;
    double* frac;
@@ -276,23 +277,33 @@
    if (G > nt / CL_LPR_STREAM) G = nt / CL_LPR_STREAM;
    return (int)G;
 }
-__host__ __device__ inline int cluster_diag_slots(int T) { return (T + 7) & ~3; }
 __host__ __device__ inline size_t cluster_resident_csr_bytes(size_t nnz_c, size_t nrows, int T) {
+   const int cluster_diag_slots = (T + 7) & ~3;
    const size_t npos = nnz_c + (size_t)T;
-   return (npos + 1) * 8 + (nrows + 2) * 8 + (size_t)cluster_diag_slots(T) * 4 + nrows * 4 + ((size_t)T + 1) * 4 + nrows * 2 + npos * 2 + 64;
+   return (npos + 1) * 8 + (nrows + 2) * 8 + (size_t)cluster_diag_slots * 4 + nrows * 4 + ((size_t)T + 1) * 4 + nrows * 2 + npos * 2 + 64;
 }
 __host__ __device__ inline size_t cluster_resident_bytes(size_t nnz_c, size_t nrows, int T) {
    return cluster_resident_csr_bytes(nnz_c, nrows, T) + nnz_c * 4 + 4;
 }
-
-__host__ __device__ inline size_t cluster_class_smem(int max_iso, size_t slice_bytes, int nt, int cs) {
+__host__ __device__ inline int cluster_diag_records(int T) { return (T + 3) / 4 + 1; }
+__host__ __device__ inline size_t cluster_slice_bytes(size_t npu, size_t nqu, size_t nrows, int T) {
+   return npu * 16 + (size_t)cluster_diag_records(T) * 16 + nqu * 8 + (nrows + 2) * 8 + nrows * 4 + ((size_t)T + 1) * 4 + nrows * 2 + 64;
+}
+__host__ __device__ inline size_t cluster_pad_allowance(long long R, int cs) { return (size_t)(14 * (R / cs + 1) + 64); }
+
+__host__ __device__ inline size_t cluster_class_smem(int max_iso, size_t slice_bytes, size_t pad_bytes, int nt, int cs) {
    const size_t fixed = cluster_fixed_doubles(max_iso, cs, slice_bytes) * sizeof(double);
    const size_t stream = (size_t)(nt / CL_LPR_STREAM) * max_iso * sizeof(double);
-   const size_t want = fixed + (slice_bytes > stream ? slice_bytes : stream) + 256;
+   const size_t want = fixed + (slice_bytes + pad_bytes > stream ? slice_bytes + pad_bytes : stream) + 256;
    return want < CL_SMEM_CAP ? want : CL_SMEM_CAP;
 }
 __host__ __device__ inline size_t cluster_slice_estimate(long long nnz, long long R, int T, int cs) {
    return (size_t)(1.12 * (double)cluster_resident_bytes((size_t)(nnz / cs + 1), (size_t)(R / cs + 1), T)) + 512;
+}
+
+__host__ __device__ inline size_t cluster_csc_scratch_entries(long long nnz, long long n_iso) { return (size_t)(2 * nnz + 128 * n_iso + 16); }
+__host__ __device__ inline size_t cluster_csc_scratch_base(long long k_a, long long t0, int T, unsigned rank) {
+   return (size_t)((2 * k_a + 128 * t0 + 8LL * T * rank + 3) & ~3LL);
 }
 
 template <int NT>
@@ -378,37 +389,43 @@
 struct ResidentSlice {
    double* al;
    double* r;
-   unsigned* jd;
+   uint4* jd;
    int* ne;
    unsigned* cp;
    unsigned short* rlen;
    unsigned short* col;
-   unsigned* ent;
-   unsigned* ent_g;
-   unsigned n_ent_s;
-   __device__ __forceinline__ unsigned get_ent(unsigned x) const { return x < n_ent_s ? ent[x] : ent_g[x]; }
-   __device__ __forceinline__ void put_ent(unsigned x, unsigned v) const { if (x < n_ent_s) ent[x] = v; else ent_g[x] = v; }
+   unsigned blk0;
+   uint4* blk_g;
+   unsigned H;
+   __device__ __forceinline__ uint4* blk() const {
+      extern __shared__ __align__(16) uint4 dyn_blocks[];
+      return dyn_blocks + blk0;
+   }
    int nrows, T;
-   unsigned nnz, npos;
+   unsigned nnz;
+   __device__ __forceinline__ const double2* a2() const { return reinterpret_cast<const double2*>(al); }
+   __device__ __forceinline__ const uint2* c4() const { return reinterpret_cast<const uint2*>(col); }
+   __device__ __forceinline__ unsigned apos(int s, int k) const {
+      const uint4 o = jd[k >> 2];
+      return 2 * (((k >> 1) & 1 ? o.y : o.x) + (unsigned)s) + (k & 1);
+   }
+   __device__ __forceinline__ unsigned cpos(int s, int k) const { return 4 * (jd[k >> 2].z + (unsigned)s) + (k & 3); }
 };
 
-#ifndef SBQ_MIN_LANES
-#define SBQ_MIN_LANES 1
-#endif
 __device__ __forceinline__ int lanes_for(int items, int nt) {
    int l = 32;
-   while (l > SBQ_MIN_LANES && (long long)items * l > nt) l >>= 1;
+   while (l > 1 && (long long)items * l > nt) l >>= 1;
    return l;
 }
 
 template <int NT>
-__device__ __forceinline__ void resident_e_pass_rows4(const ResidentSlice& S, const double* th, int& zero) {
+__device__ __forceinline__ void resident_e_pass_rows2(const ResidentSlice& S, const double* th, int& zero) {
    const int tid = threadIdx.x;
-   for (int base = 0; base < S.nrows; base += 4 * NT) {
-      int sv[4], ne[4], len[4];
-      double d[4];
-#pragma unroll
-      for (int u = 0; u < 4; ++u) {
+   for (int base = 0; base < S.nrows; base += 2 * NT) {
+      int sv[2], ne[2], len[2];
+      double d[2];
+#pragma unroll
+      for (int u = 0; u < 2; ++u) {
          sv[u] = base + u * NT + tid;
          ne[u] = -1; len[u] = 0; d[u] = 0.0;
          if (sv[u] < S.nrows) {
@@ -416,30 +433,25 @@
             if (ne[u] >= 0) len[u] = S.rlen[sv[u]];
          }
       }
-      const int maxlen = max(max(len[0], len[1]), max(len[2], len[3]));
+      const int maxlen = max(len[0], len[1]);
       for (int k = 0; k < maxlen; k += 4) {
-         const uint4 o = *reinterpret_cast<const uint4*>(S.jd + k);
-         const unsigned ov[4] = {o.x, o.y, o.z, o.w};
-         double a[4][4];
-         int c[4][4];
-#pragma unroll
-         for (int u = 0; u < 4; ++u)
+         const uint4 o = S.jd[k >> 2];
+#pragma unroll
+         for (int u = 0; u < 2; ++u) {
+            const unsigned s = (unsigned)sv[u];
+            const double2 x0 = S.a2()[k < len[u] ? o.x + s : o.x], x1 = S.a2()[k + 2 < len[u] ? o.y + s : o.x];
+            const uint2 cc = S.c4()[k < len[u] ? o.z + s : o.z];
+            const double a[4] = {x0.x, x0.y, x1.x, x1.y};
+            const int c[4] = {(int)(cc.x & 0xffffu), (int)(cc.x >> 16), (int)(cc.y & 0xffffu), (int)(cc.y >> 16)};
 #pragma unroll
             for (int e = 0; e < 4; ++e) {
-               const unsigned pos = k + e < len[u] ? ov[e] + (unsigned)sv[u] : S.npos;
-               a[u][e] = S.al[pos];
-               c[u][e] = (int)S.col[pos];
-            }
-#pragma unroll
-         for (int u = 0; u < 4; ++u)
-#pragma unroll
-            for (int e = 0; e < 4; ++e) {
-               const double t = a[u][e] * th[c[u][e]];
+               const double t = a[e] * th[c[e]];
                d[u] += k + e < len[u] ? t : 0.0;
             }
-      }
-#pragma unroll
-      for (int u = 0; u < 4; ++u) {
+         }
+      }
+#pragma unroll
+      for (int u = 0; u < 2; ++u) {
          if (sv[u] < S.nrows) {
             double r = 0.0;
             if (ne[u] >= 0) {
@@ -464,14 +476,13 @@
       double d0 = 0.0, d1 = 0.0;
       int k = 4 * lg;
       for (; k + 4 * lpr + 4 <= len; k += 8 * lpr) {
-         const uint4 o = *reinterpret_cast<const uint4*>(S.jd + k);
-         const uint4 q = *reinterpret_cast<const uint4*>(S.jd + k + 4 * lpr);
-         const unsigned p0 = o.x + s, p1 = o.y + s, p2 = o.z + s, p3 = o.w + s;
-         const unsigned p4 = q.x + s, p5 = q.y + s, p6 = q.z + s, p7 = q.w + s;
-         const int c0 = S.col[p0], c1 = S.col[p1], c2 = S.col[p2], c3 = S.col[p3];
-         const int c4 = S.col[p4], c5 = S.col[p5], c6 = S.col[p6], c7 = S.col[p7];
-         const double a0 = S.al[p0], a1 = S.al[p1], a2 = S.al[p2], a3 = S.al[p3];
-         const double a4 = S.al[p4], a5 = S.al[p5], a6 = S.al[p6], a7 = S.al[p7];
+         const uint4 o = S.jd[k >> 2], q = S.jd[(k >> 2) + lpr];
+         const double2 x0 = S.a2()[o.x + s], x1 = S.a2()[o.y + s], x2 = S.a2()[q.x + s], x3 = S.a2()[q.y + s];
+         const uint2 u0 = S.c4()[o.z + s], u1 = S.c4()[q.z + s];
+         const int c0 = u0.x & 0xffffu, c1 = u0.x >> 16, c2 = u0.y & 0xffffu, c3 = u0.y >> 16;
+         const int c4 = u1.x & 0xffffu, c5 = u1.x >> 16, c6 = u1.y & 0xffffu, c7 = u1.y >> 16;
+         const double a0 = x0.x, a1 = x0.y, a2 = x1.x, a3 = x1.y;
+         const double a4 = x2.x, a5 = x2.y, a6 = x3.x, a7 = x3.y;
          const double t0 = th[c0], t1 = th[c1], t2 = th[c2], t3 = th[c3];
          const double t4 = th[c4], t5 = th[c5], t6 = th[c6], t7 = th[c7];
          d0 += a0 * t0;
@@ -484,11 +495,12 @@
          d1 += a7 * t7;
       }
       for (; k < len; k += 4 * lpr) {
-         const uint4 o = *reinterpret_cast<const uint4*>(S.jd + k);
+         const uint4 o = S.jd[k >> 2];
          const bool v1 = k + 1 < len, v2 = k + 2 < len, v3 = k + 3 < len;
-         const unsigned p0 = o.x + s, p1 = v1 ? o.y + s : S.npos, p2 = v2 ? o.z + s : S.npos, p3 = v3 ? o.w + s : S.npos;
-         const double a0 = S.al[p0], a1 = S.al[p1], a2 = S.al[p2], a3 = S.al[p3];
-         const int c0 = S.col[p0], c1 = S.col[p1], c2 = S.col[p2], c3 = S.col[p3];
+         const double2 x0 = S.a2()[o.x + s], x1 = S.a2()[v2 ? o.y + s : o.x + s];
+         const uint2 u0 = S.c4()[o.z + s];
+         const double a0 = x0.x, a1 = x0.y, a2 = x1.x, a3 = x1.y;
+         const int c0 = u0.x & 0xffffu, c1 = u0.x >> 16, c2 = u0.y & 0xffffu, c3 = u0.y >> 16;
          const double t0 = a0 * th[c0], t1 = a1 * th[c1], t2 = a2 * th[c2], t3 = a3 * th[c3];
          d0 += t0;
          d1 += v1 ? t1 : 0.0;
@@ -507,36 +519,32 @@
    }
 }
 
+__device__ __forceinline__ void col_blocks(const ResidentSlice& S, const uint4* b, unsigned x, unsigned n, unsigned L, uint4 padv, double& sum) {
+   for (unsigned i = 0; i < n; i += 2, x += 2 * L) {
+      const uint4 e0 = b[x];
+      const uint4 e1 = i + 1 < n ? b[x + L] : padv;
+      const unsigned e[8] = {e0.x, e0.y, e0.z, e0.w, e1.x, e1.y, e1.z, e1.w};
+#pragma unroll
+      for (int u = 0; u < 8; ++u) sum += S.al[e[u] & 0xffffu] * S.r[e[u] >> 16];
+   }
+}
 template <int NT, typename Emit>
-__device__ __forceinline__ void resident_col_pass(const ResidentSlice& S, const double* scale, const Emit& emit, int lpc) {
-   const int tid = threadIdx.x, g = tid / lpc, lg = tid % lpc, par = NT / lpc;
-   const unsigned pad = ((unsigned)S.nrows << 16) | S.npos;
-   for (int base = 0; base < S.T; base += par) {
-      const int j = base + g;
+__device__ __forceinline__ void resident_col_pass(const ResidentSlice& S, const double* scale, const Emit& emit) {
+   const unsigned pad = (unsigned)S.nrows << 16;
+   const uint4 padv = make_uint4(pad, pad, pad, pad);
+   for (int j = threadIdx.x; j < S.T; j += NT) {
+      const unsigned c0 = S.cp[j], c1 = S.cp[j + 1];
       double sum = 0.0;
-      if (j < S.T) {
-         const unsigned x1 = S.cp[j + 1];
-         for (unsigned x = S.cp[j] + lg; x < x1; x += 8 * lpc) {
-            unsigned e[8];
-#pragma unroll
-            for (int u = 0; u < 8; ++u) e[u] = (x + u * lpc < x1) ? S.get_ent(x + u * lpc) : pad;
-#pragma unroll
-            for (int u = 0; u < 8; ++u) sum += S.al[e[u] & 0xffffu] * S.r[e[u] >> 16];
-         }
-      }
-      for (int o = lpc >> 1; o > 0; o >>= 1) sum += __shfl_xor_sync(0xffffffffu, sum, o);
-      if (j < S.T && lg == 0) *emit.ptr(j) = scale ? scale[j] * sum : sum;
-   }
-}
-
-template <int NCACHE>
+      col_blocks(S, S.blk(), c0 & 0x3fffu, (c1 & 0x3fffu) - (c0 & 0x3fffu), 1, padv, sum);
+      col_blocks(S, S.blk_g, c0 >> 14, (c1 >> 14) - (c0 >> 14), 1, padv, sum);
+      *emit.ptr(j) = scale ? scale[j] * sum : sum;
+   }
+}
+
 struct ColSlot {
    int j;
-   int q, lanes, wl;
-   unsigned x_tail, x1;
-   int ncache;
-   double* out;
-   unsigned e[NCACHE > 0 ? NCACHE : 1];
+   unsigned qlw;
+   unsigned bs, bg;
 };
 struct RowSlot {
    int s;
@@ -640,14 +648,13 @@
    double d0 = 0.0, d1 = 0.0;
    int k = 4 * rs.q;
    for (; k + step + 4 <= len; k += 2 * step) {
-      const uint4 o = *reinterpret_cast<const uint4*>(S.jd + k);
-      const uint4 q = *reinterpret_cast<const uint4*>(S.jd + k + step);
-      const unsigned p0 = o.x + s, p1 = o.y + s, p2 = o.z + s, p3 = o.w + s;
-      const unsigned p4 = q.x + s, p5 = q.y + s, p6 = q.z + s, p7 = q.w + s;
-      const int c0 = S.col[p0], c1 = S.col[p1], c2 = S.col[p2], c3 = S.col[p3];
-      const int c4 = S.col[p4], c5 = S.col[p5], c6 = S.col[p6], c7 = S.col[p7];
-      const double a0 = S.al[p0], a1 = S.al[p1], a2 = S.al[p2], a3 = S.al[p3];
-      const double a4 = S.al[p4], a5 = S.al[p5], a6 = S.al[p6], a7 = S.al[p7];
+      const uint4 o = S.jd[k >> 2], q = S.jd[(k + step) >> 2];
+      const double2 x0 = S.a2()[o.x + s], x1 = S.a2()[o.y + s], x2 = S.a2()[q.x + s], x3 = S.a2()[q.y + s];
+      const uint2 u0 = S.c4()[o.z + s], u1 = S.c4()[q.z + s];
+      const int c0 = u0.x & 0xffffu, c1 = u0.x >> 16, c2 = u0.y & 0xffffu, c3 = u0.y >> 16;
+      const int c4 = u1.x & 0xffffu, c5 = u1.x >> 16, c6 = u1.y & 0xffffu, c7 = u1.y >> 16;
+      const double a0 = x0.x, a1 = x0.y, a2 = x1.x, a3 = x1.y;
+      const double a4 = x2.x, a5 = x2.y, a6 = x3.x, a7 = x3.y;
       const double t0 = th[c0], t1 = th[c1], t2 = th[c2], t3 = th[c3];
       const double t4 = th[c4], t5 = th[c5], t6 = th[c6], t7 = th[c7];
       d0 += a0 * t0;
@@ -660,11 +667,12 @@
       d1 += a7 * t7;
    }
    for (; k < len; k += step) {
-      const uint4 o = *reinterpret_cast<const uint4*>(S.jd + k);
+      const uint4 o = S.jd[k >> 2];
       const bool v1 = k + 1 < len, v2 = k + 2 < len, v3 = k + 3 < len;
-      const unsigned p0 = o.x + s, p1 = v1 ? o.y + s : S.npos, p2 = v2 ? o.z + s : S.npos, p3 = v3 ? o.w + s : S.npos;
-      const double a0 = S.al[p0], a1 = S.al[p1], a2 = S.al[p2], a3 = S.al[p3];
-      const int c0 = S.col[p0], c1 = S.col[p1], c2 = S.col[p2], c3 = S.col[p3];
+      const double2 x0 = S.a2()[o.x + s], x1 = S.a2()[v2 ? o.y + s : o.x + s];
+      const uint2 u0 = S.c4()[o.z + s];
+      const double a0 = x0.x, a1 = x0.y, a2 = x1.x, a3 = x1.y;
+      const int c0 = u0.x & 0xffffu, c1 = u0.x >> 16, c2 = u0.y & 0xffffu, c3 = u0.y >> 16;
       const double t0 = a0 * th[c0], t1 = a1 * th[c1], t2 = a2 * th[c2], t3 = a3 * th[c3];
       d0 += t0;
       d1 += v1 ? t1 : 0.0;
@@ -681,39 +689,31 @@
    }
 }
 
-template <int NCACHE>
-__device__ __forceinline__ void slot_col_pass(const ResidentSlice& S, const ColSlot<NCACHE>& cs, const double* scale) {
+__device__ __forceinline__ void slot_col_blocks(const ResidentSlice& S, const uint4* b, unsigned x, unsigned n, unsigned L, double& s0, double& s1) {
+   const unsigned pad = (unsigned)S.nrows << 16, end = x + n * L;
+   for (; x < end; x += 2 * L) {
+      const uint4 e0 = b[x];
+      const uint4 e1 = x + L < end ? b[x + L] : make_uint4(pad, pad, pad, pad);
+      const unsigned e[8] = {e0.x, e0.y, e0.z, e0.w, e1.x, e1.y, e1.z, e1.w};
+      double a[8], r[8];
+#pragma unroll
+      for (int u = 0; u < 8; ++u) { a[u] = S.al[e[u] & 0xffffu]; r[u] = S.r[e[u] >> 16]; }
+#pragma unroll
+      for (int u = 0; u < 8; u += 2) {
+         s0 += a[u] * r[u];
+         s1 += a[u + 1] * r[u + 1];
+      }
+   }
+}
+
+template <typename Emit>
+__device__ __forceinline__ void slot_col_pass(const ResidentSlice& S, const ColSlot& cs, const double* scale, const Emit& emit) {
    double s0 = 0.0, s1 = 0.0;
-   if (NCACHE > 0) {
-#pragma unroll
-      for (int u0 = 0; u0 < NCACHE; u0 += 8) {
-         if (u0 < cs.ncache) {
-#pragma unroll
-            for (int u = u0; u < u0 + 8; u += 2) {
-               s0 += S.al[cs.e[u] & 0xffffu] * S.r[cs.e[u] >> 16];
-               s1 += S.al[cs.e[u + 1] & 0xffffu] * S.r[cs.e[u + 1] >> 16];
-            }
-         }
-      }
-   }
-   if (cs.x_tail < cs.x1) {
-      const unsigned pad = ((unsigned)S.nrows << 16) | S.npos;
-      for (unsigned x = cs.x_tail; x < cs.x1; x += 8 * cs.lanes) {
-         unsigned e[8];
-#pragma unroll
-         for (int u = 0; u < 8; ++u) e[u] = (x + u * cs.lanes < cs.x1) ? S.get_ent(x + u * cs.lanes) : pad;
-         double a[8], r[8];
-#pragma unroll
-         for (int u = 0; u < 8; ++u) { a[u] = S.al[e[u] & 0xffffu]; r[u] = S.r[e[u] >> 16]; }
-#pragma unroll
-         for (int u = 0; u < 8; u += 2) {
-            s0 += a[u] * r[u];
-            s1 += a[u + 1] * r[u + 1];
-         }
-      }
-   }
-   const double sum = group_sum(s0 + s1, cs.q, cs.lanes, cs.wl);
-   if (cs.j >= 0 && cs.q == 0) *cs.out = scale ? scale[cs.j] * sum : sum;
+   const int q = (int)(cs.qlw & 0xffu), lanes = (int)((cs.qlw >> 8) & 0xffu), wl = (int)(cs.qlw >> 16);
+   slot_col_blocks(S, S.blk(), cs.bs & 0xffffu, cs.bs >> 16, (unsigned)lanes, s0, s1);
+   slot_col_blocks(S, S.blk_g, cs.bg & 0xffffu, cs.bg >> 16, (unsigned)lanes, s0, s1);
+   const double sum = group_sum(s0 + s1, q, lanes, wl);
+   if (cs.j >= 0 && q == 0) *emit.ptr(cs.j) = scale ? scale[cs.j] * sum : sum;
 }
 
 __device__ __forceinline__ void cluster_arrive_release() { asm volatile("barrier.cluster.arrive.release.aligned;" ::: "memory"); }
@@ -736,7 +736,7 @@
    __device__ __forceinline__ double* ptr(int j) const { return out + j; }
 };
 
-template <int NT, int NCACHE, int MINB>
+template <int NT, int MINB>
 __global__ void __launch_bounds__(NT, MINB)
 em_cluster_kernel(DevParams p, const int32_t* __restrict__ list, int n_list, unsigned smem_launch) {
    cg::cluster_group cluster = cg::this_cluster();
@@ -754,7 +754,7 @@
    const int64_t t0 = p.loc_iso_off[l];
    const int T = (int)(p.loc_iso_off[l + 1] - t0);
 
-   extern __shared__ double smem[];
+   extern __shared__ __align__(16) double smem[];
    double* th = smem;
    double* bufA = th + T;
    double* bufB = bufA + T;
@@ -762,13 +762,15 @@
    double* part = sdiv + T;
    const int64_t* __restrict__ rp = p.row_ptr + r0;
    const size_t slice_est = cluster_slice_estimate((long long)(rp[R] - rp[0]), R, T, (int)CS);
-   double* dyn = smem + cluster_fixed_doubles(T, (int)CS, slice_est);
+   const size_t fixed_d = cluster_fixed_doubles(T, (int)CS, slice_est);
+   double* dyn = smem + fixed_d;
    __shared__ double red[NT / 32];
    __shared__ int s_rows[2];
+   __shared__ unsigned s_units[2];
    double* cur = bufA;
    double* nxt = bufB;
 
-   const unsigned smem_bytes = min(smem_launch, (unsigned)cluster_class_smem(T, slice_est, NT, (int)CS));
+   const unsigned smem_bytes = min(smem_launch, (unsigned)cluster_class_smem(T, slice_est, cluster_pad_allowance(R, (int)CS), NT, (int)CS));
 
    if (tid < 2) {
       const int64_t base = rp[0], nnz = rp[R] - base;
@@ -788,29 +790,38 @@
    const unsigned nnz_c = (unsigned)(rp[rb] - k_a);
 
    const size_t used = (size_t)((char*)dyn - (char*)smem);
-   const int lpr = lanes_for(nrows, NT), lpc = lanes_for(T, NT);
+   const int lpr = lanes_for(nrows, NT);
+   if (tid < 2) s_units[tid] = 0u;
+   __syncthreads();
    int too_long = 0;
-   for (int i = tid; i < nrows; i += NT) too_long |= (rp[ra + i + 1] - rp[ra + i]) > (int64_t)T;
+   unsigned pu = 0, qu = 0;
+   for (int i = tid; i < nrows; i += NT) {
+      const int64_t len = rp[ra + i + 1] - rp[ra + i];
+      too_long |= len > (int64_t)T;
+      pu += (unsigned)((len + 1) >> 1);
+      qu += (unsigned)((len + 3) >> 2);
+   }
+   pu = __reduce_add_sync(0xffffffffu, pu);
+   qu = __reduce_add_sync(0xffffffffu, qu);
+   if (lane == 0) { atomicAdd(&s_units[0], pu); atomicAdd(&s_units[1], qu); }
    too_long = __syncthreads_or(too_long);
-   const bool small_idx = (uint64_t)nnz_c + (uint64_t)T <= 65535u && nrows <= 65535 && !too_long;
-   const unsigned npos = nnz_c + (unsigned)T;
-   const bool csc_in_smem = small_idx && used + cluster_resident_bytes(nnz_c, (size_t)nrows, T) <= smem_bytes;
-   const bool resident = small_idx && used + cluster_resident_csr_bytes(nnz_c, (size_t)nrows, T) <= smem_bytes;
-   const int jdn = cluster_diag_slots(T);
+   const unsigned npu = s_units[0] + (unsigned)(T + 1) / 2, nqu = s_units[1] + (unsigned)(T + 3) / 4;
+   const bool small_idx = !too_long && 2ull * npu <= 65536ull && nrows <= 65535;
+   const bool resident = small_idx && used + cluster_slice_bytes(npu, nqu, (size_t)nrows, T) <= smem_bytes;
+   const int jdn = cluster_diag_records(T);
    ResidentSlice S;
-   S.al = dyn;
-   S.r = S.al + npos + 1;
-   S.jd = (unsigned*)(S.r + nrows + 1 + ((npos + nrows) & 1u));
-   S.ne = (int*)(S.jd + jdn);
+   S.al = dyn + (fixed_d & 1);
+   S.jd = reinterpret_cast<uint4*>(S.al + 2 * npu);
+   S.col = reinterpret_cast<unsigned short*>(S.jd + jdn);
+   S.r = reinterpret_cast<double*>(S.col + 4 * nqu);
+   S.ne = (int*)(S.r + nrows + 1);
    S.cp = (unsigned*)(S.ne + nrows);
    S.rlen = (unsigned short*)(S.cp + T + 1);
-   S.col = S.rlen + nrows;
-   S.ent = (unsigned*)(S.col + npos + 1 + ((npos + 1 + nrows) & 1u));
-   S.ent_g = p.csc + (size_t)k_a;
-   S.n_ent_s = 0;
-   if (csc_in_smem) S.n_ent_s = nnz_c;
-   else if (resident) S.n_ent_s = (unsigned)min((size_t)nnz_c, (smem_bytes - used - cluster_resident_csr_bytes(nnz_c, (size_t)nrows, T)) / 4);
-   S.nrows = nrows; S.T = T; S.nnz = nnz_c; S.npos = npos;
+   S.blk0 = (unsigned)(((char*)(S.rlen + nrows) - (char*)smem + 15) / 16);
+   S.blk_g = reinterpret_cast<uint4*>(p.csc + cluster_csc_scratch_base(k_a, t0, T, rank));
+   const unsigned blk_room = resident ? (unsigned)(smem_bytes / 16 - S.blk0) : 0u;
+   S.H = 0;
+   S.nrows = nrows; S.T = T; S.nnz = nnz_c;
    GlobalRows grows{rp + ra, p.alpha + k_a, p.col + k_a, p.neff + r0 + ra, k_a};
    const int G = resident ? 0 : cluster_stream_groups(T, smem_bytes, NT, (int)CS, slice_est);
    double* acc = dyn;
@@ -818,8 +829,8 @@
    double* my_acc = acc + (size_t)(g32 < G ? g32 : 0) * T;
    const bool use_slots = resident && T <= NT;
    const bool use_row_slots = resident && nrows <= NT;
-   ColSlot<NCACHE> slot;
-   slot.j = -1; slot.q = 0; slot.lanes = 1; slot.wl = 1; slot.x_tail = slot.x1 = 0; slot.ncache = 0; slot.out = part;
+   ColSlot slot;
+   slot.j = -1; slot.qlw = 1u << 8; slot.bs = slot.bg = 0;
    RowSlot rslot;
    rslot.s = -1; rslot.q = 0; rslot.lanes = 1; rslot.n = 1; rslot.len = 0; rslot.ne = -1;
 
@@ -863,30 +874,36 @@
       }
       for (int j = tid; j <= T; j += NT) S.cp[j] = 0;
       __syncthreads();
-      for (int k = tid; k < jdn; k += NT) {
-         unsigned v = 0;
-         if (k > 0) {
+      for (int q = tid; q < jdn; q += NT) {
+         unsigned v[2];
+#pragma unroll
+         for (int h = 0; h < 2; ++h) {
             int lo = 0, hi = nrows;
             while (lo < hi) {
                const int mid = (lo + hi) >> 1;
-               if ((int)S.rlen[mid] > k - 1) lo = mid + 1; else hi = mid;
-            }
-            v = (unsigned)lo | (lo > 0 ? 1u : 0u);
-         }
-         S.jd[k] = v;
+               if ((int)S.rlen[mid] > 4 * q + 2 * h) lo = mid + 1; else hi = mid;
+            }
+            v[h] = (unsigned)lo | (lo > 0 ? 1u : 0u);
+         }
+         S.jd[q] = make_uint4(v[0], v[1], v[0], 0u);
       }
       __syncthreads();
       if (tid < 32) {
-         const int chunk = (jdn + 31) / 32, k0 = lane * chunk, k1 = min(jdn, k0 + chunk);
-         unsigned sum = 0;
-         for (int k = k0; k < k1; ++k) sum += S.jd[k];
-         unsigned incl = sum;
+         const int chunk = (jdn + 31) / 32, k0 = min(jdn, lane * chunk), k1 = min(jdn, k0 + chunk);
+         unsigned sp = 0, sq = 0;
+         for (int k = k0; k < k1; ++k) { const uint4 o = S.jd[k]; sp += o.x + o.y; sq += o.z; }
+         unsigned ip = sp, iq = sq;
          for (int o = 1; o < 32; o <<= 1) {
-            const unsigned v = __shfl_up_sync(0xffffffffu, incl, o);
-            if (lane >= o) incl += v;
-         }
-         unsigned run = incl - sum;
-         for (int k = k0; k < k1; ++k) { run += S.jd[k]; S.jd[k] = run; }
+            const unsigned a = __shfl_up_sync(0xffffffffu, ip, o), b = __shfl_up_sync(0xffffffffu, iq, o);
+            if (lane >= o) { ip += a; iq += b; }
+         }
+         unsigned rp_ = ip - sp, rq = iq - sq;
+         for (int k = k0; k < k1; ++k) {
+            const uint4 o = S.jd[k];
+            S.jd[k] = make_uint4(rp_, rp_ + o.x, rq, 0u);
+            rp_ += o.x + o.y;
+            rq += o.z;
+         }
       }
       __syncthreads();
       SBQ_STICK(1)
@@ -926,9 +943,8 @@
                for (int u = 0; u < 4; ++u) {
                   const int k = lg + u * lf;
                   if (k < lenv[r]) {
-                     const unsigned pos = S.jd[k] + sv[r];
-                     S.al[pos] = a[r][u];
-                     S.col[pos] = (unsigned short)c[r][u];
+                     S.al[S.apos(sv[r], k)] = a[r][u];
+                     S.col[S.cpos(sv[r], k)] = (unsigned short)c[r][u];
                      keepv[r] |= a[r][u] > p.row_eps;
                      atomicAdd(&S.cp[c[r][u] + 1], 1u);
                   }
@@ -936,9 +952,8 @@
                for (int k = lg + 4 * lf; k < lenv[r]; k += lf) {
                   const double av = grows.al[g0v[r] + k];
                   const int cv = grows.col[g0v[r] + k];
-                  const unsigned pos = S.jd[k] + sv[r];
-                  S.al[pos] = av;
-                  S.col[pos] = (unsigned short)cv;
+                  S.al[S.apos(sv[r], k)] = av;
+                  S.col[S.cpos(sv[r], k)] = (unsigned short)cv;
                   keepv[r] |= av > p.row_eps;
                   atomicAdd(&S.cp[cv + 1], 1u);
                }
@@ -949,6 +964,10 @@
                int keep = keepv[r];
                for (int o = lf >> 1; o > 0; o >>= 1) keep |= __shfl_xor_sync(0xffffffffu, keep, o);
                if (sv[r] < nrows && lg == 0) {
+                  for (int k = lenv[r]; k < ((lenv[r] + 3) & ~3); ++k) {
+                     S.col[S.cpos(sv[r], k)] = 0;
+                     if (k < ((lenv[r] + 1) & ~1)) S.al[S.apos(sv[r], k)] = 0.0;
+                  }
                   const int n = cnt[iv[r]];
                   S.ne[sv[r]] = keep ? n : -1;
                   S.r[sv[r]] = keep ? 1.0 : 0.0;
@@ -957,7 +976,7 @@
                }
             }
          }
-         if (tid == 0) { S.al[npos] = 0.0; S.col[npos] = 0; S.r[nrows] = 0.0; }
+         if (tid == 0) S.r[nrows] = 0.0;
       }
       __syncthreads();
       if (tid < 32) {
@@ -974,6 +993,89 @@
       }
       __syncthreads();
       SBQ_STICK(2)
+      __shared__ unsigned s_slot[NT];
+      __shared__ int s_lanes[NT];
+      __shared__ int s_total;
+      __shared__ unsigned s_H;
+      unsigned slot_n = 0;
+      if (use_slots) {
+         const int len_j = tid < T ? (int)(S.cp[tid + 1] - S.cp[tid]) : 0;
+         const unsigned sl = assign_slots<NT>(T, len_j, nnz_c, s_slot, s_lanes, &s_total);
+         if (sl != 0xffffffffu) {
+            slot.j = (int)(sl & 0xffffu);
+            slot.qlw = ((sl >> 16) & 0xffu) | ((sl >> 24) << 8);
+            slot_n = S.cp[slot.j + 1] - S.cp[slot.j];
+         }
+         slot.qlw |= __reduce_max_sync(0xffffffffu, (slot.qlw >> 8) & 0xffu) << 16;
+      }
+      __syncthreads();
+      if (tid < 32) {
+         auto nblk = [&](int j, unsigned n) -> unsigned {
+            const unsigned L = use_slots ? (unsigned)s_lanes[j] >> 16 : 1u;
+            return ((n + L - 1) / L + 3) / 4;
+         };
+         auto lanes_of = [&](int j) -> unsigned { return use_slots ? (unsigned)s_lanes[j] >> 16 : 1u; };
+         unsigned hi = 0;
+         for (int j = lane; j < T; j += 32) hi = max(hi, nblk(j, S.cp[j + 1] - S.cp[j]));
+         hi = __reduce_max_sync(0xffffffffu, hi);
+         if (p.csc_smem_cap > 0) hi = min(hi, (unsigned)(p.csc_smem_cap - 1));
+         unsigned lo = 0;
+         while (lo < hi) {
+            const unsigned mid = (lo + hi + 1) >> 1;
+            long long need = 0;
+            for (int j = lane; j < T; j += 32) need += (long long)min(nblk(j, S.cp[j + 1] - S.cp[j]), mid) * lanes_of(j);
+            need = warp_sum_ll(need);
+            if (need <= (long long)blk_room) lo = mid; else hi = mid - 1;
+         }
+         const unsigned H = lo;
+         const int chunk = (T + 31) / 32, j0 = min(T, lane * chunk), j1 = min(T, j0 + chunk);
+         unsigned ss = 0, gs = 0;
+         for (int j = j0; j < j1; ++j) {
+            const unsigned nb = nblk(j, S.cp[j + 1] - S.cp[j]), L = lanes_of(j);
+            ss += min(nb, H) * L;
+            gs += (nb - min(nb, H)) * L;
+         }
+         unsigned si = ss, gi = gs;
+         for (int o = 1; o < 32; o <<= 1) {
+            const unsigned a = __shfl_up_sync(0xffffffffu, si, o), b = __shfl_up_sync(0xffffffffu, gi, o);
+            if (lane >= o) { si += a; gi += b; }
+         }
+         unsigned c_prev = S.cp[j0];
+         const unsigned c_end = S.cp[j1];
+         __syncwarp();
+         unsigned rs = si - ss, rg = gi - gs;
+         for (int j = j0; j < j1; ++j) {
+            const unsigned c_next = j + 1 < j1 ? S.cp[j + 1] : c_end;
+            const unsigned nb = nblk(j, c_next - c_prev), L = lanes_of(j);
+            S.cp[j] = rs | (rg << 14);
+            rs += min(nb, H) * L;
+            rg += (nb - min(nb, H)) * L;
+            c_prev = c_next;
+         }
+         if (lane == 31) { S.cp[T] = si | (gi << 14); s_H = H; }
+      }
+      __syncthreads();
+      S.H = s_H;
+      const unsigned pad = (unsigned)nrows << 16;
+      const uint4 padv = make_uint4(pad, pad, pad, pad);
+      if (use_slots) {
+         if (slot.j >= 0) {
+            const unsigned L = (slot.qlw >> 8) & 0xffu, q = slot.qlw & 0xffu, cb = S.cp[slot.j];
+            const unsigned nq = slot_n > q ? (slot_n - q + L - 1) / L : 0u, nb = (nq + 3) / 4;
+            const unsigned ns = min(nb, S.H), ng = nb - ns, xs = (cb & 0x3fffu) + q, xg = (cb >> 14) + q;
+            slot.bs = xs | (ns << 16);
+            slot.bg = xg | (ng << 16);
+            if (ng > 0) S.blk_g[xg + (ng - 1) * L] = padv;
+            else if (ns > 0) S.blk()[xs + (ns - 1) * L] = padv;
+         }
+      } else {
+         for (int j = tid; j < T; j += NT) {
+            const unsigned c0 = S.cp[j], c1 = S.cp[j + 1];
+            if ((c1 >> 14) > (c0 >> 14)) S.blk_g[(c1 >> 14) - 1] = padv;
+            else if ((c1 & 0x3fffu) > (c0 & 0x3fffu)) S.blk()[(c1 & 0x3fffu) - 1] = padv;
+         }
+      }
+      __syncthreads();
       {
          const int nw = NT / 32, w = tid >> 5;
          const int C = min(32, (T + nw - 1) / nw);
@@ -981,7 +1083,7 @@
          const unsigned lt = (1u << lane) - 1u;
          for (int ch = w; ch < nchunks; ch += nw) {
             const int jlo = ch * C, jn = min(C, T - jlo);
-            unsigned wp = lane < jn ? S.cp[jlo + lane] : 0u;
+            unsigned wp = 0u;
             for (int base = 0; base < nrows; base += 32) {
                const int s = base + lane;
                int len = 0, cur = 0;
@@ -990,23 +1092,28 @@
                   int lo = 0, hi = len;
                   while (lo < hi) {
                      const int mid = (lo + hi) >> 1;
-                     if ((int)S.col[S.jd[mid] + s] < jlo) lo = mid + 1; else hi = mid;
+                     if ((int)S.col[S.cpos(s, mid)] < jlo) lo = mid + 1; else hi = mid;
                   }
                   cur = lo;
                }
                unsigned pos = 0;
                int nextc = -1;
-               if (cur < len) { pos = S.jd[cur] + s; nextc = S.col[pos]; }
+               if (cur < len) { pos = S.apos(s, cur); nextc = S.col[S.cpos(s, cur)]; }
                if (__ballot_sync(0xffffffffu, nextc >= 0 && nextc < jlo + jn) == 0u) continue;
                for (int jj = 0; jj < jn; ++jj) {
                   const bool hit = nextc == jlo + jj;
                   const unsigned m = __ballot_sync(0xffffffffu, hit);
                   const unsigned basep = __shfl_sync(0xffffffffu, wp, jj);
                   if (hit) {
-                     S.put_ent(basep + __popc(m & lt), pos | ((unsigned)s << 16));
+                     const int j = jlo + jj;
+                     const unsigned i = basep + __popc(m & lt), L = use_slots ? (unsigned)s_lanes[j] >> 16 : 1u;
+                     const unsigned q = i % L, e = i / L, b = e >> 2, cb = S.cp[j];
+                     unsigned* dst = b < S.H ? reinterpret_cast<unsigned*>(S.blk() + (cb & 0x3fffu) + b * L + q)
+                                             : reinterpret_cast<unsigned*>(S.blk_g + (cb >> 14) + (b - S.H) * L + q);
+                     dst[e & 3u] = pos | ((unsigned)s << 16);
                      ++cur;
                      nextc = -1;
-                     if (cur < len) { pos = S.jd[cur] + s; nextc = S.col[pos]; }
+                     if (cur < len) { pos = S.apos(s, cur); nextc = S.col[S.cpos(s, cur)]; }
                   }
                   if (lane == jj) wp += __popc(m);
                }
@@ -1015,9 +1122,6 @@
       }
       __syncthreads();
       SBQ_STICK(3)
-      __shared__ unsigned s_slot[NT];
-      __shared__ int s_lanes[NT];
-      __shared__ int s_total;
       if (use_row_slots) {
          const unsigned info = assign_row_slots<NT>(S.rlen, nrows, nnz_c, s_slot);
          if (info != 0xffffffffu) {
@@ -1037,35 +1141,10 @@
       }
       SBQ_STICK(4)
       if (use_slots) {
-         const int len_j = tid < T ? (int)(S.cp[tid + 1] - S.cp[tid]) : 0;
-         const unsigned sl = assign_slots<NT>(T, len_j, nnz_c, s_slot, s_lanes, &s_total);
-         const unsigned pad = ((unsigned)nrows << 16) | npos;
-         if (sl != 0xffffffffu) {
-            slot.j = (int)(sl & 0xffffu);
-            slot.lanes = (int)(sl >> 24);
-            slot.q = (int)((sl >> 16) & 0xffu);
-            const unsigned x0 = S.cp[slot.j] + (unsigned)slot.q;
-            slot.x1 = S.cp[slot.j + 1];
-            slot.x_tail = x0 + (unsigned)NCACHE * slot.lanes;
-            if (NCACHE > 0) {
-#pragma unroll
-               for (int u = 0; u < NCACHE; ++u) {
-                  const unsigned x = x0 + (unsigned)u * slot.lanes;
-                  const bool v = x < slot.x1;
-                  slot.e[u] = v ? S.get_ent(x) : pad;
-                  slot.ncache += v;
-               }
-            }
-            slot.out = part + slot.j;
-         } else if (NCACHE > 0) {
-#pragma unroll
-            for (int u = 0; u < NCACHE; ++u) slot.e[u] = pad;
-         }
-         slot.wl = __reduce_max_sync(0xffffffffu, slot.lanes);
          SBQ_STICK(5)
-         slot_col_pass(S, slot, nullptr);
+         slot_col_pass(S, slot, nullptr, LocalOut{part});
       } else {
-         resident_col_pass<NT>(S, nullptr, LocalOut{part}, lpc);
+         resident_col_pass<NT>(S, nullptr, LocalOut{part});
       }
    } else {
       for (int x = tid; x < G * T; x += NT) acc[x] = 0.0;
@@ -1116,7 +1195,6 @@
    double* flags = a2a ? dsq + 16 : part + 2 * T + 32;
    double* d2p = flags + 16;
    const OwnerMap own{&cluster, a2a ? stage + (size_t)rank * Tp : stage, a2a ? T : B, a2a ? 0u : rank, a2a ? 1u : CS};
-   if (slot.j >= 0) slot.out = own.ptr(slot.j);
    const int nb = max(0, min(B, T - (int)rank * B));
    bool pend_b = false;
    if (kept_all == 0) {
@@ -1127,13 +1205,13 @@
          int zero = 0;
          if (resident) {
             if (use_row_slots) slot_e_pass(S, rslot, th, zero);
-            else if (lpr == 1) resident_e_pass_rows4<NT>(S, th, zero);
+            else if (lpr == 1) resident_e_pass_rows2<NT>(S, th, zero);
             else resident_e_pass<NT>(S, th, lpr, zero);
             SBQ_TICK(0)
             zero = __syncthreads_or(zero);
             SBQ_TICK(1)
-            if (use_slots) slot_col_pass(S, slot, th);
-            else resident_col_pass<NT>(S, th, own, lpc);
+            if (use_slots) slot_col_pass(S, slot, th, own);
+            else resident_col_pass<NT>(S, th, own);
             SBQ_TICK(2)
          } else {
             if (g32 < G) cluster_em_pass<CL_LPR_STREAM>(grows, nrows, G, g32, lg32, th, my_acc, zero);
@@ -1255,8 +1333,8 @@
    if (rank == 0 && (tid == 0 || tid == NT - 32))
       printf("setup: sort %lld jd %lld fill %lld csc %lld rowslots %lld colslots %lld\n", st[0], st[1], st[2], st[3], st[4], st[5]);
    if (rank == 0 && (tid == 0 || tid == NT - 32))
-      printf("locus %d tid %d iters %d resident %d csc_smem %d slots %d/%d lanes %d/%d ncache %d lpr %d lpc %d nrows %d nnz %u setup %lld | E %lld or %lld col %lld csync1 %lld own %lld d2 %lld csync2 %lld chk %lld (cycles/iter)\n", l, tid, iters,
-             (int)resident, (int)csc_in_smem, (int)use_row_slots, (int)use_slots, rslot.lanes, slot.lanes, slot.ncache, lpr, lpc, nrows, nnz_c, t_setup, ph[0] / iters, ph[1] / iters, ph[2] / iters, ph[3] / iters, ph[4] / iters, ph[5] / iters, ph[6] / iters, ph[7] / iters);
+      printf("locus %d tid %d iters %d resident %d idx_blocks_smem %u slots %d/%d lanes %d/%d idx_blocks %u+%u lpr %d nrows %d nnz %u setup %lld | E %lld or %lld col %lld csync1 %lld own %lld d2 %lld csync2 %lld chk %lld (cycles/iter)\n", l, tid, iters,
+             (int)resident, S.H, (int)use_row_slots, (int)use_slots, rslot.lanes, (int)((slot.qlw >> 8) & 0xffu), slot.bs >> 16, slot.bg >> 16, lpr, nrows, nnz_c, t_setup, ph[0] / iters, ph[1] / iters, ph[2] / iters, ph[3] / iters, ph[4] / iters, ph[5] / iters, ph[6] / iters, ph[7] / iters);
 #endif
    if (pend_b) cluster_wait();
    cluster.sync();
```

Measured after the change: 53.96 billion, median of 6. 5.6% higher.
